# olsson-group/thermodynamic-interpolation

Hardware: AMD Instinct MI355X
Metric: integration-steps/sec (whole node) + drift rel-L2 vs CPU ref (higher is better)
Workload: dtype f32 state and accumulation; matrix products on fp16 MFMA with 2-way split fp32 operands (hi + lo halves, 3 products)

## Files before the change

### include/ti_hip.h

```cpp
#ifndef TI_HIP_H
#define TI_HIP_H

#include <stddef.h>
#include <stdint.h>

#ifdef __cplusplus
extern "C" {
#endif

#define TI_ABI_VERSION 5

enum { TI_OK = 0, TI_E_ARG = -1, TI_E_HIP = -2, TI_E_NAN = -3, TI_E_ALLOC = -4, TI_E_UNSUPPORTED = -5 };
enum { TI_MEM_HOST = 0, TI_MEM_DEVICE = 1 };
enum { TI_VARIANT_AMBIENT = 0, TI_VARIANT_LATENT_MULTI = 1, TI_VARIANT_LATENT_SINGLE = 2 };
enum { TI_PREC_F32 = 0, TI_PREC_F16X2 = 1, TI_PREC_F16 = 2 };
enum { TI_SCHEME_EULER = 0, TI_SCHEME_HEUN = 1, TI_SCHEME_EM = 2,
       TI_SCHEME_DOPRI5 = 3, TI_SCHEME_MIDPOINT = 4, TI_SCHEME_RK4 = 5,
       TI_SCHEME_DOPRI5_TRAJ = 6 };

typedef struct ti_handle ti_handle;

typedef struct ti_painn_desc {
    int32_t variant;
    int32_t n_features;
// ... 33 lines not shown

int ti_version(void);
int ti_device_count(void);
const char* ti_last_error(void);

ti_handle* ti_adw_create(const ti_adw_desc* desc, const double* weights, size_t n_weights, int device);
ti_handle* ti_adw_create_nd(const ti_adw_desc* desc, int32_t dim, const double* weights, size_t n_weights, int device);
int ti_adw_drift(ti_handle* h, const float* x, float t, const float* beta0, const float* beta1, int64_t B, float* out, int mem);
int ti_adw_drift_div(ti_handle* h, const float* x, float t, const float* beta0, const float* beta1, int64_t B, float* out,
                     float* out_div, int mem);
int ti_adw_drift_tv(ti_handle* h, const float* x, const float* t, const float* beta0, const float* beta1, int64_t B, float* out,
                    float* out_div, int mem);
int ti_adw_rollout(ti_handle* h, const ti_rollout_desc* desc, const float* x0, const float* beta0, const float* beta1,
                   int64_t B, float* out_path, int64_t* n_fevals);
int ti_adw_rollout_dlogp(ti_handle* h, const ti_rollout_desc* desc, const float* x0, const float* beta0, const float* beta1,
                         int64_t B, float* out_path, float* out_dlogp, int64_t* n_fevals);
int ti_adw_rollout_fused(ti_handle* h, const ti_rollout_desc* desc, const float* x0, const float* beta0, const float* beta1,
                         int64_t B, float* out_path, float* out_dlogp , int64_t* n_fevals);

ti_handle* ti_painn_create(const ti_painn_desc* desc, const float* weights, size_t n_weights,
                           const int32_t* edge_src, const int32_t* edge_dst, const int32_t* edge_type,
                           const int32_t* atom_ids, int device);
int ti_painn_drift(ti_handle* h, const float* x, float t, const float* cond, int64_t B, float* out, int mem);
int ti_painn_drift_tv(ti_handle* h, const float* x, const float* t, const float* cond, int64_t B, float* out, int mem);
int ti_painn_rollout(ti_handle* h, const ti_rollout_desc* desc, const float* x0, const float* cond, int64_t B,
                     float* out_path, int64_t* n_fevals);

int ti_painn_drift_jvp(ti_handle* h, const float* x, const float* xdot, float t, const float* cond, int64_t B, float* out,
                       float* out_tan, int mem);
int ti_painn_drift_div(ti_handle* h, const float* x, float t, const float* cond, int64_t B, float* out, float* out_div, int mem);
int ti_painn_drift_div_tv(ti_handle* h, const float* x, const float* t, const float* cond, int64_t B, float* out, float* out_div, int mem);
int ti_painn_rollout_dlogp(ti_handle* h, const ti_rollout_desc* desc, const float* x0, const float* cond, int64_t B,
                           float div_scale, float out_scale, int reverse_ode, float* out_path, float* out_dlogp, int64_t* n_fevals);

int ti_painn_drift_div_est(ti_handle* h, const float* x, float t, const float* cond, int64_t B, int32_t n_probes, uint64_t probe_seed,
                           int64_t traj_offset, float* out, float* out_div, int mem);
int ti_painn_drift_div_est_tv(ti_handle* h, const float* x, const float* t, const float* cond, int64_t B, int32_t n_probes,
                              uint64_t probe_seed, int64_t traj_offset, float* out, float* out_div, int mem);
int ti_painn_rollout_dlogp_est(ti_handle* h, const ti_rollout_desc* desc, int32_t n_probes, uint64_t probe_seed, const float* x0,
                               const float* cond, int64_t B, float div_scale, float out_scale, int reverse_ode, float* out_path,
                               float* out_dlogp, int64_t* n_fevals);

int ti_rollout_step_counts(ti_handle* h, int64_t* accepted, int64_t* rejected, int64_t B);
void ti_destroy(ti_handle* h);
enum { TI_STREAM_OWN = 0, TI_STREAM_EXTERNAL = 1 };
int ti_set_stream(ti_handle* h, void* hip_stream, int mode);
int ti_wait_stream(ti_handle* h, void* producer_stream);
enum { TI_TEMPLATE_AUTO = -1, TI_TEMPLATE_THROUGHPUT = 0, TI_TEMPLATE_LATENCY = 1, TI_TEMPLATE_PAIR = 2 };
int ti_painn_set_template(ti_handle* h, int which);
int ti_painn_template_for(ti_handle* h, int64_t B);
int ti_painn_set_edge_mask(ti_handle* h, const uint32_t* mask, int64_t B, int mem);
int ti_painn_set_molecules(ti_handle* h, const int32_t* n_atoms, const uint32_t* mask, const uint8_t* pair_type, int64_t B, int mem);
enum { TI_OBS_RMSD = 0, TI_OBS_DIST = 1, TI_OBS_ANGLE = 2, TI_OBS_TORSION = 3, TI_OBS_COORD = 4 };
int ti_obs_cv(ti_handle* h, const int32_t* desc, int32_t K, const float* ref, const int32_t* select, const float* x, int64_t B,
              float* out_cv, int mem);
int ti_obs_weights(ti_handle* h, const float* logw, int64_t B, float* out_w, double* out_ess, int mem);
int ti_obs_hist(ti_handle* h, const float* values, int64_t stride, const float* logw, int64_t B, int32_t n_bins, double lo, double hi,
                double* out_hist, double* out_tails, int mem);
enum { TI_BOOT_ESS = 0, TI_BOOT_TFEP = 1, TI_BOOT_MEAN = 2 };
enum { TI_BOOT_FILTER_NONE = 0, TI_BOOT_FILTER_ONCE = 1, TI_BOOT_FILTER_RESAMPLE = 2 };
#define TI_BOOT_DOMAIN 0x424f4f54u
#define TI_BOOT_MAX_RESAMPLES (1 << 20)
typedef struct {
    int32_t  estimator, filter;
    double   k;
    double   level;
    int64_t  n_boot;
    int64_t  first;
    uint64_t seed;
} ti_boot_desc;
int ti_obs_bootstrap(ti_handle* h, const float* logw, int64_t n, const ti_boot_desc* d,
                     const int32_t* idx, int64_t n_draw, double* out, double* out_boot, int mem);
int ti_obs_set_observer(ti_handle* h, const int32_t* desc, int32_t K, const float* ref, const int32_t* select, int32_t every,
                        float* out_cv, int mem);
int ti_reserve(ti_handle* h, int64_t B);
enum { TI_KERNEL_PAINN_EDGE = 0, TI_KERNEL_PAINN_UPDATE = 1, TI_KERNEL_PAINN_EMBED = 2, TI_KERNEL_PAINN_READOUT = 3,
       TI_KERNEL_ADW = 4, TI_KERNEL_INTEGRATE = 5, TI_KERNEL_PAINN_JVP_EDGE = 6, TI_KERNEL_PAINN_JVP_UPDATE = 7,
       TI_KERNEL_PAINN_JVP_READOUT = 8, TI_KERNEL_PAINN_JVP_FILTER = 9, TI_KERNEL_COUNT = 10 };
int ti_profile_enable(ti_handle* h, int on);
int ti_profile_read(ti_handle* h, int kernel, int64_t* n_launches, double* total_ms);
int ti_painn_debug_tap(ti_handle* h, int stop_after_stage);
int ti_painn_debug_read(ti_handle* h, int what, float* out, size_t n_floats);
int ti_painn_debug_poison(ti_handle* h, int64_t B, float value);
int ti_selftest(int device);

#ifdef __cplusplus
}
#endif
#endif
```

### thermodynamic-interpolation_amd/_lib.py

```python
from __future__ import annotations

import ctypes as C
import os

import numpy as np

HERE = os.path.dirname(os.path.abspath(__file__))
SO_PATH = os.environ.get("TI_LIB_PATH") or os.path.join(HERE, "libti_hip.so")

TI_OK, TI_E_ARG, TI_E_HIP, TI_E_NAN, TI_E_ALLOC, TI_E_UNSUPPORTED = 0, -1, -2, -3, -4, -5
MEM_HOST, MEM_DEVICE = 0, 1
SCHEMES = {"euler": 0, "heun": 1, "em": 2, "dopri5": 3, "midpoint": 4, "rk4": 5}
SCHEME_DOPRI5_TRAJ = 6
PRECISIONS = {"f32": 0, "f16x2": 1, "f16": 2}
KERNELS = {"painn_edge": 0, "painn_update": 1, "painn_embed": 2, "painn_readout": 3, "adw": 4, "integrate": 5,
           "painn_jvp_edge": 6, "painn_jvp_update": 7, "painn_jvp_readout": 8, "painn_jvp_filter": 9}

ABI_SYMBOLS = [
    "ti_rollout_rows", "ti_version", "ti_device_count", "ti_last_error",
    "ti_adw_create", "ti_adw_drift", "ti_adw_drift_div", "ti_adw_rollout", "ti_adw_rollout_dlogp",
    "ti_painn_create", "ti_painn_drift", "ti_painn_rollout", "ti_painn_drift_jvp", "ti_painn_drift_div", "ti_painn_rollout_dlogp",
    "ti_destroy", "ti_set_stream", "ti_wait_stream", "ti_painn_set_template", "ti_painn_template_for", "ti_reserve", "ti_profile_enable", "ti_profile_read",
    "ti_painn_debug_tap", "ti_painn_debug_read", "ti_painn_debug_poison", "ti_selftest",
    "ti_painn_drift_tv", "ti_painn_drift_div_tv", "ti_adw_drift_tv", "ti_rollout_step_counts",
    "ti_painn_drift_div_est", "ti_painn_drift_div_est_tv", "ti_painn_rollout_dlogp_est",
    "ti_adw_create_nd", "ti_painn_set_edge_mask", "ti_painn_set_molecules",
    "ti_obs_cv", "ti_obs_weights", "ti_obs_hist", "ti_obs_set_observer",
    "ti_adw_rollout_fused",
    "ti_obs_bootstrap",
]
OBS_KINDS = {"rmsd": 0, "dist": 1, "angle": 2, "torsion": 3, "coord": 4}
BOOT_ESTIMATORS = {"ess": 0, "tfep": 1, "mean": 2}
BOOT_FILTERS = {"none": 0, "once": 1, "resample": 2}
BOOT_DOMAIN = 0x424F4F54
BOOT_MAX_RESAMPLES = 1 << 20


class PainnDesc(C.Structure):
    _fields_ = [("variant", C.c_int32), ("n_features", C.c_int32), ("n_layers", C.c_int32), ("n_types", C.c_int32),
                ("n_atoms", C.c_int32), ("n_edges", C.c_int32), ("temp_length", C.c_float), ("time_length", C.c_float),
                ("length_scale", C.c_float), ("temp_mean", C.c_float), ("temp_range", C.c_float), ("precision", C.c_int32)]


class AdwDesc(C.Structure):
    _fields_ = [("hidden_size", C.c_int32), ("num_layers", C.c_int32), ("precision", C.c_int32)]


class RolloutDesc(C.Structure):
    _fields_ = [("scheme", C.c_int32), ("n_step", C.c_int32), ("save_every", C.c_int32), ("mem", C.c_int32),
                ("eps", C.c_float), ("com_free_noise", C.c_int32), ("seed", C.c_uint64), ("traj_offset", C.c_int64),
                ("t_grid", C.POINTER(C.c_float)), ("rtol", C.c_float), ("atol", C.c_float), ("step_offset", C.c_int64)]


class BootDesc(C.Structure):
    _fields_ = [("estimator", C.c_int32), ("filter", C.c_int32), ("k", C.c_double), ("level", C.c_double), ("n_boot", C.c_int64),
                ("first", C.c_int64), ("seed", C.c_uint64)]


class TiError(RuntimeError):
    def __init__(self, code, msg):
        super().__init__(f"libti_hip error {code}: {msg}")
        self.code = code


_lib = None


def _preload_torch_hip_runtime():
    import importlib.util
    try:
        spec = importlib.util.find_spec("torch")
    except (ImportError, ValueError):
        spec = None
    if spec is None or not spec.origin:
        return
    cand = os.path.join(os.path.dirname(spec.origin), "lib", "libamdhip64.so")
    if os.path.exists(cand):
        C.CDLL(cand, mode=C.RTLD_GLOBAL)


def lib():
    global _lib
    if _lib is not None:
        return _lib
    if not os.path.exists(SO_PATH):
        raise RuntimeError(f"{SO_PATH} is missing: build it with `python -c 'import __graft_entry__ as g; g.build()'` "
                           "(hipcc, gfx950).  There is no CPU fallback for the sampling path.")
    _preload_torch_hip_runtime()
    L = C.CDLL(SO_PATH)
    fp, ip, vp = C.POINTER(C.c_float), C.POINTER(C.c_int32), C.c_void_p
    L.ti_rollout_rows.restype = C.c_int64
    L.ti_rollout_rows.argtypes = [C.c_int32, C.c_int32]
    L.ti_last_error.restype = C.c_char_p
    L.ti_painn_create.restype = vp
    L.ti_painn_create.argtypes = [C.POINTER(PainnDesc), fp, C.c_size_t, ip, ip, ip, ip, C.c_int]
    L.ti_painn_drift.argtypes = [vp, vp, C.c_float, vp, C.c_int64, vp, C.c_int]
    L.ti_painn_rollout.argtypes = [vp, C.POINTER(RolloutDesc), vp, vp, C.c_int64, vp, C.POINTER(C.c_int64)]
    L.ti_painn_drift_jvp.argtypes = [vp, vp, vp, C.c_float, vp, C.c_int64, vp, vp, C.c_int]
    L.ti_painn_drift_div.argtypes = [vp, vp, C.c_float, vp, C.c_int64, vp, vp, C.c_int]
    L.ti_painn_rollout_dlogp.argtypes = [vp, C.POINTER(RolloutDesc), vp, vp, C.c_int64, C.c_float, C.c_float, C.c_int, vp, vp, C.POINTER(C.c_int64)]
    L.ti_adw_create.restype = vp
    L.ti_adw_create.argtypes = [C.POINTER(AdwDesc), C.POINTER(C.c_double), C.c_size_t, C.c_int]
    L.ti_adw_create_nd.restype = vp
    L.ti_adw_create_nd.argtypes = [C.POINTER(AdwDesc), C.c_int32, C.POINTER(C.c_double), C.c_size_t, C.c_int]
    L.ti_adw_drift.argtypes = [vp, vp, C.c_float, vp, vp, C.c_int64, vp, C.c_int]
    L.ti_adw_rollout.argtypes = [vp, C.POINTER(RolloutDesc), vp, vp, vp, C.c_int64, vp, C.POINTER(C.c_int64)]
    L.ti_adw_drift_div.argtypes = [vp, vp, C.c_float, vp, vp, C.c_int64, vp, vp, C.c_int]
    L.ti_adw_rollout_dlogp.argtypes = [vp, C.POINTER(RolloutDesc), vp, vp, vp, C.c_int64, vp, vp, C.POINTER(C.c_int64)]
    L.ti_adw_rollout_fused.argtypes = [vp, C.POINTER(RolloutDesc), vp, vp, vp, C.c_int64, vp, vp, C.POINTER(C.c_int64)]
    L.ti_destroy.argtypes = [vp]
    L.ti_destroy.restype = None
    L.ti_set_stream.argtypes = [vp, vp, C.c_int]
    L.ti_wait_stream.argtypes = [vp, vp]
    L.ti_painn_set_template.argtypes = [vp, C.c_int]
    L.ti_painn_template_for.argtypes = [vp, C.c_int64]
    L.ti_reserve.argtypes = [vp, C.c_int64]
    L.ti_profile_enable.argtypes = [vp, C.c_int]
    L.ti_profile_read.argtypes = [vp, C.c_int, C.POINTER(C.c_int64), C.POINTER(C.c_double)]
    L.ti_painn_debug_tap.argtypes = [vp, C.c_int]
    L.ti_painn_debug_read.argtypes = [vp, C.c_int, fp, C.c_size_t]
    L.ti_painn_debug_poison.argtypes = [vp, C.c_int64, C.c_float]
    L.ti_selftest.argtypes = [C.c_int]
    L.ti_painn_drift_tv.argtypes = [vp, vp, vp, vp, C.c_int64, vp, C.c_int]
    L.ti_painn_drift_div_tv.argtypes = [vp, vp, vp, vp, C.c_int64, vp, vp, C.c_int]
    L.ti_adw_drift_tv.argtypes = [vp, vp, vp, vp, vp, C.c_int64, vp, vp, C.c_int]
    L.ti_rollout_step_counts.argtypes = [vp, C.POINTER(C.c_int64), C.POINTER(C.c_int64), C.c_int64]
    L.ti_painn_drift_div_est.argtypes = [vp, vp, C.c_float, vp, C.c_int64, C.c_int32, C.c_uint64, C.c_int64, vp, vp, C.c_int]
    L.ti_painn_drift_div_est_tv.argtypes = [vp, vp, vp, vp, C.c_int64, C.c_int32, C.c_uint64, C.c_int64, vp, vp, C.c_int]
    L.ti_painn_rollout_dlogp_est.argtypes = [vp, C.POINTER(RolloutDesc), C.c_int32, C.c_uint64, vp, vp, C.c_int64, C.c_float, C.c_float,
                                             C.c_int, vp, vp, C.POINTER(C.c_int64)]
    L.ti_painn_set_edge_mask.argtypes = [vp, vp, C.c_int64, C.c_int]
    L.ti_painn_set_molecules.argtypes = [vp, vp, vp, vp, C.c_int64, C.c_int]
    L.ti_obs_cv.argtypes = [vp, ip, C.c_int32, fp, ip, vp, C.c_int64, vp, C.c_int]
    L.ti_obs_weights.argtypes = [vp, vp, C.c_int64, vp, C.POINTER(C.c_double), C.c_int]
    L.ti_obs_hist.argtypes = [vp, vp, C.c_int64, vp, C.c_int64, C.c_int32, C.c_double, C.c_double, C.POINTER(C.c_double), C.POINTER(C.c_double),
                              C.c_int]
    L.ti_obs_set_observer.argtypes = [vp, ip, C.c_int32, fp, ip, C.c_int32, vp, C.c_int]
    L.ti_obs_bootstrap.argtypes = [vp, vp, C.c_int64, C.POINTER(BootDesc), vp, C.c_int64, C.POINTER(C.c_double), vp, C.c_int]
    _lib = L
    return L


def check(rc):
    if rc != TI_OK:
        raise TiError(rc, lib().ti_last_error().decode())


def last_error() -> str:
    return lib().ti_last_error().decode()


def fptr(a: np.ndarray):
    return a.ctypes.data_as(C.POINTER(C.c_float))


def iptr(a: np.ndarray):
    return a.ctypes.data_as(C.POINTER(C.c_int32))


def as_ptr(buf, *, shape=None, out=False, what="buffer"):
    if buf is None:
        return None, None, False, None
    if isinstance(buf, int):
        return C.c_void_p(buf), None, True, None
    if hasattr(buf, "data_ptr"):
        if str(buf.dtype) != "torch.float32":
            raise TypeError(f"{what} must be float32, got {buf.dtype}")
        if not buf.is_contiguous():
            raise ValueError(f"{what} must be contiguous")
        if shape is not None and tuple(buf.shape) != tuple(shape):
            raise ValueError(f"{what} must have shape {tuple(shape)}, got {tuple(buf.shape)}")
        dev = bool(buf.is_cuda)
        return C.c_void_p(buf.data_ptr()), buf, dev, (buf.device.index if dev else None)
    if out:
        if not isinstance(buf, np.ndarray) or buf.dtype != np.float32 or not buf.flags["C_CONTIGUOUS"] or not buf.flags["WRITEABLE"]:
            raise TypeError(f"{what} must be a writable C-contiguous float32 numpy array (or a torch tensor); it is filled in place")
        a = buf
    else:
        a = np.ascontiguousarray(buf, dtype=np.float32)
    if shape is not None and tuple(a.shape) != tuple(shape):
        raise ValueError(f"{what} must have shape {tuple(shape)}, got {tuple(a.shape)}")
    return C.c_void_p(a.ctypes.data), a, False, None
```

### thermodynamic-interpolation_amd/build.py

```python
from __future__ import annotations

import os
import shutil
import subprocess
from concurrent.futures import ThreadPoolExecutor

HERE = os.path.dirname(os.path.abspath(__file__))
CSRC = os.path.join(HERE, "csrc")
SO = os.path.join(HERE, "libti_hip.so")
SOURCES = ["api_common.hip", "api_painn.hip", "api_adw.hip", "api_obs.hip", "painn_pack.hip", "painn_host.hip",
           "painn_kernels.hip", "painn_edge_nb1.hip", "painn_edge_nb2.hip", "painn_edge_nb4.hip", "painn_edge_nb8.hip",
           "painn_pair_nb1.hip", "painn_pair_nb2.hip", "painn_pair_nb4.hip", "painn_jvp_kernels.hip", "adw_kernels.hip", "ode_kernels.hip",
           "painn_edge_mask_nb1.hip", "painn_edge_mask_nb2.hip", "painn_edge_mask_nb4.hip", "painn_edge_mask_nb8.hip",
           "painn_pair_mask_nb1.hip", "painn_pair_mask_nb2.hip", "painn_pair_mask_nb4.hip",
           "ode_ragged_kernels.hip",
           "obs_kernels.hip",
           "adw_fused_kernels.hip",
           "obs_boot_kernels.hip"]
HEADERS = ["ti_handle.hpp", "rollout.hpp", "mfma_chain.hpp", "dispatch.hpp", "ti_internal.hpp", "ode_device.hpp", "adw_device.hpp", "painn_edge_kernel.hpp", "painn_pair_kernel.hpp", "pair_template.hpp",
           "painn_edge_kernel_body.inc", "painn_pair_kernel_body.inc", "painn_jvp_edge_body.inc", "painn_jvp_filter_body.inc", os.path.join("..", "..", "include", "ti_hip.h")]
FLAGS = ["--offload-arch=gfx950", "-O3", "-std=c++17", "-fPIC", "-Xclang", "-target-feature", "-Xclang", "-packed-fp32-ops"]
EXTRA_FLAGS = {"painn_edge_nb8.hip": ["-mllvm", "-amdgpu-spill-sgpr-to-vgpr=0"], "painn_edge_mask_nb8.hip": ["-mllvm", "-amdgpu-spill-sgpr-to-vgpr=0"]}


def hipcc() -> str:
    exe = shutil.which("hipcc") or "/opt/rocm/bin/hipcc"
    if not os.path.exists(exe):
        raise RuntimeError("hipcc not found (need ROCm to build libti_hip.so)")
    return exe


def _stale(target: str, deps) -> bool:
    if not os.path.exists(target):
        return True
    t = os.path.getmtime(target)
    return any(os.path.getmtime(d) > t for d in deps)


def build(force: bool = False, jobs: int = 8, verbose: bool = False) -> str:
    deps = [os.path.join(CSRC, f) for f in SOURCES + HEADERS]
    if not force and not _stale(SO, deps):
        return SO
    objdir = os.path.join(HERE, "build")
    os.makedirs(objdir, exist_ok=True)
    cc = hipcc()

    def compile_one(src):
        obj = os.path.join(objdir, src.replace(".hip", ".o"))
        if force or _stale(obj, [os.path.join(CSRC, src)] + [os.path.join(CSRC, h) for h in HEADERS]):
            cmd = [cc, *FLAGS, *EXTRA_FLAGS.get(src, []), "-c", os.path.join(CSRC, src), "-o", obj]
            if verbose:
                print(" ".join(cmd), flush=True)
            subprocess.check_call(cmd)
        return obj

    with ThreadPoolExecutor(max_workers=jobs) as ex:
        objs = list(ex.map(compile_one, SOURCES))
    subprocess.check_call([cc, "--offload-arch=gfx950", "-shared", "-fPIC", "-o", SO, *objs])
    return SO


if __name__ == "__main__":
    print(build(verbose=True))
```

### thermodynamic-interpolation_amd/csrc/api_painn.hip

```cpp
#include "rollout.hpp"

extern "C" {

ti_handle* ti_painn_create(const ti_painn_desc* d, const float* weights, size_t n_weights, const int32_t* edge_src,
                           const int32_t* edge_dst, const int32_t* edge_type, const int32_t* atom_ids, int device)
{
    ti_handle* out = nullptr;
    const int rc = guarded([&]() -> int {
        if (!d || !weights || !atom_ids) return fail(TI_E_ARG, "NULL argument");
        const int F = d->n_features, L = d->n_layers, A = d->n_atoms, E = d->n_edges;
        if (F != 32 && F != 64 && F != 128 && F != 256) return fail(TI_E_UNSUPPORTED, "n_features must be 32, 64, 128 or 256");
        if (L < 1) return fail(TI_E_ARG, "n_layers must be >= 1");
        if (A < 1 || A > 32) return fail(TI_E_UNSUPPORTED, "n_atoms must be in 1..32 (the reference caps it at n_types = 25)");
        if (E < 0 || (E > 0 && (!edge_src || !edge_dst || !edge_type))) return fail(TI_E_ARG, "edge arrays missing");
        if (d->variant < 0 || d->variant > 2) return fail(TI_E_ARG, "unknown variant");
        if (d->n_types < 1) return fail(TI_E_ARG, "n_types must be >= 1");
        if (d->precision != TI_PREC_F32 && d->precision != TI_PREC_F16X2 && d->precision != TI_PREC_F16) return fail(TI_E_ARG, "unknown precision");
        for (int k = 0; k < E; ++k)
            if (edge_src[k] < 0 || edge_src[k] >= A || edge_dst[k] < 0 || edge_dst[k] >= A || edge_type[k] < 0 || edge_type[k] > 3)
                return fail(TI_E_ARG, "edge index / type out of range");
        for (int a = 0; a < A; ++a) if (atom_ids[a] < 0 || atom_ids[a] >= d->n_types) return fail(TI_E_ARG, "atom id out of range");
        std::unique_ptr<ti_handle> h(new_handle(0, device));
        h->d = *d; h->NB = F / 32;
        h->nE = d->variant == TI_VARIANT_AMBIENT ? 4 : d->variant == TI_VARIANT_LATENT_MULTI ? 3 : 2;
        h->ncond = d->variant == TI_VARIANT_AMBIENT ? 2 : d->variant == TI_VARIANT_LATENT_MULTI ? 1 : 0;
        size_t o = 0;
        h->edge_emb = o; o += 4 * (size_t)F; h->atom_emb = o; o += (size_t)d->n_types * F;
        o = take_mlp(h->embed, o, h->nE * F, F, F);
        h->phi.resize(L); h->w.resize(L); h->upd.resize(L); h->U.resize(L); h->V.resize(L);
        for (int l = 0; l < L; ++l) {
            o = take_mlp(h->phi[l], o, 2 * F, F, 5 * F); o = take_mlp(h->w[l], o, F, F, 5 * F);
            h->U[l] = o; o += (size_t)F * F; h->V[l] = o; o += (size_t)F * F;
            o = take_mlp(h->upd[l], o, 2 * F, F, 3 * F);
        }
        o = take_mlp(h->readout, o, F, F, 2);
        h->Vr = o; o += F;
        if (o != n_weights) return fail(TI_E_ARG, "weight count mismatch: expected " + std::to_string(o) + ", got " + std::to_string(n_weights));
        h->b2_gate = weights[h->readout.b2 + 1];
        std::vector<float> flat(weights, weights + n_weights);
        if (d->precision != TI_PREC_F32)
            for (size_t i = 0; i < n_weights; ++i)
                if (!(std::fabs(weights[i]) < 65504.0f))
                    return fail(TI_E_UNSUPPORTED, "precisions f16x2 / f16 need every weight to be finite and below 65504 in magnitude (weight " + std::to_string(i) + ")");
        while (flat.size() % 4) flat.push_back(0.f);
        const size_t vr_aligned = flat.size();
        flat.insert(flat.end(), weights + h->Vr, weights + h->Vr + F);
        h->Vr = vr_aligned;
        h->flat.upload(flat);
        h->atom_ids.upload(std::vector<int32_t>(atom_ids, atom_ids + A));
        build_templates(h.get(), edge_src, edge_dst, edge_type);
        h->has_pair = pair_build_exists(h->NB, 4, d->precision) && build_pair_template(h.get(), edge_src, edge_dst, edge_type);
        select_template(h.get(), 1 << 20);
        pack_painn(h.get(), weights);
        HIP_CHECK(configure_painn_kernels(h->NB));
        HIP_CHECK(configure_painn_jvp_kernels(h->NB));
        out = h.release();
        return TI_OK;
    });
    return rc == TI_OK ? out : nullptr;
}

enum DriftMode { DRIFT, DRIFT_JVP, DRIFT_DIV, DRIFT_DIV_EST };

static int painn_drift_impl(ti_handle* h, DriftMode mode, const float* x, const float* xdot, float t, const float* tv, bool per_mol_t,
                            const float* cond, int64_t B, int32_t n_probes, uint64_t probe_seed, int64_t traj_offset, float* out,
                            float* out_tan, float* out_div, int mem)
{
    const bool jvp = mode == DRIFT_JVP, div = mode == DRIFT_DIV || mode == DRIFT_DIV_EST;
    if (!h || h->kind != 0) return fail(TI_E_ARG, "not a painn handle");
    if (mode != DRIFT && h->d.precision == TI_PREC_F16) return fail(TI_E_UNSUPPORTED, MSG_NO_FP16_TANGENT);
    if (mode == DRIFT_DIV_EST && n_probes < 1) return fail(TI_E_ARG, "n_probes must be >= 1");
    if (B < 0 || (B > 0 && (!x || (per_mol_t && !tv) || (jvp && (!xdot || !out_tan)) || !out || (div && !out_div) || (h->ncond > 0 && !cond))))
        return fail(TI_E_ARG, "NULL buffer");
    if (B == 0) return TI_OK;
    if (div && h->tap >= 0) return fail(TI_E_ARG, MSG_TAP_ENTRIES);
    return guarded([&]() -> int {
        set_device(h);
        select_template(h, B, mode == DRIFT);
        ensure_painn_ws(h, B);
        if (jvp) ensure_jvp_ws(h, B, 1);
        const size_t n = (size_t)B * h->d.n_atoms * 3, nc = (size_t)B * h->d.n_atoms * h->ncond;
        Staged sg(h, mem);
        const float* xd = sg.in(x, h->x, n);
        const float* xdd = jvp ? sg.in(xdot, h->xt, n) : nullptr;
        const float* cd = sg.in(cond, h->cond, nc);
        const float* td = per_mol_t ? sg.in(tv, h->rk_tv, (size_t)B) : nullptr;
        float* od = sg.out(out, h->b1, n);
        float* otd = jvp ? sg.out(out_tan, h->tout, n) : nullptr;
        float* dd = div ? sg.out(out_div, h->divb, (size_t)B) : nullptr;
        if (mode == DRIFT_DIV_EST) {
            painn_make_probes(h, B, n_probes, probe_seed, traj_offset);
            painn_drift_div_est_dev(h, xd, t, cd, B, n_probes, od, dd, td);
        } else if (mode == DRIFT_DIV) painn_drift_div_dev(h, xd, t, cd, B, od, dd, td);
        else {
            const JvpRun jr{1, xdd, otd};
            painn_drift_dev(h, xd, t, cd, B, od, jvp ? &jr : nullptr, td);
        }
        sg.finish(h->tap < 0);
        return TI_OK;
    });
}

int ti_painn_drift(ti_handle* h, const float* x, float t, const float* cond, int64_t B, float* out, int mem)
{
    return painn_drift_impl(h, DRIFT, x, nullptr, t, nullptr, false, cond, B, 0, 0, 0, out, nullptr, nullptr, mem);
}

int ti_painn_drift_tv(ti_handle* h, const float* x, const float* t, const float* cond, int64_t B, float* out, int mem)
{
    return painn_drift_impl(h, DRIFT, x, nullptr, 0.f, t, true, cond, B, 0, 0, 0, out, nullptr, nullptr, mem);
}

int ti_painn_drift_jvp(ti_handle* h, const float* x, const float* xdot, float t, const float* cond, int64_t B, float* out,
                       float* out_tan, int mem)
{
    return painn_drift_impl(h, DRIFT_JVP, x, xdot, t, nullptr, false, cond, B, 0, 0, 0, out, out_tan, nullptr, mem);
}

int ti_painn_drift_div(ti_handle* h, const float* x, float t, const float* cond, int64_t B, float* out, float* out_div, int mem)
{
    return painn_drift_impl(h, DRIFT_DIV, x, nullptr, t, nullptr, false, cond, B, 0, 0, 0, out, nullptr, out_div, mem);
}

int ti_painn_drift_div_tv(ti_handle* h, const float* x, const float* t, const float* cond, int64_t B, float* out, float* out_div, int mem)
{
    return painn_drift_impl(h, DRIFT_DIV, x, nullptr, 0.f, t, true, cond, B, 0, 0, 0, out, nullptr, out_div, mem);
}

int ti_painn_drift_div_est(ti_handle* h, const float* x, float t, const float* cond, int64_t B, int32_t n_probes, uint64_t probe_seed,
                           int64_t traj_offset, float* out, float* out_div, int mem)
{
    return painn_drift_impl(h, DRIFT_DIV_EST, x, nullptr, t, nullptr, false, cond, B, n_probes, probe_seed, traj_offset, out, nullptr, out_div, mem);
}

int ti_painn_drift_div_est_tv(ti_handle* h, const float* x, const float* t, const float* cond, int64_t B, int32_t n_probes,
                              uint64_t probe_seed, int64_t traj_offset, float* out, float* out_div, int mem)
{
    return painn_drift_impl(h, DRIFT_DIV_EST, x, nullptr, 0.f, t, true, cond, B, n_probes, probe_seed, traj_offset, out, nullptr, out_div, mem);
}

static int painn_rollout_impl(ti_handle* h, const ti_rollout_desc* rd, DriftMode mode, int n_probes, uint64_t probe_seed, const float* x0,
                              const float* cond, int64_t B, float div_scale, float out_scale, int reverse_ode, float* out_path,
                              float* out_dlogp, int64_t* n_fevals)
{
    const bool dlogp = mode != DRIFT;
    if (!dlogp) { if (int rc = check_rollout_desc(rd)) return rc; }
    if (!h || h->kind != 0) return fail(TI_E_ARG, "not a painn handle");
    if (dlogp) {
        if (h->d.precision == TI_PREC_F16) return fail(TI_E_UNSUPPORTED, MSG_NO_FP16_TANGENT);
        if (mode == DRIFT_DIV_EST && n_probes < 1) return fail(TI_E_ARG, "n_probes must be >= 1");
        if (int rc = check_rollout_desc(rd)) return rc;
        if (rd->scheme == TI_SCHEME_EM) return fail(TI_E_UNSUPPORTED, "dlogp is defined for the deterministic schemes only (EULER, HEUN)");
    }
    if (rd->scheme == TI_SCHEME_DOPRI5_TRAJ && h->obs[1].K > 0) return fail(TI_E_UNSUPPORTED, MSG_TRAJ_OBSERVER);
    if (B < 0 || (B > 0 && (!x0 || !out_path || (dlogp && !out_dlogp) || (h->ncond > 0 && !cond)))) return fail(TI_E_ARG, "NULL buffer");
    if (B == 0) { if (n_fevals) *n_fevals = 0; return TI_OK; }
    return guarded([&]() -> int {
        set_device(h);
        select_template(h, B, !dlogp);
        ensure_painn_ws(h, B);
        const int A = h->d.n_atoms;
        const size_t n = (size_t)B * A * 3, nc = (size_t)B * A * h->ncond;
        const hipMemcpyKind in_kind = rd->mem == TI_MEM_DEVICE ? hipMemcpyDeviceToDevice : hipMemcpyHostToDevice;
        HIP_CHECK(hipMemcpyAsync(h->x.p, x0, n * sizeof(float), in_kind, h->stream));
        const float* cd = cond;
        if (rd->mem == TI_MEM_HOST && nc) { HIP_CHECK(hipMemcpyAsync(h->cond.p, cond, nc * sizeof(float), hipMemcpyHostToDevice, h->stream)); cd = h->cond.p; }
        const int saved_tap = h->tap; h->tap = -1;
        const Ragged rg = ragged_of(h);
        if (mode == DRIFT_DIV_EST) painn_make_probes(h, B, n_probes, probe_seed, rd->traj_offset);
        DlogpAux aux;
        if (dlogp) {
            aux.dl = h->dl.p; aux.d1 = h->divb.p; aux.d2 = h->div2.p; aux.scaled = h->dlscaled.p; aux.out = out_dlogp;
            aux.n_dl = (size_t)B; aux.div_scale = div_scale; aux.out_scale = out_scale;
        }
        auto eval = [&](const float* xs, float t, const float* tv, float* o, float* dv) {
            if (!dlogp) { painn_drift_dev(h, xs, t, cd, B, o, nullptr, tv); return; }
            if (mode == DRIFT_DIV_EST) painn_drift_div_est_dev(h, xs, t, cd, B, n_probes, o, dv, tv);
            else painn_drift_div_dev(h, xs, t, cd, B, o, dv, tv);
            if (reverse_ode) {
                HIP_CHECK(launch_scale(o, o, -1.0f, (long long)n, h->stream));
                HIP_CHECK(launch_scale(dv, dv, -1.0f, (long long)B, h->stream));
            }
        };
        auto drift = [&](const float* xs, float t, float* o, float* dv) { eval(xs, t, nullptr, o, dv); };
        auto drift_tv = [&](const float* xs, const float* tv, float* o, float* dv) { eval(xs, 0.f, tv, o, dv); };
        const int rc = rd->scheme == TI_SCHEME_DOPRI5_TRAJ ? rollout_rk_traj(h, rd, h->x.p, B, A * 3, out_path, n_fevals, drift_tv, aux, rg)
                     : rd->scheme >= TI_SCHEME_DOPRI5 ? rollout_rk(h, rd, h->x.p, n, out_path, n_fevals, drift, aux, rg)
                                                      : rollout_common(h, rd, h->x.p, h->b1.p, h->b2.p, h->xt.p, n, B, A * 3, A, out_path, n_fevals, drift, aux, rg);
        h->tap = saved_tap;
        return rc;
    });
}

int ti_painn_rollout(ti_handle* h, const ti_rollout_desc* rd, const float* x0, const float* cond, int64_t B, float* out_path,
                     int64_t* n_fevals)
{
    return painn_rollout_impl(h, rd, DRIFT, 0, 0, x0, cond, B, 0.f, 0.f, 0, out_path, nullptr, n_fevals);
}

int ti_painn_rollout_dlogp(ti_handle* h, const ti_rollout_desc* rd, const float* x0, const float* cond, int64_t B, float div_scale,
                           float out_scale, int reverse_ode, float* out_path, float* out_dlogp, int64_t* n_fevals)
{
    return painn_rollout_impl(h, rd, DRIFT_DIV, 0, 0, x0, cond, B, div_scale, out_scale, reverse_ode, out_path, out_dlogp, n_fevals);
}

int ti_painn_rollout_dlogp_est(ti_handle* h, const ti_rollout_desc* rd, int32_t n_probes, uint64_t probe_seed, const float* x0,
                               const float* cond, int64_t B, float div_scale, float out_scale, int reverse_ode, float* out_path,
                               float* out_dlogp, int64_t* n_fevals)
{
    return painn_rollout_impl(h, rd, DRIFT_DIV_EST, n_probes, probe_seed, x0, cond, B, div_scale, out_scale, reverse_ode, out_path, out_dlogp, n_fevals);
}

int ti_painn_debug_tap(ti_handle* h, int stage)
{
    if (!h || h->kind != 0) return fail(TI_E_ARG, "not a painn handle");
    if (h->d.precision == TI_PREC_F16 && stage >= 0) return fail(TI_E_UNSUPPORTED, "debug taps read fp32 state; not available in the fp16 storage mode");
    h->tap = stage;
    return TI_OK;
}

int ti_painn_debug_poison(ti_handle* h, int64_t B, float value)
{
    if (!h || h->kind != 0 || B <= 0) return fail(TI_E_ARG, "not a painn handle / B");
    return guarded([&]() -> int {
        set_device(h);
        ensure_painn_ws(h, B);
        const size_t N = (size_t)B * h->d.n_atoms, F = h->d.n_features;
        const unsigned bits = __builtin_bit_cast(unsigned, value);
        HIP_CHECK(hipMemsetD32Async((hipDeviceptr_t)h->dsacc.p, (int)bits, N * F, h->stream));
        HIP_CHECK(hipMemsetD32Async((hipDeviceptr_t)h->dvacc.p, (int)bits, N * 3 * F, h->stream));
        HIP_CHECK(hipMemsetD32Async((hipDeviceptr_t)h->cacc.p, (int)bits, N * 3 * F, h->stream));
        static_assert(sizeof(*h->e.p) == 4 && sizeof(*h->enc.p) == 4 && sizeof(*h->geo.p) == 4, "32-bit fills");
        HIP_CHECK(hipMemsetD32Async((hipDeviceptr_t)h->e.p, (int)bits, h->e.n, h->stream));
        HIP_CHECK(hipMemsetD32Async((hipDeviceptr_t)h->enc.p, (int)bits, h->enc.n, h->stream));
        HIP_CHECK(hipMemsetD32Async((hipDeviceptr_t)h->geo.p, (int)bits, h->geo.n, h->stream));
        return TI_OK;
    });
}

int ti_painn_debug_read(ti_handle* h, int what, float* out, size_t n_floats)
{
    if (!h || h->kind != 0 || !out) return fail(TI_E_ARG, "bad argument");
    return guarded([&]() -> int {
        set_device(h);
        const size_t A = h->d.n_atoms, F = h->d.n_features, E = h->d.n_edges, B = (size_t)h->last_B, N = B * A;
        HIP_CHECK(hipStreamSynchronize(h->stream));
        if (what == 0) {
            if (n_floats != N * F) return fail(TI_E_ARG, "size mismatch (s)");
            std::vector<float> ds(n_floats);
            HIP_CHECK(hipMemcpy(out, h->s.p, n_floats * sizeof(float), hipMemcpyDeviceToHost));
            HIP_CHECK(hipMemcpy(ds.data(), h->dsacc.p, n_floats * sizeof(float), hipMemcpyDeviceToHost));
            for (size_t i = 0; i < n_floats; ++i) out[i] += ds[i];
        } else if (what == 1) {
            if (n_floats != N * 3 * F) return fail(TI_E_ARG, "size mismatch (v)");
            std::vector<float> v(n_floats), dv(n_floats), cc(n_floats);
            HIP_CHECK(hipMemcpy(v.data(), h->v.p, n_floats * sizeof(float), hipMemcpyDeviceToHost));
            HIP_CHECK(hipMemcpy(dv.data(), h->dvacc.p, n_floats * sizeof(float), hipMemcpyDeviceToHost));
            HIP_CHECK(hipMemcpy(cc.data(), h->cacc.p, n_floats * sizeof(float), hipMemcpyDeviceToHost));
            for (size_t nd = 0; nd < N; ++nd)
                for (size_t f = 0; f < F; ++f)
                    for (int c = 0; c < 3; ++c) {
                        const int c1 = (c + 1) % 3, c2 = (c + 2) % 3;
                        auto at = [&](const std::vector<float>& a, int cc2) { return a[(nd * 3 + cc2) * F + f]; };
                        out[(nd * 3 + c) * F + f] = (at(v, c) + at(dv, c)) + (at(cc, c1) * at(v, c2) - at(cc, c2) * at(v, c1));
                    }
        } else if (what == 2) {
            if (n_floats != B * E * F) return fail(TI_E_ARG, "size mismatch (e)");
            const size_t RB = ti::EDGE_ROWS_PER_BLOCK, rows = (B + h->G - 1) / h->G * h->parts * h->nblk * RB * (h->active == 2 ? 2 : 1);
            std::vector<float> e(rows * F);
            HIP_CHECK(hipMemcpy(e.data(), h->e.p, e.size() * sizeof(float), hipMemcpyDeviceToHost));
            for (size_t m = 0; m < B; ++m)
                for (size_t k = 0; k < E; ++k)
                    std::memcpy(out + (m * E + h->perm[k]) * F, e.data() + edge_row_of(h, m, k) * F, F * sizeof(float));
        } else if (what >= 3 && what <= 5) {
            if (h->last_D != 1 || (size_t)h->last_VB != B) return fail(TI_E_ARG, "tangent taps need a preceding ti_painn_drift_jvp call");
            auto fetch = [&](const DevBuf<float>& b, size_t n) { std::vector<float> v(n); HIP_CHECK(hipMemcpy(v.data(), b.p, n * sizeof(float), hipMemcpyDeviceToHost)); return v; };
            if (what == 3) {
                if (n_floats != N * F) return fail(TI_E_ARG, "size mismatch (ts)");
                const auto ts = fetch(h->ts, n_floats), td = fetch(h->tdsacc, n_floats);
                for (size_t i = 0; i < n_floats; ++i) out[i] = ts[i] + td[i];
            } else if (what == 4) {
                if (n_floats != N * 3 * F) return fail(TI_E_ARG, "size mismatch (tv)");
                const auto v = fetch(h->v, n_floats), cc = fetch(h->cacc, n_floats);
                const auto tv = fetch(h->tv, n_floats), tdv = fetch(h->tdvacc, n_floats), tcc = fetch(h->tcacc, n_floats);
                for (size_t nd = 0; nd < N; ++nd)
                    for (size_t f = 0; f < F; ++f)
                        for (int c = 0; c < 3; ++c) {
                            const int c1 = (c + 1) % 3, c2 = (c + 2) % 3;
                            auto at = [&](const std::vector<float>& a, int cc2) { return a[(nd * 3 + cc2) * F + f]; };
                            out[(nd * 3 + c) * F + f] = (at(tv, c) + at(tdv, c)) + ((at(tcc, c1) * at(v, c2) + at(cc, c1) * at(tv, c2)) -
                                                                                     (at(tcc, c2) * at(v, c1) + at(cc, c2) * at(tv, c1)));
                        }
            } else {
                if (n_floats != B * E * F) return fail(TI_E_ARG, "size mismatch (te)");
                const size_t RB = ti::EDGE_ROWS_PER_BLOCK, rows = (B + h->G - 1) / h->G * h->parts * h->nblk * RB;
                const auto e = fetch(h->te, rows * F);
                for (size_t m = 0; m < B; ++m)
                    for (size_t k = 0; k < E; ++k)
                        std::memcpy(out + (m * E + h->perm[k]) * F, e.data() + edge_row_of(h, m, k) * F, F * sizeof(float));
            }
        } else return fail(TI_E_ARG, "unknown tap");
        return TI_OK;
    });
}

int ti_painn_set_template(ti_handle* h, int which)
{
    if (!h || h->kind != 0) return fail(TI_E_ARG, "not a painn handle");
    if (which != TI_TEMPLATE_AUTO && which != TI_TEMPLATE_THROUGHPUT && which != TI_TEMPLATE_LATENCY && which != TI_TEMPLATE_PAIR) return fail(TI_E_ARG, "unknown template");
    if (which == TI_TEMPLATE_LATENCY && h->n_tpl < 2) which = TI_TEMPLATE_THROUGHPUT;
    if (which == TI_TEMPLATE_PAIR && !h->has_pair) which = TI_TEMPLATE_THROUGHPUT;
    h->pinned_tpl = which;
    return TI_OK;
}

int ti_painn_template_for(ti_handle* h, int64_t B)
{
    if (!h || h->kind != 0) return fail(TI_E_ARG, "not a painn handle");
// ... 53 lines not shown
```

### thermodynamic-interpolation_amd/csrc/painn_edge_kernel.hpp

```cpp
#pragma once
#include <hip/amd_detail/amd_hip_unsafe_atomics.h>

#include "dispatch.hpp"
#include "mfma_chain.hpp"
#include "ti_internal.hpp"

namespace ti {

struct EV {
    static constexpr int W_B0 = 0, W_G0 = 1, W_BE0 = 2, W_B1 = 3, W_G1 = 4, W_BE1 = 5, P_G0 = 6, P_BE0 = 7, P_B1 = 8, P_G1 = 9,
                         P_BE1 = 10, P_B2 = 11, W_B2 = 16, COUNT = 21;
};

__device__ __forceinline__ void add_noret(float* p, float v) { unsafeAtomicAdd(p, v); }
__device__ __forceinline__ void acc_out(float* p, float v, bool first)
{
    if (first) (void)__hip_atomic_exchange(p, v, __ATOMIC_RELAXED, __HIP_MEMORY_SCOPE_AGENT);
    else unsafeAtomicAdd(p, v);
}

__host__ __device__ constexpr int edge_superchunk(int NB, int WAVES, bool H16 = false) { return ((WAVES == 8 && NB == 4) ? 4 : 2) * (H16 && NB == 4 ? 2 : 1); }
__host__ __device__ constexpr int edge_chunk4(int NB, bool H16) { return (H16 ? 128 : 256) * NB; }
__host__ __device__ constexpr bool edge_build_exists(int NB, int WAVES, int PREC, int NS)
{
    return PREC >= 0 && PREC <= 2 && (WAVES == 4 ? NS == 2 || NS == 4 : WAVES == 8 && NS == 2 && NB <= 4 && !(PREC == 2 && NB == 1));
}
template <int NBK, bool FIRST, bool LAST, int PREC, int WAVES, int NS>
__global__ __launch_bounds__(64 * WAVES, (NBK <= 8 ? 2 * 4 / WAVES : 1)) void painn_edge_kernel(const EdgeParams p)
#define TI_ROWS_GROUP (gi - mg * p.parts)
#include "painn_edge_kernel_body.inc"
#undef TI_ROWS_GROUP

template <int NBK, bool FIRST, bool LAST, int PREC, int WAVES, int NS>
__global__ __launch_bounds__(64 * WAVES, (NBK <= 8 ? 2 * 4 / WAVES : 1)) void painn_edge_mask_kernel(const EdgeParams p)
#define TI_ROWS_GROUP (int)gi
#include "painn_edge_kernel_body.inc"
#undef TI_ROWS_GROUP

static size_t edge_lds_bytes(int NB, int WAVES, bool h16) { return 2 * edge_superchunk(NB, WAVES, h16) * (size_t)edge_chunk4(NB, h16) * 16 + WAVES * 256 + 21 * (size_t)32 * NB * 4; }


enum LayerPos { POS_MIDDLE = 0, POS_FIRST = 1, POS_LAST = 2, POS_ONLY = 3 };
inline int layer_pos(bool first, bool last) { return (first ? 1 : 0) | (last ? 2 : 0); }

template <int NB, bool MASK, class F>
static hipError_t with_edge_builds(int waves, int ns, int prec, int pos, F&& f)
{
    hipError_t e = hipSuccess;
    bool any = false;
    dispatch_int<4, 8>(waves, [&](auto wc) { dispatch_int<2, 4>(ns, [&](auto nc) { dispatch_int<0, 1, 2>(prec, [&](auto pc) {
        constexpr int WAVES = decltype(wc)::value, NS = decltype(nc)::value, PREC = decltype(pc)::value;
        if constexpr (edge_build_exists(NB, WAVES, PREC, NS))
            dispatch_int<POS_MIDDLE, POS_FIRST, POS_LAST, POS_ONLY>(pos, [&](auto oc) {
                constexpr bool FIRST = (decltype(oc)::value & 1) != 0, LAST = (decltype(oc)::value & 2) != 0;
                any = true;
                if (e != hipSuccess) return;
                if constexpr (MASK) e = f(painn_edge_mask_kernel<2 * NB, FIRST, LAST, PREC, WAVES, NS>, WAVES, edge_lds_bytes(NB, WAVES, PREC == 2));
                else e = f(painn_edge_kernel<2 * NB, FIRST, LAST, PREC, WAVES, NS>, WAVES, edge_lds_bytes(NB, WAVES, PREC == 2));
            });
    }); }); });
    return any ? e : hipErrorInvalidValue;
}

template <int NB, bool MASK>
hipError_t configure_edge_unit()
{
    return with_edge_builds<NB, MASK>(EVERY, EVERY, EVERY, EVERY, [](auto kernel, int, size_t lds) { return set_lds(kernel, lds); });
}
template <int NB, bool MASK>
hipError_t launch_edge_unit(bool first, bool last, int prec, const EdgeParams& p, hipStream_t st)
{
    if (p.max_slots > EDGE_MAX_SLOTS) return hipErrorInvalidValue;
    const bool wide = prec != 0 && p.n_groups >= 2048 && p.max_slots <= 2 && edge_build_exists(NB, 8, prec, 2);
    return with_edge_builds<NB, MASK>(wide ? 8 : 4, p.max_slots <= 2 ? 2 : 4, prec, layer_pos(first, last), [&](auto kernel, int waves, size_t lds) {
        hipLaunchKernelGGL(kernel, dim3((unsigned)((p.n_groups + waves - 1) / waves)), dim3(64 * waves), lds, st, p);
        return hipGetLastError();
    });
}

}
```

### thermodynamic-interpolation_amd/csrc/painn_host.hip

```cpp
#include "ti_handle.hpp"

namespace ti {

void ensure_painn_ws(ti_handle* h, long long B)
{
    if (B <= h->cap) return;
    const size_t A = h->d.n_atoms, F = h->d.n_features, N = (size_t)B * A;
    h->x.alloc(N * 3); h->b1.alloc(N * 3); h->b2.alloc(N * 3); h->xt.alloc(N * 3);
    h->cond.alloc(std::max<size_t>(N * h->ncond, 1));
    const size_t se = h->d.precision == TI_PREC_F16 ? 2 : 1;
    h->s.alloc((N * F + se - 1) / se); h->P.alloc((N * F + se - 1) / se);
    h->v.alloc((N * 3 * F + se - 1) / se); h->dvacc.alloc(N * 3 * F); h->cacc.alloc(N * 3 * F); h->dsacc.alloc(N * F);
    h->e.alloc((edge_rows_for(h, B) * F + se - 1) / se);
    h->enc.alloc((edge_rows_for(h, B) * F + se - 1) / se); h->geo.alloc(edge_rows_for(h, B) * 4);
    h->divb.alloc(B); h->div2.alloc(B); h->dl.alloc(B); h->dlscaled.alloc(B);
    h->cap = B;
}

long long jvp_virtual_molecules(const ti_handle* h, long long B, int D) { return (B + h->G - 1) / h->G * D * h->G; }

size_t jvp_bytes_per_vm(const ti_handle* h)
{
    const size_t A = h->d.n_atoms, F = h->d.n_features;
    const size_t erows = ((size_t)h->parts * h->nblk * ti::EDGE_ROWS_PER_BLOCK + h->G - 1) / h->G;
    return (A * F * 12 + erows * F + A * 3) * sizeof(float);
}

void ensure_jvp_ws(ti_handle* h, long long B, int D)
{
    const long long VB = jvp_virtual_molecules(h, B, D);
    const size_t A = h->d.n_atoms, F = h->d.n_features, N = (size_t)VB * A;
    const size_t pgroups = ((size_t)B + h->G - 1) / h->G * h->parts;
    const size_t wq_floats = std::max<size_t>(pgroups * h->nblk * 5 * h->NB * 6 * 64 * 4, 4);
    const size_t st_floats = std::max<size_t>(pgroups * h->nblk * 4 * (2 * h->NB) * 64 * 4, 4);
    grow(h->wq, wq_floats);
    grow(h->phist, st_floats);
    const size_t ns_floats = (((size_t)B * A + 15) / 16) * 13 * (2 * h->NB) * 64 * 4;
    grow(h->nodest, ns_floats);
    const size_t te_floats = (size_t)VB / h->G * h->parts * h->nblk * ti::EDGE_ROWS_PER_BLOCK * F;
    grow(h->te, te_floats);
    if (VB <= h->jvp_cap) return;
    if (N >= ((size_t)1 << 31)) throw std::invalid_argument("too many tangent nodes in one pass (lower TI_JVP_WS_GB)");
    h->ts.alloc(N * F); h->tP.alloc(N * F); h->tdsacc.alloc(N * F);
    h->tv.alloc(N * 3 * F); h->tdvacc.alloc(N * 3 * F); h->tcacc.alloc(N * 3 * F);
    h->tout.alloc(N * 3);
    h->jvp_cap = VB;
}

long long jvp_chunk_molecules(const ti_handle* h, int D)
{
    double gb = 48.0;
    if (const char* e = std::getenv("TI_JVP_WS_GB")) gb = std::max(0.001, std::atof(e));
    const double per_mol = (double)jvp_bytes_per_vm(h) * D;
    const long long by_mem = (long long)(gb * 1e9 / per_mol);
    const long long by_index = (long long)(((size_t)1 << 31) - 1) / ((long long)D * h->d.n_atoms) - h->G;
    const long long c = std::max<long long>(1, std::min(by_mem, by_index));
    return c >= h->G ? c / h->G * h->G : c;
}

#ifdef TI_STAMPS
static DevBuf<unsigned long long> stamp_buf;
static size_t stamps_len(long long groups) { return 2048 + 2 * (size_t)groups + 16; }

static unsigned long long* stamps_arm(long long groups, hipStream_t st)
{
    if (!std::getenv("TI_STAMPS_DUMP")) return nullptr;
    const size_t n_st = stamps_len(groups);
    grow(stamp_buf, n_st);
    HIP_CHECK(hipMemsetAsync(stamp_buf.p, 0, n_st * 8, st));
    return stamp_buf.p;
}

static void stamps_dump(const ti_handle* h, const unsigned long long* stamps, long long groups, hipStream_t st)
{
    if (!stamps) return;
    const size_t n_st = stamps_len(groups);
    std::vector<unsigned long long> hs(n_st);
    HIP_CHECK(hipStreamSynchronize(st));
    HIP_CHECK(hipMemcpy(hs.data(), stamps, n_st * 8, hipMemcpyDeviceToHost));
    for (int w = 0; w < 32; ++w) {
        if (!hs[(size_t)w * 64 + 1]) continue;
        std::fprintf(stderr, "STAMP %d:", w);
        for (int k = 1; k < 64 && hs[(size_t)w * 64 + k]; ++k) std::fprintf(stderr, " %llu", hs[(size_t)w * 64 + k] - hs[(size_t)w * 64 + k - 1]);
        std::fprintf(stderr, "\n");
    }
    std::vector<double> clk;
    for (long long g2 = 0; g2 < groups; ++g2) { const auto c = hs[2048 + 2 * g2], r = hs[2048 + 2 * g2 + 1]; if (r) clk.push_back(100e6 * (double)c / (double)r); }
    std::sort(clk.begin(), clk.end());
    if (!clk.empty()) std::fprintf(stderr, "INKERNEL_CLOCK_GHZ median %.4f  p10 %.4f  p90 %.4f  waves %zu  layout %d  precision %d\n", clk[clk.size() / 2] / 1e9,
                                   clk[clk.size() / 10] / 1e9, clk[clk.size() * 9 / 10] / 1e9, clk.size(), h->active, h->d.precision);
}
#endif

void painn_drift_dev(ti_handle* h, const float* x_dev, float t, const float* cond_dev, long long B, float* out_dev,
                     const JvpRun* jr, const float* tv, long long b0)
{
    const int A = h->d.n_atoms, F = h->d.n_features, L = h->d.n_layers, NB = h->NB;
    const long long N = B * A, groups = (B + h->G - 1) / h->G * h->parts;
    hipStream_t st = h->stream;
    const bool split = h->d.precision == TI_PREC_F16X2;
    const int prec = h->d.precision;
    const uint32_t* mrows = nullptr;
    if (h->emask_B > 0) {
        if (b0 % h->G) throw std::invalid_argument("an edge mask needs whole molecule groups per tangent pass (raise TI_JVP_WS_GB)");
        mrows = masked_rows(h, h->active) + (size_t)(b0 / h->G) * h->parts * h->nblk * ti::EDGE_ROWS_PER_BLOCK;
    }
    if (jr && prec == TI_PREC_F16) throw std::invalid_argument(MSG_NO_FP16_TANGENT);
    if (jr && h->active == 2) throw std::logic_error("tangent passes walk directed edge rows (select_template(.., allow_pair = false))");
    const int32_t* nat = h->ragged ? h->natoms_dev.p + b0 : nullptr;
    const float* xdot = jr ? jr->xdot : nullptr;
    if (nat) {
        const size_t n3 = (size_t)B * A * 3, nc = (size_t)B * A * h->ncond;
        grow(h->xpark, n3);
        HIP_CHECK(launch_park_pads(h->xpark.p, x_dev, nat, B, 1, A, 3, 1, st));
        x_dev = h->xpark.p;
        if (nc) {
            grow(h->cpark, nc);
            HIP_CHECK(launch_park_pads(h->cpark.p, cond_dev, nat, B, 1, A, h->ncond, 0, st));
            cond_dev = h->cpark.p;
        }
        if (xdot) {
            grow(h->dpark, n3 * jr->D);
            HIP_CHECK(launch_park_pads(h->dpark.p, xdot, nat, B * jr->D, jr->D, A, 3, 0, st));
            xdot = h->dpark.p;
        }
    }
    const long long VB = jr ? jvp_virtual_molecules(h, B, jr->D) : 0, VN = VB * A, vgroups = VB / h->G * h->parts;
    if (jr) {
        ensure_jvp_ws(h, B, jr->D);
        h->last_VB = B * jr->D; h->last_D = jr->D;
        const size_t nb = (size_t)VN * F * sizeof(float);
        HIP_CHECK(hipMemsetAsync(h->ts.p, 0, nb, st)); HIP_CHECK(hipMemsetAsync(h->tP.p, 0, nb, st));
        HIP_CHECK(hipMemsetAsync(h->tdsacc.p, 0, nb, st));
        HIP_CHECK(hipMemsetAsync(h->tv.p, 0, 3 * nb, st)); HIP_CHECK(hipMemsetAsync(h->tdvacc.p, 0, 3 * nb, st));
        HIP_CHECK(hipMemsetAsync(h->tcacc.p, 0, 3 * nb, st));
    }
    const size_t vbytes = (size_t)N * 3 * F * sizeof(float);
    const bool ft = h->first_touch && h->tap < 0;
    if (!ft || jr || L == 0) {
        HIP_CHECK(hipMemsetAsync(h->v.p, 0, prec == TI_PREC_F16 ? vbytes / 2 : vbytes, st));
        HIP_CHECK(hipMemsetAsync(h->cacc.p, 0, vbytes, st));
    }
    if (!ft) {
        HIP_CHECK(hipMemsetAsync(h->dvacc.p, 0, vbytes, st));
        HIP_CHECK(hipMemsetAsync(h->dsacc.p, 0, (size_t)N * F * sizeof(float), st));
    }
    {
        EmbedParams p{};
        p.stream = h->S(h->st_embed16); p.nch = h->st_embed16.nch; p.mlp = h->vec(h->embed);
        p.pb0 = L > 0 ? h->F(h->phi[0].b0) : h->F(h->embed.b2);
        p.atom_emb = h->F(h->atom_emb); p.atom_ids = h->atom_ids.p; p.cond = cond_dev; p.ncond = h->ncond; p.A = A; p.N = N;
        p.t = t; p.tv = tv; p.temp_length = h->d.temp_length; p.time_length = h->d.time_length; p.temp_mean = h->d.temp_mean; p.temp_range = h->d.temp_range;
        p.s = h->s.p; p.P = h->P.p;
        Timed tm(h, TI_KERNEL_PAINN_EMBED);
        HIP_CHECK(launch_embed(NB, h->nE, prec, p, st));
    }
    h->last_B = B;
    if (h->tap == 0) return;
    for (int l = 0; l < L; ++l) {
        if (jr && h->nblk > 0) {
            {
                JvpFilterParams p{};
                p.stream = h->S(h->st_edge[l]); p.nch = h->st_edge[l].nch; p.vecs = h->edge_vecs.p + (size_t)l * 21 * F;
                p.edge_emb = h->F(h->edge_emb); p.rows = h->rows.p; p.nblk = h->nblk; p.G = h->G; p.parts = h->parts; p.A = A; p.first = l == 0; p.last = l == L - 1;
                p.B = B; p.n_groups = groups; p.length_scale = h->d.length_scale; p.x = x_dev; p.P = h->P.p; p.e = h->e.p;
                p.wq = reinterpret_cast<float4*>(h->wq.p); p.st = reinterpret_cast<float4*>(h->phist.p);
                const bool typed = mrows && !h->ptype.empty();
                if (typed) p.rows = mrows;
                Timed tm(h, TI_KERNEL_PAINN_JVP_FILTER);
                HIP_CHECK(launch_jvp_filter(NB, split, p, st, typed));
            }
            JvpEdgeParams p{};
            p.stream = h->S(h->st_jvp_phi[l]); p.nch = h->st_jvp_phi[l].nch; p.pad = h->jvp_phi_pad[l]; p.vecs = h->edge_vecs.p + (size_t)l * 21 * F;
            p.edge_emb = h->F(h->edge_emb); p.rows = h->rows.p; p.slotnode = h->slotnode.p;
            p.nblk = h->nblk; p.G = h->G; p.parts = h->parts; p.A = A; p.D = jr->D; p.first = l == 0; p.last = l == L - 1;
            p.B = B; p.n_groups = vgroups;
            p.x = x_dev; p.xdot = xdot; p.P = h->P.p; p.v = h->v.p; p.e = h->e.p; p.wq = reinterpret_cast<const float4*>(h->wq.p);
            p.st = reinterpret_cast<const float4*>(h->phist.p); p.tP = h->tP.p; p.tv = h->tv.p;
            p.te = h->te.p; p.tdsacc = h->tdsacc.p; p.tdvacc = h->tdvacc.p; p.tcacc = h->tcacc.p;
            if (mrows) p.rows = mrows;
            Timed tm(h, TI_KERNEL_PAINN_JVP_EDGE);
            HIP_CHECK(launch_jvp_edge(NB, split, p, st, mrows != nullptr));
        }
        if (h->nblk > 0) {
            EdgeParams p{};
            p.stream = h->S(h->st_edge[l]); p.nch = h->st_edge[l].nch; p.vecs = h->edge_vecs.p + (size_t)l * 21 * F;
            p.edge_emb = h->F(h->edge_emb); p.rows = h->rows.p; p.slotnode = h->slotnode.p; p.nslots = nullptr;
            p.nblk = h->nblk; p.G = h->G; p.parts = h->parts; p.A = A; p.max_slots = h->max_slots; p.B = B; p.n_groups = groups; p.length_scale = h->d.length_scale;
            p.x = x_dev; p.P = h->P.p; p.v = h->v.p; p.dsacc = h->dsacc.p; p.dvacc = h->dvacc.p; p.cacc = h->cacc.p; p.e = h->e.p; p.enc = h->enc.p; p.geo = h->geo.p;
            for (int i = 0; i < 6; ++i) p.wscale[i] = 1.0f;
            if (edge_one_chain(prec)) {
                p.stream = h->S(h->st_edge1[l]); p.nch = h->st_edge1[l].nch; p.vecs = h->edge_vecs1.p + (size_t)l * 21 * F;
                for (int i = 0; i < 6; ++i) p.wscale[i] = h->edge_scale[(size_t)l * 6 + i];
            }
            if (mrows) p.rows = mrows;
            Timed tm(h, TI_KERNEL_PAINN_EDGE);
#ifdef TI_STAMPS
            if (l == 2) p.stamps = stamps_arm(groups, st);
#endif
            if (h->active == 2) {
                HIP_CHECK(launch_pair(NB, l == 0, l == L - 1, prec, p, st, mrows != nullptr));
#ifdef TI_STAMPS
                stamps_dump(h, p.stamps, groups, st);
#endif
            } else {
                HIP_CHECK(launch_edge(NB, l == 0, l == L - 1, prec, p, st, mrows != nullptr));
#ifdef TI_STAMPS
                stamps_dump(h, p.stamps, groups, st);
#endif
            }
        }
        if (h->tap == 1 + 2 * l) return;
        if (jr) {
            {
                JvpNodeParams p{};
                p.stream = h->S(h->st_jvp_update[l]); p.nch = h->st_jvp_update[l].nch; p.vecs = h->upd_vecs.p + (size_t)l * 10 * F;
                p.N = N; p.s = h->s.p; p.v = h->v.p; p.dsacc = h->dsacc.p; p.dvacc = h->dvacc.p; p.cacc = h->cacc.p;
                p.ns = reinterpret_cast<float4*>(h->nodest.p);
                Timed tm(h, TI_KERNEL_PAINN_JVP_FILTER);
                HIP_CHECK(launch_jvp_node(NB, split, p, st));
            }
            JvpUpdateParams p{};
            p.stream = h->S(h->st_jvp_update[l]); p.nch = h->st_jvp_update[l].nch; p.vecs = h->upd_vecs.p + (size_t)l * 10 * F;
            p.N = VN; p.B = B; p.A = A; p.D = jr->D; p.G = h->G; p.has_next = l + 1 < L;
            p.v = h->v.p; p.cacc = h->cacc.p; p.ns = reinterpret_cast<const float4*>(h->nodest.p);
            p.ts = h->ts.p; p.tv = h->tv.p; p.tdsacc = h->tdsacc.p; p.tdvacc = h->tdvacc.p; p.tcacc = h->tcacc.p; p.tP = h->tP.p;
            p.zero_acc = !ft;
            Timed tm(h, TI_KERNEL_PAINN_JVP_UPDATE);
            HIP_CHECK(launch_jvp_update(NB, split, p, st));
        }
        {
            UpdateParams p{};
            p.stream = h->S(h->st_update[l]); p.nch = h->st_update[l].nch; p.vecs = h->upd_vecs.p + (size_t)l * 10 * F;
            p.N = N; p.s = h->s.p; p.v = h->v.p; p.dsacc = h->dsacc.p; p.dvacc = h->dvacc.p; p.cacc = h->cacc.p; p.P = h->P.p;
            p.first_layer = l == 0; p.zero_acc = !ft;
            const bool folded = h->nblk > 0 && h->active == 2 && l > 0 && pair_folds_cross(prec);
            Timed tm(h, TI_KERNEL_PAINN_UPDATE);
            HIP_CHECK(launch_update(NB, l + 1 < L, prec, p, st, folded));
        }
        if (h->tap == 2 + 2 * l) return;
    }
    if (jr) {
        JvpReadoutParams p{};
        p.stream = h->S(h->st_jvp_readout); p.nch = h->st_jvp_readout.nch; p.vecs = h->jvp_ro_vecs.p; p.b2_gate = h->b2_gate;
        p.N = VN; p.B = B; p.A = A; p.D = jr->D; p.G = h->G; p.s = h->s.p; p.v = h->v.p; p.ts = h->ts.p; p.tv = h->tv.p; p.tout = jr->tout;
        Timed tm(h, TI_KERNEL_PAINN_JVP_READOUT);
        HIP_CHECK(launch_jvp_readout(NB, split, p, st));
    }
    {
        ReadoutParams p{};
        p.stream = h->S(h->st_jvp_readout); p.nch = h->st_jvp_readout.nch; p.mlp = h->vec(h->readout);
        p.w2_gate = h->F(h->readout.W2 + F); p.b2_gate = h->b2_gate; p.Vr = h->F(h->Vr);
        p.N = N; p.s = h->s.p; p.v = h->v.p; p.out = out_dev;
        Timed tm(h, TI_KERNEL_PAINN_READOUT);
        HIP_CHECK(launch_readout(NB, prec, p, st));
    }
    if (nat) {
        HIP_CHECK(launch_zero_pads(out_dev, nat, B, 1, A, 3, st));
        if (jr && jr->D == 1) HIP_CHECK(launch_zero_pads(jr->tout, nat, B, 1, A, 3, st));
    }
}

void painn_drift_div_dev(ti_handle* h, const float* x_dev, float t, const float* cond_dev, long long B, float* out_dev, float* div_dev,
                         const float* tv)
{
    const int A = h->d.n_atoms, D = 3 * A;
    const long long chunk = jvp_chunk_molecules(h, D);
    for (long long b0 = 0; b0 < B; b0 += chunk) {
        const long long bc = std::min(chunk, B - b0);
        ensure_jvp_ws(h, bc, D);
        JvpRun jr{D, nullptr, h->tout.p};
        painn_drift_dev(h, x_dev + (size_t)b0 * A * 3, t, cond_dev ? cond_dev + (size_t)b0 * A * h->ncond : nullptr, bc,
                        out_dev + (size_t)b0 * A * 3, &jr, tv ? tv + b0 : nullptr, b0);
        if (h->ragged) HIP_CHECK(launch_div_reduce_ragged(h->tout.p, bc, D, h->G, h->natoms_dev.p + b0, div_dev + b0, h->stream));
        else HIP_CHECK(launch_div_reduce(h->tout.p, bc, D, h->G, div_dev + b0, h->stream));
    }
    h->last_B = std::min(chunk, B);
}

void painn_make_probes(ti_handle* h, long long B, int k, uint64_t seed, long long traj0)
{
    const int n3 = 3 * h->d.n_atoms;
    grow(h->probes, (size_t)B * k * n3);
    HIP_CHECK(launch_probes(h->probes.p, seed, traj0, B, k, n3, h->stream));
// ... 61 lines not shown
```

### thermodynamic-interpolation_amd/csrc/painn_kernels.hip

```cpp
#include <hip/amd_detail/amd_hip_unsafe_atomics.h>

#include "dispatch.hpp"
#include "mfma_chain.hpp"
#include "ti_internal.hpp"

namespace ti {


struct UV {
    static constexpr int B0 = 0, G0 = 1, BE0 = 2, B1 = 3, G1 = 4, BE1 = 5, B2 = 6 , PB0 = 9, COUNT = 10;
};

__host__ __device__ constexpr int update_superchunk(int NB, bool H16) { return H16 && NB == 4 ? 4 : 2; }
__host__ __device__ constexpr int update_chunk4(int NB, bool H16) { return (H16 ? 128 : 256) * NB; }
template <int NBK, bool HAS_NEXT, int PREC, bool FOLDED = false>
__global__ __launch_bounds__(256, (NBK <= 8 ? 2 : 1)) void painn_update_kernel(const UpdateParams p)
{
    constexpr bool H16 = PREC == 2;
    constexpr int F = 16 * NBK, NB = (F + 31) / 32, WAVES = 4, T = 64 * WAVES, CH4 = update_chunk4(NB, H16);
    using A16 = r16::Act<NBK>;
    using OP = typename r16::OpSel<NBK, PREC>::type;
    extern __shared__ f32x4 lds[];
    const int lane = threadIdx.x & 63, wave = __builtin_amdgcn_readfirstlane(threadIdx.x >> 6), j = lane & 15, q = lane >> 4;
    constexpr int SC = update_superchunk(NB, H16);
// ... 338 lines not shown
    }
    pipe.drain();
    r16::ln_silu(h2, p.mlp.g1, p.mlp.be1, q);
    float gate = 0.f;
#pragma unroll
    for (int nb = 0; nb < NBK; ++nb) {
        const f32x4 w = r16::load_block(p.w2_gate, nb, q);
#pragma unroll
        for (int r = 0; r < 4; ++r) gate += h2.b[nb][r] * w[r];
    }
    gate = r16::xquarters(gate) + p.b2_gate;
#pragma unroll
    for (int c = 0; c < 3; ++c) {
        float vv = 0.f;
#pragma unroll
        for (int nb = 0; nb < NBK; ++nb) {
            const f32x4 x = r16::load_state<H16>(p.v, (nd * 3 + c) * F, nb, q), w = r16::load_block(p.Vr, nb, q);
#pragma unroll
            for (int r = 0; r < 4; ++r) vv += x[r] * w[r];
        }
        vv = r16::xquarters(vv);
        if (ok && q == 0) p.out[node * 3 + c] = vv * gate;
    }
}

static size_t update_lds_bytes(int NB, bool h16) { return 2 * update_superchunk(NB, h16) * (size_t)update_chunk4(NB, h16) * 16 + 10 * (size_t)32 * NB * 4; }
static size_t node16_lds_bytes(int NB, bool h16) { return 2 * 2 * (size_t)update_chunk4(NB, h16) * 16; }

enum NodeKernel { NODE_EMBED, NODE_UPDATE, NODE_READOUT };
constexpr bool node_build_exists(NodeKernel k, int PREC, int n, bool flag)
{
    return k == NODE_EMBED ? n >= 2 : k == NODE_UPDATE ? n <= 1 && (!flag || pair_folds_cross(PREC)) : n == 0 && !flag;
}
template <NodeKernel K, int NBK, int PREC, int N, bool FLAG>
constexpr auto node_kernel()
{
    if constexpr (K == NODE_EMBED) return painn_embed16_kernel<NBK, N, PREC, FLAG>;
    else if constexpr (K == NODE_UPDATE) return painn_update_kernel<NBK, N != 0, PREC, FLAG>;
    else return painn_readout16_kernel<NBK, PREC>;
}
template <NodeKernel K, class F>
static hipError_t with_node_builds(int NB, int prec, int n, int flag, F&& f)
{
    hipError_t e = hipSuccess;
    bool any = false;
    dispatch_int<1, 2, 4, 8>(NB, [&](auto bc) { dispatch_int<0, 1, 2>(prec, [&](auto pc) { dispatch_int<0, 1, 2, 3, 4>(n, [&](auto nc) { dispatch_bool(flag, [&](auto fc) {
        constexpr int nb = decltype(bc)::value, PREC = decltype(pc)::value, N = decltype(nc)::value;
        constexpr bool FLAG = decltype(fc)::value;
        if constexpr (node_build_exists(K, PREC, N, FLAG)) {
            any = true;
            if (e == hipSuccess) e = f(node_kernel<K, 2 * nb, PREC, N, FLAG>(), K == NODE_UPDATE ? update_lds_bytes(nb, PREC == 2) : node16_lds_bytes(nb, PREC == 2));
        }
    }); }); }); });
    return any ? e : hipErrorInvalidValue;
}
template <NodeKernel K>
static hipError_t configure_node(int NB)
{
    return with_node_builds<K>(NB, EVERY, EVERY, EVERY, [](auto kernel, size_t lds) { return set_lds(kernel, lds); });
}
template <NodeKernel K, class P>
static hipError_t launch_node(int NB, int prec, int n, bool flag, const P& p, hipStream_t st)
{
    return with_node_builds<K>(NB, prec, n, flag, [&](auto kernel, size_t lds) {
        hipLaunchKernelGGL(kernel, dim3((unsigned)((p.N + 63) / 64)), dim3(256), lds, st, p);
        return hipGetLastError();
    });
}

template <class F>
static hipError_t with_message_units(int NB, int masked, F&& f)
{
    hipError_t e = hipSuccess;
    const bool any = dispatch_int<1, 2, 4, 8>(NB, [&](auto bc) { dispatch_bool(masked, [&](auto mc) { if (e == hipSuccess) e = f(bc, mc); }); });
    return any ? e : hipErrorInvalidValue;
}

hipError_t configure_painn_kernels(int NB)
{
    hipError_t e;
    if ((e = configure_node<NODE_EMBED>(NB)) != hipSuccess) return e;
    if ((e = configure_node<NODE_UPDATE>(NB)) != hipSuccess) return e;
    if ((e = configure_node<NODE_READOUT>(NB)) != hipSuccess) return e;
    return with_message_units(NB, EVERY, [](auto bc, auto mc) {
        constexpr int nb = decltype(bc)::value;
        constexpr bool MASK = decltype(mc)::value;
        hipError_t e = configure_edge_unit<nb, MASK>();
        if constexpr (pair_build_exists(nb, 4, TI_PREC_F32)) { if (e == hipSuccess) e = configure_pair_unit<nb, MASK>(); }
        return e;
    });
}

hipError_t launch_embed(int NB, int nseg, int prec, const EmbedParams& p, hipStream_t st)
{
    return launch_node<NODE_EMBED>(NB, prec, nseg, p.tv != nullptr, p, st);
}
hipError_t launch_update(int NB, bool has_next, int prec, const UpdateParams& p, hipStream_t st, bool folded)
{
    return launch_node<NODE_UPDATE>(NB, prec, has_next, folded, p, st);
}
hipError_t launch_readout(int NB, int prec, const ReadoutParams& p, hipStream_t st) { return launch_node<NODE_READOUT>(NB, prec, 0, false, p, st); }

hipError_t launch_edge(int NB, bool first, bool last, int prec, const EdgeParams& p, hipStream_t st, bool masked)
{
    return with_message_units(NB, masked, [&](auto bc, auto mc) { return launch_edge_unit<decltype(bc)::value, decltype(mc)::value>(first, last, prec, p, st); });
}
hipError_t launch_pair(int NB, bool first, bool last, int prec, const EdgeParams& p, hipStream_t st, bool masked)
{
    return with_message_units(NB, masked, [&](auto bc, auto mc) {
        constexpr int nb = decltype(bc)::value;
        if constexpr (pair_build_exists(nb, 4, TI_PREC_F32)) return launch_pair_unit<nb, decltype(mc)::value>(first, last, prec, p, st);
        else return hipErrorInvalidValue;
    });
}

}
```

### thermodynamic-interpolation_amd/csrc/painn_pack.hip

```cpp
#include "pair_template.hpp"
#include "ti_handle.hpp"

namespace ti {

void pack_chunk16(std::vector<float>& dst, const float* W, int ld, int n_rows, int row0, int col0, int NBK)
{
    const size_t base = dst.size();
    dst.resize(base + (size_t)2 * NBK * 64 * 4);
    for (int blk = 0; blk < 2; ++blk)
        for (int nbi = 0; nbi < NBK; ++nbi)
            for (int l = 0; l < 64; ++l)
                for (int r = 0; r < 4; ++r) {
                    const int row = row0 + 16 * blk + (l & 15), col = col0 + 16 * nbi + 4 * (l >> 4) + r;
                    dst[base + ((size_t)(blk * NBK + nbi) * 64 + l) * 4 + r] = row < n_rows ? W[(size_t)row * ld + col] : 0.f;
                }
}

void pack_chunk16_split(std::vector<float>& dst, const float* W, int ld, int n_rows, int row0, int col0, int NBK)
{
    const size_t base = dst.size();
    dst.resize(base + (size_t)2 * NBK * 64 * 4);
    _Float16* out = reinterpret_cast<_Float16*>(dst.data() + base);
    const int KS = NBK / 2;
    for (int blk = 0; blk < 2; ++blk)
        for (int m = 0; m < KS; ++m)
            for (int l = 0; l < 64; ++l)
                for (int i = 0; i < 8; ++i) {
                    const int row = row0 + 16 * blk + (l & 15), col = col0 + 16 * (2 * m + (i >> 2)) + 4 * (l >> 4) + (i & 3);
                    const float w = row < n_rows ? W[(size_t)row * ld + col] : 0.f;
                    const _Float16 h = (_Float16)w;
                    const _Float16 lo = (_Float16)((w - (float)h) * 2048.0f);
                    out[((size_t)((blk * KS + m) * 2 + 0) * 64 + l) * 8 + i] = h;
                    out[((size_t)((blk * KS + m) * 2 + 1) * 64 + l) * 8 + i] = lo;
                }
}

void pack_chunk16_split1(std::vector<float>& dst, const float* W, int ld, int n_rows, int row0, int col0, int NBK, float S)
{
    const size_t base = dst.size();
    dst.resize(base + (size_t)2 * NBK * 64 * 4);
    _Float16* out = reinterpret_cast<_Float16*>(dst.data() + base);
    const int KS = NBK / 2;
    for (int blk = 0; blk < 2; ++blk)
        for (int m = 0; m < KS; ++m)
            for (int l = 0; l < 64; ++l)
                for (int i = 0; i < 8; ++i) {
                    const int row = row0 + 16 * blk + (l & 15), col = col0 + 16 * (2 * m + (i >> 2)) + 4 * (l >> 4) + (i & 3);
                    const float w = (row < n_rows ? W[(size_t)row * ld + col] : 0.f) * S;
                    const _Float16 h = (_Float16)w;
                    out[((size_t)((blk * KS + m) * 2 + 0) * 64 + l) * 8 + i] = h;
                    out[((size_t)((blk * KS + m) * 2 + 1) * 64 + l) * 8 + i] = (_Float16)(w - (float)h);
                }
}
float matrix_pow2_scale(const float* W, int ld, int rows, int col0, int cols, const float* bias = nullptr, int n_bias = 0)
{
    float mx = 0.f, mb = 0.f;
    for (int r = 0; r < rows; ++r)
        for (int c = 0; c < cols; ++c) mx = std::max(mx, std::fabs(W[(size_t)r * ld + col0 + c]));
    for (int i = 0; i < n_bias; ++i) mb = std::max(mb, std::fabs(bias[i]));
    if (!(mx > 0.f) || !std::isfinite(mx)) return 1.0f;
    int e; std::frexp(mx, &e);
    int k = std::min(60, std::max(-60, 14 - e));
    if (mb > 0.f && std::isfinite(mb)) { int eb; std::frexp(mb, &eb); k = std::min(k, std::max(-60, 14 - eb)); }
    return std::ldexp(1.0f, k);
}

void pack_chunk16_half(std::vector<float>& dst, const float* W, int ld, int n_rows, int row0, int col0, int NBK)
{
    const size_t base = dst.size();
    dst.resize(base + (size_t)NBK * 64 * 4);
    _Float16* out = reinterpret_cast<_Float16*>(dst.data() + base);
    const int KS = NBK / 2;
    for (int blk = 0; blk < 2; ++blk)
        for (int m = 0; m < KS; ++m)
            for (int l = 0; l < 64; ++l)
                for (int i = 0; i < 8; ++i) {
                    const int row = row0 + 16 * blk + (l & 15), col = col0 + 16 * (2 * m + (i >> 2)) + 4 * (l >> 4) + (i & 3);
                    out[((size_t)(blk * KS + m) * 64 + l) * 8 + i] = (_Float16)(row < n_rows ? W[(size_t)row * ld + col] : 0.f);
                }
}

size_t take_mlp(MlpOff& m, size_t o, int f_in, int f_h, int f_out)
// ... 194 lines not shown
                    if (t == 2) {
                        const long long mol = g * T.G + ti::prow_molI(w);
                        if (mol < B && !((m[mol * A + ti::prow_atomJ(w)] >> ti::prow_atomI(w)) & 1u)) w &= ~1u;
                        else if (mol < B && pt) w = (w & ~(3u << 17)) | ((uint32_t)pt[((size_t)mol * A + ti::prow_atomI(w)) * A + ti::prow_atomJ(w)] << 17);
                    } else {
                        const long long mol = g * T.G + ti::row_mol(w);
                        if (mol < B && !((m[mol * A + ti::row_dst(w)] >> ti::row_src(w)) & 1u)) w |= 63u << 18;
                        else if (mol < B && pt) w = (w & ~(3u << 16)) | ((uint32_t)pt[((size_t)mol * A + ti::row_src(w)) * A + ti::row_dst(w)] << 16);
                    }
                }
                dst[i] = w;
            }
        }
    h->mrows[t].upload(out);
    h->mrows_ok[t] = true;
    return h->mrows[t].p;
}

size_t edge_row_of(const ti_handle* h, size_t m, size_t k)
{
    const ti_handle::Tpl& T = h->tpl[h->active];
    if (h->active == 2) {
        const size_t A = h->d.n_atoms;
        return (m / T.G) * (size_t)T.nblk * 2 * ti::EDGE_ROWS_PER_BLOCK + (size_t)h->pair_pos[((m % T.G) * A + h->esrc[h->perm[k]]) * A + h->edst[h->perm[k]]];
    }
    const size_t part = T.part_of[k], r = T.pos[(m % T.G) * (size_t)h->d.n_edges + k];
    return ((m / T.G) * T.P + part) * T.nblk * ti::EDGE_ROWS_PER_BLOCK + r;
}

size_t edge_rows_for(const ti_handle* h, long long B, long long copies)
{
    size_t best = 1;
    for (int t = 0; t < h->n_tpl; ++t) {
        const ti_handle::Tpl& T = h->tpl[t];
        best = std::max<size_t>(best, (size_t)((B + T.G - 1) / T.G) * (size_t)copies * T.P * T.nblk * ti::EDGE_ROWS_PER_BLOCK);
    }
    if (h->has_pair && copies == 1)
        best = std::max<size_t>(best, (size_t)((B + h->tpl[2].G - 1) / h->tpl[2].G) * h->tpl[2].nblk * 2 * ti::EDGE_ROWS_PER_BLOCK);
    return best;
}

void pack_painn(ti_handle* h, const float* wts)
{
    const int F = h->d.n_features, L = h->d.n_layers, NB = h->NB, nE = h->nE;
    std::vector<float> pk;
    auto begin_stream = [&]() { return pk.size() / 4; };
    size_t o = 0;
    const int NBK = F / 16;
    const int prec = h->d.precision;
    const size_t ch4 = (prec == TI_PREC_F16 ? 128 : 256) * (size_t)NB;
    auto chunk16 = [&](size_t W, int ld, int n_rows, int row0, int col0) {
        if (prec == TI_PREC_F16) pack_chunk16_half(pk, wts + W, ld, n_rows, row0, col0, NBK);
        else if (prec == TI_PREC_F16X2) pack_chunk16_split(pk, wts + W, ld, n_rows, row0, col0, NBK);
        else pack_chunk16(pk, wts + W, ld, n_rows, row0, col0, NBK);
    };
    auto layer16 = [&](size_t W, int ld, int n_rows, int col0) { for (int nbo = 0; nbo < NB; ++nbo) chunk16(W, ld, n_rows, 32 * nbo, col0); };
    auto end_stream16 = [&](size_t off4) { return Stream{off4, (int)((pk.size() / 4 - off4) / ch4)}; };
    auto pad_even = [&](size_t off4) { if (((pk.size() / 4 - off4) / ch4) % 2) pk.resize(pk.size() + 4 * ch4, 0.f); };
    o = begin_stream();
    for (int seg = 0; seg < nE; ++seg) layer16(h->embed.W0, nE * F, F, seg * F);
    layer16(h->embed.W1, F, F, 0); layer16(h->embed.W2, F, F, 0);
    if (L > 0) layer16(h->phi[0].W0, 2 * F, F, 0);
    else pk.resize(pk.size() + 4 * ch4 * NB, 0.f);
    pad_even(o);
    h->st_embed16 = end_stream16(o);
    for (int l = 0; l < L; ++l) {
        const bool first = l == 0, last = l == L - 1;
        o = begin_stream();
        layer16(h->w[l].W0, F, F, 0); layer16(h->w[l].W1, F, F, 0);
        layer16(h->phi[l].W0, 2 * F, F, F);
        layer16(h->phi[l].W1, F, F, 0);
        for (int nbo = 0; nbo < NB; ++nbo)
            for (int c : {2, 3, 1, 0, 4}) {
                if (c == 3 && last) continue;
                if ((c == 0 || c == 4) && first) continue;
                chunk16(h->phi[l].W2, F, 5 * F, c * F + 32 * nbo, 0);
                chunk16(h->w[l].W2, F, 5 * F, c * F + 32 * nbo, 0);
            }
        h->st_edge.push_back(end_stream16(o));
        if (edge_one_chain(prec)) {
            const float S[6] = {matrix_pow2_scale(wts + h->w[l].W0, F, F, 0, F, wts + h->w[l].b0, F), matrix_pow2_scale(wts + h->w[l].W1, F, F, 0, F, wts + h->w[l].b1, F),
                                matrix_pow2_scale(wts + h->phi[l].W0, 2 * F, F, 0, 2 * F, wts + h->phi[l].b0, F), matrix_pow2_scale(wts + h->phi[l].W1, F, F, 0, F, wts + h->phi[l].b1, F),
                                matrix_pow2_scale(wts + h->phi[l].W2, F, 5 * F, 0, F, wts + h->phi[l].b2, 5 * F), matrix_pow2_scale(wts + h->w[l].W2, F, 5 * F, 0, F, wts + h->w[l].b2, 5 * F)};
            auto layer1 = [&](size_t W, int ld, int n_rows, int col0, float sc) { for (int nbo = 0; nbo < NB; ++nbo) pack_chunk16_split1(pk, wts + W, ld, n_rows, 32 * nbo, col0, NBK, sc); };
            o = begin_stream();
            layer1(h->w[l].W0, F, F, 0, S[0]); layer1(h->w[l].W1, F, F, 0, S[1]);
            layer1(h->phi[l].W0, 2 * F, F, F, S[2]);
            layer1(h->phi[l].W1, F, F, 0, S[3]);
            for (int nbo = 0; nbo < NB; ++nbo)
                for (int c : {2, 3, 1, 0, 4}) {
                    if (c == 3 && last) continue;
                    if ((c == 0 || c == 4) && first) continue;
                    pack_chunk16_split1(pk, wts + h->phi[l].W2, F, 5 * F, c * F + 32 * nbo, 0, NBK, S[4]);
                    pack_chunk16_split1(pk, wts + h->w[l].W2, F, 5 * F, c * F + 32 * nbo, 0, NBK, S[5]);
                }
            h->st_edge1.push_back(end_stream16(o));
            h->edge_scale.insert(h->edge_scale.end(), S, S + 6);
        }
        o = begin_stream();
        layer16(h->V[l], F, F, 0);
        layer16(h->upd[l].W0, 2 * F, F, 0); layer16(h->upd[l].W0, 2 * F, F, F);
        layer16(h->upd[l].W1, F, F, 0);
        for (int nbo = 0; nbo < NB; ++nbo) {
            chunk16(h->upd[l].W2, F, 3 * F, F + 32 * nbo, 0);
            chunk16(h->upd[l].W2, F, 3 * F, 2 * F + 32 * nbo, 0);
        }
        layer16(h->upd[l].W2, F, 3 * F, 0);
        for (int c = 0; c < 3; ++c) layer16(h->U[l], F, F, 0);
        if (!last) layer16(h->phi[l + 1].W0, 2 * F, F, 0);
        pad_even(o);
        h->st_update.push_back(end_stream16(o));
        for (int which = 1; which < 2; ++which) {
            const MlpOff& m = h->phi[l];
            o = begin_stream();
            layer16(m.W0, 2 * F, F, F);
            layer16(m.W1, F, F, 0);
            for (int nbo = 0; nbo < NB; ++nbo)
                for (int c : {2, 3, 1, 0, 4}) {
                    if (c == 3 && last) continue;
                    if ((c == 0 || c == 4) && first) continue;
                    chunk16(m.W2, F, 5 * F, c * F + 32 * nbo, 0);
                }
            const int real = end_stream16(o).nch;
            pad_even(o);
            h->st_jvp_phi.push_back(end_stream16(o));
            h->jvp_phi_pad.push_back(real & 1);
        }
        o = begin_stream();
        for (int c = 0; c < 3; ++c) layer16(h->V[l], F, F, 0);
        layer16(h->upd[l].W0, 2 * F, F, 0); layer16(h->upd[l].W0, 2 * F, F, F);
        layer16(h->upd[l].W1, F, F, 0);
        for (int nbo = 0; nbo < NB; ++nbo) {
            chunk16(h->upd[l].W2, F, 3 * F, F + 32 * nbo, 0);
            chunk16(h->upd[l].W2, F, 3 * F, 2 * F + 32 * nbo, 0);
        }
        layer16(h->upd[l].W2, F, 3 * F, 0);
        for (int c = 0; c < 3; ++c) layer16(h->U[l], F, F, 0);
        if (!last) layer16(h->phi[l + 1].W0, 2 * F, F, 0);
        pad_even(o);
        h->st_jvp_update.push_back(end_stream16(o));
    }
    o = begin_stream();
    for (size_t Wm : {h->readout.W0, h->readout.W1})
        for (int nbo = 0; nbo < NB; ++nbo) {
            chunk16(Wm, F, F, 32 * nbo, 0);
        }
    pad_even(o);
    h->st_jvp_readout = end_stream16(o);
    h->packed.upload(pk);
    {
        std::vector<float> rv;
        const MlpOff& r = h->readout;
        for (size_t off : {r.b0, r.g0, r.be0, r.b1, r.g1, r.be1, r.W2 + (size_t)F, r.b2 + 2}) rv.insert(rv.end(), wts + off, wts + off + F);
        h->jvp_ro_vecs.upload(rv);
    }
    std::vector<float> ev;
    for (int l = 0; l < L; ++l) {
        const MlpOff &w = h->w[l], &ph = h->phi[l];
        for (size_t off : {w.b0, w.g0, w.be0, w.b1, w.g1, w.be1, ph.g0, ph.be0, ph.b1, ph.g1, ph.be1}) ev.insert(ev.end(), wts + off, wts + off + F);
        ev.insert(ev.end(), wts + ph.b2, wts + ph.b2 + 5 * F);
        ev.insert(ev.end(), wts + w.b2, wts + w.b2 + 5 * F);
    }
    h->edge_vecs.upload(ev);
    if (edge_one_chain(prec)) {
        std::vector<float> ev1 = ev;
        for (int l = 0; l < L; ++l) {
            const float* S = h->edge_scale.data() + (size_t)l * 6;
            float* b = ev1.data() + (size_t)l * 21 * F;
            auto mul = [&](int row, int n, float sc) { for (int i = 0; i < n * F; ++i) b[(size_t)row * F + i] *= sc; };
            mul(0, 1, S[0]); mul(3, 1, S[1]); mul(8, 1, S[3]); mul(11, 5, S[4]); mul(16, 5, S[5]);
        }
        h->edge_vecs1.upload(ev1);
    }
    std::vector<float> uv;
    for (int l = 0; l < L; ++l) {
        const MlpOff& u = h->upd[l];
        for (size_t off : {u.b0, u.g0, u.be0, u.b1, u.g1, u.be1}) uv.insert(uv.end(), wts + off, wts + off + F);
        uv.insert(uv.end(), wts + u.b2, wts + u.b2 + 3 * F);
        if (l + 1 < L) uv.insert(uv.end(), wts + h->phi[l + 1].b0, wts + h->phi[l + 1].b0 + F);
        else uv.insert(uv.end(), F, 0.f);
// ... 6 lines not shown
```

### thermodynamic-interpolation_amd/csrc/painn_pair_kernel.hpp

```cpp
#pragma once
#include "painn_edge_kernel.hpp"

namespace ti {

__host__ __device__ constexpr int pair_superchunk() { return 2; }
static size_t pair_lds_bytes(int NB, int WAVES, int PREC)
{
    return (size_t)2 * pair_superchunk() * edge_chunk4(NB, false) * 16 + WAVES * 256 + 21 * (size_t)32 * NB * 4 +
           (pair_folds_cross(PREC) ? (size_t)WAVES * 12 * 64 * 4 : 0);
}

template <int NBK, bool FIRST, bool LAST, int PREC, int WAVES>
__global__ __launch_bounds__(64 * WAVES, 2 * 4 / WAVES) void painn_pair_kernel(const EdgeParams p)
#define TI_PAIR_ROWS p.rows
#include "painn_pair_kernel_body.inc"
#undef TI_PAIR_ROWS

template <int NBK, bool FIRST, bool LAST, int PREC, int WAVES>
__global__ __launch_bounds__(64 * WAVES, 2 * 4 / WAVES) void painn_pair_mask_kernel(const EdgeParams p)
#define TI_PAIR_ROWS (p.rows + (size_t)gi * p.nblk * 16)
#include "painn_pair_kernel_body.inc"
#undef TI_PAIR_ROWS

template <int NB, bool MASK, class F>
static hipError_t with_pair_builds(int waves, int prec, int pos, F&& f)
{
    hipError_t e = hipSuccess;
    bool any = false;
    dispatch_int<4, 8>(waves, [&](auto wc) { dispatch_int<0, 1>(prec, [&](auto pc) {
        constexpr int WAVES = decltype(wc)::value, PREC = decltype(pc)::value;
        if constexpr (pair_build_exists(NB, WAVES, PREC))
            dispatch_int<POS_MIDDLE, POS_FIRST, POS_LAST, POS_ONLY>(pos, [&](auto oc) {
                constexpr bool FIRST = (decltype(oc)::value & 1) != 0, LAST = (decltype(oc)::value & 2) != 0;
                any = true;
                if (e != hipSuccess) return;
                if constexpr (MASK) e = f(painn_pair_mask_kernel<2 * NB, FIRST, LAST, PREC, WAVES>, WAVES, pair_lds_bytes(NB, WAVES, PREC));
                else e = f(painn_pair_kernel<2 * NB, FIRST, LAST, PREC, WAVES>, WAVES, pair_lds_bytes(NB, WAVES, PREC));
            });
    }); });
    return any ? e : hipErrorInvalidValue;
}

template <int NB, bool MASK>
hipError_t configure_pair_unit()
{
    return with_pair_builds<NB, MASK>(EVERY, EVERY, EVERY, [](auto kernel, int, size_t lds) { return set_lds(kernel, lds); });
}
template <int NB, bool MASK>
hipError_t launch_pair_unit(bool first, bool last, int prec, const EdgeParams& p, hipStream_t st)
{
    const bool wide = prec == 1 && p.n_groups >= 2048;
    return with_pair_builds<NB, MASK>(wide ? 8 : 4, prec, layer_pos(first, last), [&](auto kernel, int waves, size_t lds) {
        hipLaunchKernelGGL(kernel, dim3((unsigned)((p.n_groups + waves - 1) / waves)), dim3(64 * waves), lds, st, p);
        return hipGetLastError();
    });
}

}
```

### thermodynamic-interpolation_amd/csrc/painn_pair_kernel_body.inc

```
{
    static_assert(PREC == 0 || PREC == 1, "the fp16 storage mode keeps the directed message kernel");
    constexpr int F = 16 * NBK, NB = (F + 31) / 32, T = 64 * WAVES, CH4 = edge_chunk4(NB, false);
    using A16 = r16::Act<NBK>;
    constexpr bool ONE = edge_one_chain(PREC);
    using OP = std::conditional_t<ONE, r16::Opnd1<NBK>, typename r16::OpSel<NBK, PREC>::type>;
    extern __shared__ f32x4 lds[];
    const int lane = threadIdx.x & 63, wave = __builtin_amdgcn_readfirstlane(threadIdx.x >> 6), j = lane & 15, q = lane >> 4;
    constexpr int SC = pair_superchunk(), NBUF = 2;
    float* scratch = reinterpret_cast<float*>(lds + NBUF * SC * CH4) + wave * 64;
    float* vec = reinterpret_cast<float*>(lds + NBUF * SC * CH4) + WAVES * 64;
    for (int i = threadIdx.x; i < EV::COUNT * F / 4; i += T)
        reinterpret_cast<f32x4*>(vec)[i] = reinterpret_cast<const f32x4*>(p.vecs)[i];
    PipeDMA<NB, T, SC, CH4> pipe;
    pipe.init(reinterpret_cast<const f32x4*>(p.stream), p.nch, lds, wave, lane);

    const float eps_w0 = ONE ? 1e-5f * p.wscale[0] * p.wscale[0] : 1e-5f, eps_w1 = ONE ? 1e-5f * p.wscale[1] * p.wscale[1] : 1e-5f;
    const float eps_p0 = ONE ? 1e-5f * p.wscale[2] * p.wscale[2] : 1e-5f, eps_p1 = ONE ? 1e-5f * p.wscale[3] * p.wscale[3] : 1e-5f;
    const float s_p0 = ONE ? p.wscale[2] : 1.0f, inv_out = ONE ? 1.0f / (p.wscale[4] * p.wscale[5]) : 1.0f;
    const long long gi_raw = (long long)blockIdx.x * WAVES + wave;
    const bool group_ok = gi_raw < p.n_groups;
    const long long gi = group_ok ? gi_raw : p.n_groups - 1;
    const long long gnode0 = gi * p.G * (long long)p.A;
    const unsigned mol_cap = (unsigned)(p.B - 1 - gi * p.G);
    auto lnode_of = [&](int mol_local, int atom) {
        const unsigned m = (unsigned)mol_local < mol_cap ? (unsigned)mol_local : mol_cap;
        return m * (unsigned)p.A + (unsigned)atom;
    };
    const float* const x_g = p.x + gnode0 * 3;
    const float* const P_g = p.P + gnode0 * F;
    const float* const v_g = p.v + gnode0 * 3 * F;
    float* const ds_g = p.dsacc + gnode0 * F;
    float* const dv_g = p.dvacc + gnode0 * 3 * F;
    float* const c_g = p.cacc + gnode0 * 3 * F;

#ifdef TI_STAMPS
    constexpr int STAMP_SLOTS = 64;
    const bool st_wg = blockIdx.x >= 300 && blockIdx.x < 304;
    unsigned long long* const st_buf = p.stamps ? p.stamps + ((size_t)(blockIdx.x - 300) * WAVES + wave) * STAMP_SLOTS : nullptr;
    int st_i = 0;
    unsigned long long clk0 = 0, rt0 = 0;
    if (p.stamps) { clk0 = __builtin_amdgcn_s_memtime(); rt0 = __builtin_amdgcn_s_memrealtime(); }
#define TI_STAMP() do { if (st_wg && st_buf && blk == 3 && st_i < STAMP_SLOTS) { const unsigned long long t_ = __builtin_amdgcn_s_memtime(); if (lane == 0) st_buf[st_i] = t_; ++st_i; } } while (0)
#else
#define TI_STAMP() do { } while (0)
#endif

    for (int blk = 0; blk < p.nblk; ++blk) {
        TI_STAMP();
        const uint32_t meta = TI_PAIR_ROWS[blk * 16 + j];
        const unsigned lI = lnode_of(prow_molI(meta), prow_atomI(meta)), lJ = lnode_of(prow_molJ(meta), prow_atomJ(meta));
        const bool row_ok = (meta & 1u) != 0;
        const size_t brow0 = ((size_t)gi * p.nblk + blk) * 16;
        const size_t erowA = brow0 * 2, erowB = erowA + 16;
        OP enc;
        f32x4* const enc_park = reinterpret_cast<f32x4*>(p.enc) + (brow0 / 16) * (sizeof(OP) / 16) * 64 + lane;
        f32x4* const geo_park = reinterpret_cast<f32x4*>(p.geo) + brow0 + j;
        if constexpr (FIRST) {
            const float* const xI = x_g + lI * 3u;
            const float* const xJ = x_g + lJ * 3u;
            const float rx = xI[0] - xJ[0];
            const float ry = xI[1] - xJ[1];
            const float rz = xI[2] - xJ[2];
            const float dist = sqrtf(rx * rx + ry * ry + rz * rz);
            const float den = 1.0f + dist;
            if (q == 0) {
                f32x4 dd = {rx / den, ry / den, rz / den, 0.f};
                *reinterpret_cast<f32x4*>(scratch + j * 4) = dd;
                if (group_ok && row_ok) *geo_park = dd;
            }
            A16 t;
            r16::posenc_set(t, dist / p.length_scale, q);
            enc.set(t);
            if (group_ok && row_ok) r16::opnd_store(enc, enc_park);
        } else {
            if (q == 0) {
                f32x4 dd = {0.f, 0.f, 0.f, 0.f};
                if (row_ok) dd = *geo_park;
                *reinterpret_cast<f32x4*>(scratch + j * 4) = dd;
            }
            __builtin_memset(&enc, 0, sizeof(OP));
            if (row_ok) r16::opnd_load(enc, enc_park);
        }
        TI_STAMP();
        OP g2;
        {
            OP g1;
            A16 t1;
#pragma unroll
            for (int c = 0; c < NB; ++c) {
                f32x4 a0 = r16::load_block(vec + EV::W_B0 * F, 2 * c, q), a1 = r16::load_block(vec + EV::W_B0 * F, 2 * c + 1, q);
                r16::gemm_on_pipe<false>(a0, a1, enc, pipe, lane);
                t1.b[2 * c] = a0; t1.b[2 * c + 1] = a1;
                pipe.release();
            }
            TI_STAMP();
            r16::ln_silu(t1, vec + EV::W_G0 * F, vec + EV::W_BE0 * F, q, eps_w0);
            g1.set(t1);
            TI_STAMP();
#pragma unroll
            for (int c = 0; c < NB; ++c) {
                f32x4 a0 = r16::load_block(vec + EV::W_B1 * F, 2 * c, q), a1 = r16::load_block(vec + EV::W_B1 * F, 2 * c + 1, q);
                r16::gemm_on_pipe<false>(a0, a1, g1, pipe, lane);
                t1.b[2 * c] = a0; t1.b[2 * c + 1] = a1;
                pipe.release();
            }
            TI_STAMP();
            r16::ln_silu(t1, vec + EV::W_G1 * F, vec + EV::W_BE1 * F, q, eps_w1);
            g2.set(t1);
            TI_STAMP();
        }
        OP h2A, h2B;
        {
            OP inA, inB;
            A16 tA, tB;
            float scA, scB;
            if (FIRST) {
                r16::load_set(tA, p.edge_emb + prow_type(meta) * F, q);
                scA = inA.set_scaled(tA);
                inB = inA; scB = scA;
            } else {
#pragma unroll
                for (int nb = 0; nb < NBK; ++nb) { tA.b[nb] = f32x4{0.f, 0.f, 0.f, 0.f}; tB.b[nb] = f32x4{0.f, 0.f, 0.f, 0.f}; }
                if (row_ok) {
                    r16::load_set(tA, p.e + erowA * F + (unsigned)(j * F), q);
                    r16::load_set(tB, p.e + erowB * F + (unsigned)(j * F), q);
                }
                scA = inA.set_scaled(tA);
                scB = inB.set_scaled(tB);
            }
            const float ivA = r16::pow2_inverse(scA) * s_p0, ivB = r16::pow2_inverse(scB) * s_p0;
            TI_STAMP();
#pragma unroll
            for (int c = 0; c < NB; ++c) {
                const float* const PI = P_g + lI * (unsigned)F;
                const float* const PJ = P_g + lJ * (unsigned)F;
                f32x4 a0 = r16::load_block(PI, 2 * c, q) * ivA, a1 = r16::load_block(PI, 2 * c + 1, q) * ivA;
                f32x4 b0 = r16::load_block(PJ, 2 * c, q) * ivB, b1 = r16::load_block(PJ, 2 * c + 1, q) * ivB;
                r16::gemm_x2_on_pipe<false>(a0, a1, b0, b1, inA, inB, pipe, lane);
                tA.b[2 * c] = a0 * scA; tA.b[2 * c + 1] = a1 * scA;
                tB.b[2 * c] = b0 * scB; tB.b[2 * c + 1] = b1 * scB;
                pipe.release();
            }
            TI_STAMP();
            r16::ln_silu(tA, vec + EV::P_G0 * F, vec + EV::P_BE0 * F, q, eps_p0);
            r16::ln_silu(tB, vec + EV::P_G0 * F, vec + EV::P_BE0 * F, q, eps_p0);
            inA.set(tA); inB.set(tB);
            TI_STAMP();
#pragma unroll
            for (int c = 0; c < NB; ++c) {
                f32x4 a0 = r16::load_block(vec + EV::P_B1 * F, 2 * c, q), a1 = r16::load_block(vec + EV::P_B1 * F, 2 * c + 1, q);
                f32x4 b0 = a0, b1 = a1;
                r16::gemm_x2_on_pipe<false>(a0, a1, b0, b1, inA, inB, pipe, lane);
                tA.b[2 * c] = a0; tA.b[2 * c + 1] = a1;
                tB.b[2 * c] = b0; tB.b[2 * c + 1] = b1;
                pipe.release();
            }
            TI_STAMP();
            r16::ln_silu(tA, vec + EV::P_G1 * F, vec + EV::P_BE1 * F, q, eps_p1);
            r16::ln_silu(tB, vec + EV::P_G1 * F, vec + EV::P_BE1 * F, q, eps_p1);
            h2A.set(tA); h2B.set(tB);
            TI_STAMP();
        }
        uint32_t mi[4];
#pragma unroll
        for (int r = 0; r < 4; ++r) mi[r] = TI_PAIR_ROWS[blk * 16 + 4 * q + r];
        f32x4 wfac;
#pragma unroll
        for (int r = 0; r < 4; ++r) wfac[r] = (mi[r] & 1u) ? inv_out : 0.0f;
        const int snJ = p.slotnode[blk * 16 + 4 + q], snI = p.slotnode[blk * 16 + q];
        const bool haveA = group_ok && snJ >= 0 && gi * p.G + slot_mol(snJ) < p.B;
        const bool haveB = group_ok && snI >= 0 && gi * p.G + slot_mol(snI) < p.B;
        const bool qfA = (snJ & SLOT_FIRST_TOUCH) != 0, qfB = (snI & SLOT_FIRST_TOUCH) != 0;
        const unsigned lnA = (unsigned)slot_mol(snJ) * (unsigned)p.A + (unsigned)(snJ & 255), lnB = (unsigned)slot_mol(snI) * (unsigned)p.A + (unsigned)(snI & 255);
        auto acc_ptr = [&](unsigned lnode, int off) {
            return off < F ? ds_g + (lnode * (unsigned)F + (unsigned)off) : off < 4 * F ? dv_g + (lnode * (unsigned)(3 * F) + (unsigned)(off - F)) : c_g + (lnode * (unsigned)(3 * F) + (unsigned)(off - 4 * F));
        };
        const unsigned lIq = lnode_of(prow_molI(mi[0]), prow_atomI(mi[0]));

        auto out3 = [&](int c, int nbo, f32x4& rA0, f32x4& rA1, f32x4& rB0, f32x4& rB1) {
            const float* bp = vec + (EV::P_B2 + c) * F + 32 * nbo + j;
            const float* bw = vec + (EV::W_B2 + c) * F + 32 * nbo + j;
            const float p0 = bp[0], p1 = bp[16], q0 = bw[0], q1 = bw[16];
            f32x4 a0 = {p0, p0, p0, p0}, a1 = {p1, p1, p1, p1}, b0 = a0, b1 = a1, w0 = {q0, q0, q0, q0}, w1 = {q1, q1, q1, q1};
            r16::gemm_x2_on_pipe<true>(a0, a1, b0, b1, h2A, h2B, pipe, lane);
            pipe.release();
            r16::gemm_on_pipe<true>(w0, w1, g2, pipe, lane);
            pipe.release();
            w0 *= wfac; w1 *= wfac;
            rA0 = a0 * w0; rA1 = a1 * w1;
            rB0 = b0 * w0; rB1 = b1 * w1;
        };
        auto sumA = [&](const f32x4& v) {
            using QS = r16::QuarterSum<4>;
            return QS::swap32_add(QS::swap16_add(v[0], v[1]), QS::swap16_add(v[2], v[3]));
        };
        auto putA = [&](float z0, float z1, int off) {
            if (haveA) { float* d = acc_ptr(lnA, off); acc_out(d, z0, qfA); acc_out(d + 16, z1, qfA); }
        };
        auto putB = [&](float z0, float z1, int off) {
            if (haveB) { float* d = acc_ptr(lnB, off); acc_out(d, z0, qfB); acc_out(d + 16, z1, qfB); }
        };
        auto sumB = [&](const f32x4& v) { return (v[0] + v[1]) + (v[2] + v[3]); };
        auto emitA = [&](const f32x4& v0, const f32x4& v1, int off) { putA(sumA(v0), sumA(v1), off); };
        auto emitB = [&](const f32x4& v0, const f32x4& v1, int off) { putB(sumB(v0), sumB(v1), off); };
        auto rows4 = [&](float x, float (&o)[4]) {
            float a = x, b = x;
            lane_swap16(a, b);
            o[0] = a; o[2] = a; lane_swap32(o[0], o[2]);
            o[1] = b; o[3] = b; lane_swap32(o[1], o[3]);
        };
        constexpr bool GATHER_EARLY = PREC != 0;
        constexpr bool FOLD = pair_folds_cross(PREC) && !FIRST;
        f32x4* const zpark = reinterpret_cast<f32x4*>(vec + EV::COUNT * F) + wave * 3 * 64 + lane;
        static_assert(!FOLD || GATHER_EARLY, "the fold crosses with the v[dst] rows that the early gathers hold");
        const unsigned lJq = snJ >= 0 ? lnode_of(slot_mol(snJ), snJ & 255) : lIq;
        const float wrow = (meta & 1u) ? inv_out : 0.0f;

#pragma unroll 1
        for (int nbo = 0; nbo < NB; ++nbo) {
            const int fo = 32 * nbo + j;
            TI_STAMP();
            {
                f32x4 a0, a1, b0, b1;
                out3(2, nbo, a0, a1, b0, b1);
                emitA(a0, a1, fo);
                emitB(b0, b1, fo);
            }
            TI_STAMP();
            if constexpr (!LAST) {
                f32x4 a0 = r16::load_block(vec + (EV::P_B2 + 3) * F, 2 * nbo, q), a1 = r16::load_block(vec + (EV::P_B2 + 3) * F, 2 * nbo + 1, q);
                f32x4 b0 = a0, b1 = a1;
                f32x4 w0 = r16::load_block(vec + (EV::W_B2 + 3) * F, 2 * nbo, q), w1 = r16::load_block(vec + (EV::W_B2 + 3) * F, 2 * nbo + 1, q);
                float* const ea = p.e + erowA * F + (unsigned)(j * F);
                float* const eb = p.e + erowB * F + (unsigned)(j * F);
                f32x4 oA0, oA1, oB0, oB1;
                if (FIRST) {
                    const float* em = p.edge_emb + prow_type(meta) * F;
                    oA0 = r16::load_block(em, 2 * nbo, q); oA1 = r16::load_block(em, 2 * nbo + 1, q);
                    oB0 = oA0; oB1 = oA1;
                } else {
                    oA0 = oA1 = oB0 = oB1 = f32x4{0.f, 0.f, 0.f, 0.f};
                    if (row_ok) {
                        oA0 = r16::load_block(ea, 2 * nbo, q); oA1 = r16::load_block(ea, 2 * nbo + 1, q);
                        oB0 = r16::load_block(eb, 2 * nbo, q); oB1 = r16::load_block(eb, 2 * nbo + 1, q);
                    }
                }
                r16::gemm_x2_on_pipe<false>(a0, a1, b0, b1, h2A, h2B, pipe, lane);
                pipe.release();
                r16::gemm_on_pipe<false>(w0, w1, g2, pipe, lane);
                pipe.release();
                w0 *= wrow; w1 *= wrow;
                if (group_ok && row_ok) {
                    r16::store_block(ea, 2 * nbo, q, oA0 + a0 * w0); r16::store_block(ea, 2 * nbo + 1, q, oA1 + a1 * w1);
                    r16::store_block(eb, 2 * nbo, q, oB0 + b0 * w0); r16::store_block(eb, 2 * nbo + 1, q, oB1 + b1 * w1);
                }
            }
            TI_STAMP();
            {
                f32x4 sA0, sA1, sB0, sB1, gA0 = {0, 0, 0, 0}, gA1 = {0, 0, 0, 0}, gB0 = {0, 0, 0, 0}, gB1 = {0, 0, 0, 0};
                out3(1, nbo, sA0, sA1, sB0, sB1);
                float vI[3][2], vJ[3][2];
                if (!FIRST) {
                    const float* vp = v_g + (lIq * (unsigned)(3 * F) + (unsigned)fo);
                    const float* vq = v_g + (lJq * (unsigned)(3 * F) + (unsigned)fo);
#pragma unroll
                    for (int c = 0; c < 3; ++c) {
                        vI[c][0] = vp[c * F]; vI[c][1] = vp[c * F + 16];
                        if (GATHER_EARLY) { vJ[c][0] = vq[c * F]; vJ[c][1] = vq[c * F + 16]; }
                    }
                    out3(0, nbo, gA0, gA1, gB0, gB1);
                }
                f32x4 dir[4];
#pragma unroll
                for (int r = 0; r < 4; ++r) dir[r] = *reinterpret_cast<const f32x4*>(scratch + (4 * q + r) * 4);
                float zA[3][2], zB[3][2];
#pragma unroll
                for (int c = 0; c < 3; ++c) {
                    f32x4 v0, v1;
#pragma unroll
                    for (int r = 0; r < 4; ++r) {
                        v0[r] = sA0[r] * dir[r][c]; v1[r] = sA1[r] * dir[r][c];
                        if (!FIRST) { v0[r] = fmaf(gA0[r], vI[c][0], v0[r]); v1[r] = fmaf(gA1[r], vI[c][1], v1[r]); }
                    }
                    zA[c][0] = sumA(v0); zA[c][1] = sumA(v1);
                    if (!GATHER_EARLY) putA(zA[c][0], zA[c][1], (1 + c) * F + fo);
                }
#pragma unroll
                for (int c = 0; c < 3; ++c) {
                    f32x4 v0, v1;
                    float j0[4], j1[4];
                    if (!FIRST) {
                        if (GATHER_EARLY) { rows4(vJ[c][0], j0); rows4(vJ[c][1], j1); }
                        else
#pragma unroll
                            for (int r = 0; r < 4; ++r) {
                                const float* vr = v_g + (lnode_of(prow_molJ(mi[r]), prow_atomJ(mi[r])) * (unsigned)(3 * F) + (unsigned)(c * F + fo));
                                j0[r] = vr[0]; j1[r] = vr[16];
                            }
                    }
#pragma unroll
                    for (int r = 0; r < 4; ++r) {
                        v0[r] = -(sB0[r] * dir[r][c]); v1[r] = -(sB1[r] * dir[r][c]);
                        if (!FIRST) { v0[r] = fmaf(gB0[r], j0[r], v0[r]); v1[r] = fmaf(gB1[r], j1[r], v1[r]); }
                    }
                    zB[c][0] = sumB(v0); zB[c][1] = sumB(v1);
                    if (!GATHER_EARLY) putB(zB[c][0], zB[c][1], (1 + c) * F + fo);
                }
                TI_STAMP();
                if constexpr (FOLD) {
                    zpark[0] = f32x4{zA[0][0], zA[0][1], zA[1][0], zA[1][1]};
                    zpark[64] = f32x4{zA[2][0], zA[2][1], zB[0][0], zB[0][1]};
                    zpark[128] = f32x4{zB[1][0], zB[1][1], zB[2][0], zB[2][1]};
                    f32x4 cA0, cA1, cB0, cB1;
                    out3(4, nbo, cA0, cA1, cB0, cB1);
                    f32x4 dc[4];
#pragma unroll
                    for (int r = 0; r < 4; ++r) dc[r] = *reinterpret_cast<const f32x4*>(scratch + (4 * q + r) * 4);
                    {
                        const f32x4 z0 = zpark[0], z1 = zpark[64], z2 = zpark[128];
                        zA[0][0] = z0[0]; zA[0][1] = z0[1]; zA[1][0] = z0[2]; zA[1][1] = z0[3];
                        zA[2][0] = z1[0]; zA[2][1] = z1[1]; zB[0][0] = z1[2]; zB[0][1] = z1[3];
                        zB[1][0] = z2[0]; zB[1][1] = z2[1]; zB[2][0] = z2[2]; zB[2][1] = z2[3];
                    }
                    float kA[3][2], kB[3][2];
#pragma unroll
                    for (int c = 0; c < 3; ++c) {
                        f32x4 a0, a1, b0, b1;
#pragma unroll
                        for (int r = 0; r < 4; ++r) {
                            a0[r] = cA0[r] * dc[r][c]; a1[r] = cA1[r] * dc[r][c];
                            b0[r] = -(cB0[r] * dc[r][c]); b1[r] = -(cB1[r] * dc[r][c]);
                        }
                        kA[c][0] = sumA(a0); kA[c][1] = sumA(a1);
                        kB[c][0] = sumB(b0); kB[c][1] = sumB(b1);
                    }
#pragma unroll
                    for (int c = 0; c < 3; ++c) {
                        const int c1 = (c + 1) % 3, c2 = (c + 2) % 3;
#pragma unroll
                        for (int h = 0; h < 2; ++h) {
                            zA[c][h] += kA[c1][h] * vJ[c2][h] - kA[c2][h] * vJ[c1][h];
                            zB[c][h] += kB[c1][h] * vI[c2][h] - kB[c2][h] * vI[c1][h];
                        }
                    }
                }
                if (GATHER_EARLY)
#pragma unroll
                    for (int c = 0; c < 3; ++c) { putA(zA[c][0], zA[c][1], (1 + c) * F + fo); putB(zB[c][0], zB[c][1], (1 + c) * F + fo); }
                if (!FIRST && !FOLD) {
                    f32x4 cA0, cA1, cB0, cB1;
                    out3(4, nbo, cA0, cA1, cB0, cB1);
#pragma unroll
                    for (int c = 0; c < 3; ++c) {
                        f32x4 v0, v1;
#pragma unroll
                        for (int r = 0; r < 4; ++r) { v0[r] = cA0[r] * dir[r][c]; v1[r] = cA1[r] * dir[r][c]; }
                        emitA(v0, v1, (4 + c) * F + fo);
                    }
#pragma unroll
                    for (int c = 0; c < 3; ++c) {
                        f32x4 v0, v1;
#pragma unroll
                        for (int r = 0; r < 4; ++r) { v0[r] = -(cB0[r] * dir[r][c]); v1[r] = -(cB1[r] * dir[r][c]); }
                        emitB(v0, v1, (4 + c) * F + fo);
                    }
                }
            }
        }
    }
    pipe.drain();
#ifdef TI_STAMPS
    if (p.stamps && lane == 0) {
        const unsigned long long clk1 = __builtin_amdgcn_s_memtime(), rt1 = __builtin_amdgcn_s_memrealtime();
        unsigned long long* c = p.stamps + 2048 + 2 * (size_t)gi_raw;
        c[0] = clk1 - clk0; c[1] = rt1 - rt0;
    }
#endif
}
```

### thermodynamic-interpolation_amd/csrc/painn_pair_mask_nb1.hip

```cpp
#include "painn_pair_kernel.hpp"

namespace ti {
template hipError_t configure_pair_unit<1, true>();
template hipError_t launch_pair_unit<1, true>(bool, bool, int, const EdgeParams&, hipStream_t);
}
```

### thermodynamic-interpolation_amd/csrc/painn_pair_mask_nb2.hip

```cpp
#include "painn_pair_kernel.hpp"

namespace ti {
template hipError_t configure_pair_unit<2, true>();
template hipError_t launch_pair_unit<2, true>(bool, bool, int, const EdgeParams&, hipStream_t);
}
```

### thermodynamic-interpolation_amd/csrc/painn_pair_mask_nb4.hip

```cpp
#include "painn_pair_kernel.hpp"

namespace ti {
template hipError_t configure_pair_unit<4, true>();
template hipError_t launch_pair_unit<4, true>(bool, bool, int, const EdgeParams&, hipStream_t);
}
```

### thermodynamic-interpolation_amd/csrc/painn_pair_nb1.hip

```cpp
#include "painn_pair_kernel.hpp"

namespace ti {
template hipError_t configure_pair_unit<1, false>();
template hipError_t launch_pair_unit<1, false>(bool, bool, int, const EdgeParams&, hipStream_t);
}
```

### thermodynamic-interpolation_amd/csrc/painn_pair_nb2.hip

```cpp
#include "painn_pair_kernel.hpp"

namespace ti {
template hipError_t configure_pair_unit<2, false>();
template hipError_t launch_pair_unit<2, false>(bool, bool, int, const EdgeParams&, hipStream_t);
}
```

### thermodynamic-interpolation_amd/csrc/painn_pair_nb4.hip

```cpp
#include "painn_pair_kernel.hpp"

namespace ti {
template hipError_t configure_pair_unit<4, false>();
template hipError_t launch_pair_unit<4, false>(bool, bool, int, const EdgeParams&, hipStream_t);
}
```

### thermodynamic-interpolation_amd/csrc/ti_handle.hpp

```cpp
#pragma once
#include <algorithm>
#include <array>
#include <climits>
#include <cmath>
#include <cstdio>
#include <cstdlib>
#include <cstring>
#include <map>
#include <memory>
#include <stdexcept>
#include <string>
#include <utility>
#include <vector>

#include "ti_internal.hpp"

namespace ti {

int fail(int code, const std::string& msg);

struct HipError : std::runtime_error { using std::runtime_error::runtime_error; };
struct Unsupported : std::runtime_error { using std::runtime_error::runtime_error; };
#define HIP_CHECK(expr) do { hipError_t e__ = (expr); if (e__ != hipSuccess) \
    throw HipError(std::string(#expr) + ": " + hipGetErrorString(e__)); } while (0)

constexpr const char* MSG_NO_FP16_TANGENT = "the fp16 storage mode has no divergence / tangent path (use f32 or f16x2)";
constexpr const char* MSG_TRAJ_OBSERVER = "TI_SCHEME_DOPRI5_TRAJ writes its rows per trajectory inside a kernel: detach the observer (ti_obs_set_observer)";
constexpr const char* MSG_TAP_ENTRIES = "debug taps apply to ti_painn_drift / ti_painn_drift_jvp only";
constexpr const char* MSG_EM_DLOGP = "dlogp is defined for a deterministic flow: EM needs eps = 0";

struct MlpOff { size_t W0, b0, g0, be0, W1, b1, g1, be1, W2, b2; int f_in, f_h, f_out; };

template <typename T>
struct DevBuf {
    T* p = nullptr; size_t n = 0;
    void alloc(size_t count) { release(); if (count) { HIP_CHECK(hipMalloc((void**)&p, count * sizeof(T))); n = count; } }
    void upload(const std::vector<T>& h) { alloc(h.size()); if (n) HIP_CHECK(hipMemcpy(p, h.data(), n * sizeof(T), hipMemcpyHostToDevice)); }
    void release() { if (p) { (void)hipFree(p); p = nullptr; n = 0; } }
    ~DevBuf() { release(); }
};

template <typename T>
void grow(DevBuf<T>& b, size_t n) { if (b.n < n) b.alloc(n); }

struct Stream { size_t off4; int nch; };

}

using namespace ti;

struct ti_handle {
    int kind = 0;
    int device = 0;
    hipStream_t own_stream = nullptr, stream = nullptr;
    hipEvent_t wait_ev = nullptr;
    bool prof = false;
    std::vector<std::pair<hipEvent_t, hipEvent_t>> ev[TI_KERNEL_COUNT];
    DevBuf<float> flat, packed;
    DevBuf<int> nanflag;
    long long cap = 0;

    ti_painn_desc d{};
    int NB = 0, nE = 0, ncond = 0, G = 1, nblk = 0;
    MlpOff embed{}, readout{}; std::vector<MlpOff> phi, w, upd; std::vector<size_t> U, V;
    size_t edge_emb = 0, atom_emb = 0, Vr = 0; float b2_gate = 0.f;
    Stream st_embed16{}; std::vector<Stream> st_edge, st_edge1, st_update;
    struct Tpl {
        int G = 1, P = 1, nblk = 0;
        DevBuf<uint32_t> rows; DevBuf<int32_t> slotnode;
        std::vector<uint32_t> rows_h;
        std::vector<int> part_of, part_start, part_len;
        std::vector<int> pos;
        int max_slots = 0;
    } tpl[3];
    bool has_pair = false; std::vector<int> pair_pos; double pair_fill = 0.0;
    int n_tpl = 1, active = 0, parts = 1, max_slots = 0, pinned_tpl = TI_TEMPLATE_AUTO;
    bool first_touch = false;
    std::vector<uint32_t> emask; long long emask_B = 0; bool emask_sym = true;
    DevBuf<uint32_t> mrows[3]; bool mrows_ok[3] = {false, false, false};
    std::vector<int32_t> natoms; std::vector<uint8_t> ptype; bool ragged = false; long long n_real = 0;
    DevBuf<int32_t> natoms_dev; DevBuf<float> xpark, cpark, dpark;
    struct { const uint32_t* p = nullptr; } rows; struct { const int32_t* p = nullptr; } slotnode;
    DevBuf<int32_t> atom_ids;
    std::vector<int> perm;
    std::vector<int32_t> esrc, edst;
    DevBuf<float> x, cond, s, P, v, dsacc, dvacc, cacc, e, enc, geo, b1, b2, xt, edge_vecs, edge_vecs1, upd_vecs;
    std::vector<float> edge_scale;
    int tap = -1; long long last_B = 0;
    std::vector<Stream> st_jvp_update, st_jvp_phi; Stream st_jvp_readout{}; std::vector<int> jvp_phi_pad;
    DevBuf<float> jvp_ro_vecs, ts, tP, tv, tdsacc, tdvacc, tcacc, te, tout, wq, phist, nodest, divb, dl, dlscaled, div2;
    long long jvp_cap = 0, last_VB = 0; int last_D = 1;
    DevBuf<float> probes;
    DevBuf<float> rk_ws; DevBuf<double> rk_red;
    DevBuf<TrajCtl> rk_ctl; DevBuf<float> rk_tv, rk_path, rk_dpath; DevBuf<int> rk_status; DevBuf<double> rk_grid;
    std::vector<int64_t> traj_accepted, traj_rejected;

    ti_adw_desc ad{};
    size_t a_be_vecs = 0, a_net_vecs = 0;
    float a_be_b_out = 0.f, a_b_out = 0.f;
    int a_dim = 1;
    Stream st_be{}, st_net{};
    DevBuf<float> ax, ab1, ab2, axt, aemb_u, abeta0_u, abeta1_u, adl, ad1, ad2; DevBuf<int32_t> aidx;
    DevBuf<float> abeta0_r, abeta1_r, aemb_r, atv;
    DevBuf<float> af_b0, af_b1, af_tv, af_emb, af_path, af_dl; DevBuf<AdwFusedStep> af_steps;

    struct ObsSet { int K = 0; bool has_ref = false, has_sel = false; DevBuf<int32_t> desc, sel; DevBuf<float> ref; } obs[2];
    int obs_every = 0, obs_mem = TI_MEM_HOST; float* obs_out = nullptr;
    DevBuf<float> obs_x, obs_cv, obs_val, obs_logw, obs_w; DevBuf<double> obs_red, obs_part;
    DevBuf<float> boot_pop; DevBuf<int32_t> boot_idx; DevBuf<double> boot_est, boot_pt; DevBuf<int> boot_flag;

    ~ti_handle()
    {
        for (auto& v2 : ev) for (auto& pr : v2) { (void)hipEventDestroy(pr.first); (void)hipEventDestroy(pr.second); }
        if (wait_ev) (void)hipEventDestroy(wait_ev);
        if (own_stream) (void)hipStreamDestroy(own_stream);
    }
    const float* F(size_t off) const { return flat.p + off; }
    const float4* S(const Stream& s2) const { return reinterpret_cast<const float4*>(packed.p) + s2.off4; }
    MlpVec vec(const MlpOff& m) const { return MlpVec{F(m.b0), F(m.g0), F(m.be0), F(m.b1), F(m.g1), F(m.be1), F(m.b2)}; }
};

namespace ti {

struct Timed {
    ti_handle* h; int slot; hipEvent_t a = nullptr, b = nullptr;
    Timed(ti_handle* h_, int slot_) : h(h_), slot(slot_)
    {
        if (!h->prof) return;
        HIP_CHECK(hipEventCreate(&a)); HIP_CHECK(hipEventCreate(&b));
        HIP_CHECK(hipEventRecord(a, h->stream));
    }
    ~Timed()
    {
        if (!a) return;
        (void)hipEventRecord(b, h->stream);
        h->ev[slot].emplace_back(a, b);
    }
};

inline void set_device(const ti_handle* h) { HIP_CHECK(hipSetDevice(h->device)); }

template <typename Fn>
int guarded(Fn&& fn)
{
    try { return fn(); }
    catch (const HipError& e) { return fail(TI_E_HIP, e.what()); }
    catch (const Unsupported& e) { return fail(TI_E_UNSUPPORTED, e.what()); }
    catch (const std::bad_alloc&) { return fail(TI_E_ALLOC, "host allocation failed"); }
    catch (const std::exception& e) { return fail(TI_E_ARG, e.what()); }
}

inline ti_handle* new_handle(int kind, int device)
{
    int ndev = 0;
    if (hipGetDeviceCount(&ndev) != hipSuccess || ndev <= 0) throw HipError("no HIP device available (libti_hip has no CPU fallback)");
    if (device < 0 || device >= ndev) throw std::invalid_argument("device index out of range");
    HIP_CHECK(hipSetDevice(device));
    std::unique_ptr<ti_handle> h(new ti_handle());
    h->kind = kind; h->device = device;
    HIP_CHECK(hipStreamCreateWithFlags(&h->own_stream, hipStreamNonBlocking));
    h->stream = h->own_stream;
    h->nanflag.alloc(1);
    return h.release();
}

struct Staged {
    ti_handle* h; bool host;
    struct { void* dst; const void* src; size_t bytes; } back[2] = {}; int n_back = 0;
    Staged(ti_handle* h_, int mem) : h(h_), host(mem == TI_MEM_HOST) {}
    template <typename T>
    const T* in(const T* p, DevBuf<T>& b, size_t n)
    {
        if (!host) return p;
        grow(b, n);
        if (n) HIP_CHECK(hipMemcpyAsync(b.p, p, n * sizeof(T), hipMemcpyHostToDevice, h->stream));
        return b.p;
    }
    template <typename T>
    T* out(T* p, DevBuf<T>& b, size_t n)
    {
        if (!host) return p;
        grow(b, n);
        back[n_back++] = {p, b.p, n * sizeof(T)};
        return b.p;
    }
    void finish(bool copy_back = true)
    {
        for (int i = 0; copy_back && i < n_back; ++i) HIP_CHECK(hipMemcpyAsync(back[i].dst, back[i].src, back[i].bytes, hipMemcpyDeviceToHost, h->stream));
        HIP_CHECK(hipStreamSynchronize(h->stream));
    }
};

struct JvpRun {
    int D;
    const float* xdot;
    float* tout;
};

inline int obs_floats_per_traj(const ti_handle* h) { return h->kind == 0 ? 3 * h->d.n_atoms : h->a_dim; }

void pack_chunk16(std::vector<float>& dst, const float* W, int ld, int n_rows, int row0, int col0, int NBK);
void pack_chunk16_split(std::vector<float>& dst, const float* W, int ld, int n_rows, int row0, int col0, int NBK);
size_t take_mlp(MlpOff& m, size_t o, int f_in, int f_h, int f_out);
void pack_painn(ti_handle* h, const float* wts);
void build_templates(ti_handle* h, const int32_t* src, const int32_t* dst, const int32_t* etype);
bool build_pair_template(ti_handle* h, const int32_t* src, const int32_t* dst, const int32_t* etype);
int pinned_template(const ti_handle* h);
bool mask_blocks_pair(const ti_handle* h);
int template_for(const ti_handle* h, long long B, bool allow_pair = true);
void select_template(ti_handle* h, long long B, bool allow_pair = true);
const uint32_t* masked_rows(ti_handle* h, int t);
size_t edge_row_of(const ti_handle* h, size_t m, size_t k);
size_t edge_rows_for(const ti_handle* h, long long B, long long copies = 1);

void ensure_painn_ws(ti_handle* h, long long B);
void ensure_jvp_ws(ti_handle* h, long long B, int D);
void painn_drift_dev(ti_handle* h, const float* x_dev, float t, const float* cond_dev, long long B, float* out_dev,
                     const JvpRun* jr = nullptr, const float* tv = nullptr, long long b0 = 0);
void painn_drift_div_dev(ti_handle* h, const float* x_dev, float t, const float* cond_dev, long long B, float* out_dev, float* div_dev,
                         const float* tv = nullptr);
void painn_make_probes(ti_handle* h, long long B, int k, uint64_t seed, long long traj0);
void painn_drift_div_est_dev(ti_handle* h, const float* x_dev, float t, const float* cond_dev, long long B, int k, float* out_dev,
                             float* est_dev, const float* tv = nullptr);
int set_graph_state(ti_handle* h, std::vector<uint32_t>& m, std::vector<int32_t>& natoms, std::vector<uint8_t>& ptype, long long B);
void clear_graph_state(ti_handle* h);

void ensure_adw_ws(ti_handle* h, long long B);
void obs_cv_dev(ti_handle* h, int which, const float* x_dev, long long B, float* cv_dev);

}
```

### thermodynamic-interpolation_amd/csrc/ti_internal.hpp

```cpp
#pragma once
#include <hip/hip_runtime.h>
#include <stdint.h>

#include <algorithm>
#include <string>
#include <vector>

#include "../../include/ti_hip.h"

namespace ti {

constexpr int32_t SLOT_FIRST_TOUCH = 1 << 30;
__host__ __device__ inline int slot_mol(int32_t sn) { return (sn >> 8) & 0x3fffff; }
constexpr int ROW_VALID = 1;
constexpr int EDGE_ROWS_PER_BLOCK = 16;
constexpr int EDGE_MAX_SLOTS = 4;
__host__ __device__ inline int row_mol(uint32_t w) { return (w >> 1) & 31; }
__host__ __device__ inline int row_src(uint32_t w) { return (w >> 6) & 31; }
__host__ __device__ inline int row_dst(uint32_t w) { return (w >> 11) & 31; }
__host__ __device__ inline int row_type(uint32_t w) { return (w >> 16) & 3; }
__host__ __device__ inline int row_slot(uint32_t w) { return (w >> 18) & 63; }

constexpr int PAIR_MAX_G = 8;
__host__ __device__ inline int prow_molI(uint32_t w) { return (w >> 1) & 7; }
__host__ __device__ inline int prow_atomI(uint32_t w) { return (w >> 4) & 31; }
__host__ __device__ inline int prow_molJ(uint32_t w) { return (w >> 9) & 7; }
__host__ __device__ inline int prow_atomJ(uint32_t w) { return (w >> 12) & 31; }
__host__ __device__ inline int prow_type(uint32_t w) { return (w >> 17) & 3; }

struct MlpVec {
    const float *b0, *g0, *be0, *b1, *g1, *be1, *b2;
};

struct EdgeParams {
    const float4* stream; int nch;
    const float* vecs;
    const float* edge_emb;
    const uint32_t* rows; const int32_t* slotnode; const int32_t* nslots;
    int nblk, G, parts, A;
    int max_slots;
    long long B, n_groups;
    float length_scale;
    const float* x;
    const float* P;
    const float* v;
    float* dsacc;
    float* dvacc;
    float* cacc;
    float* e;
    float* enc;
    float wscale[6];
    float* geo;
    unsigned long long* stamps;
};

struct EmbedParams {
    const float4* stream; int nch;
    MlpVec mlp; const float* pb0;
    const float* atom_emb; const int32_t* atom_ids; const float* cond;
    int ncond, A; long long N;
    float t, temp_length, time_length, temp_mean, temp_range;
    const float* tv;
    float* s; float* P;
};

struct UpdateParams {
    const float4* stream; int nch;
    const float* vecs;
    long long N;
    float *s, *v, *dsacc, *dvacc, *cacc, *P;
    int first_layer;
    int zero_acc;
};

struct ReadoutParams {
    const float4* stream; int nch;
    MlpVec mlp; const float* w2_gate; float b2_gate; const float* Vr;
    long long N;
    const float *s, *v; float* out;
};

hipError_t launch_embed(int NB, int nseg, int prec, const EmbedParams& p, hipStream_t st);
hipError_t launch_edge(int NB, bool first, bool last, int prec, const EdgeParams& p, hipStream_t st, bool masked = false);
__host__ __device__ constexpr bool edge_one_chain(int prec) { return prec == TI_PREC_F16X2; }
hipError_t launch_pair(int NB, bool first, bool last, int prec, const EdgeParams& p, hipStream_t st, bool masked = false);
__host__ __device__ constexpr bool pair_build_exists(int NB, int WAVES, int PREC)
{
    return (NB == 1 || NB == 2 || NB == 4) && (PREC == TI_PREC_F32 ? WAVES == 4 : PREC == TI_PREC_F16X2 && (WAVES == 4 || WAVES == 8));
}
__host__ __device__ constexpr bool pair_folds_cross(int prec) { return prec == TI_PREC_F16X2; }
hipError_t launch_update(int NB, bool has_next, int prec, const UpdateParams& p, hipStream_t st, bool folded = false);
hipError_t launch_readout(int NB, int prec, const ReadoutParams& p, hipStream_t st);
hipError_t configure_painn_kernels(int NB);
template <int NB, bool MASK> hipError_t launch_edge_unit(bool first, bool last, int prec, const EdgeParams& p, hipStream_t st);
template <int NB, bool MASK> hipError_t configure_edge_unit();
template <int NB, bool MASK> hipError_t launch_pair_unit(bool first, bool last, int prec, const EdgeParams& p, hipStream_t st);
template <int NB, bool MASK> hipError_t configure_pair_unit();

struct JvpFilterParams {
    const float4* stream; int nch; const float* vecs; const float* edge_emb;
    const uint32_t* rows;
    int nblk, G, parts, A, first, last;
    long long B, n_groups;
    float length_scale;
    const float *x, *P, *e;
    float4* wq;
    float4* st;
};
struct JvpEdgeParams {
    const float4* stream; int nch, pad; const float* vecs; const float* edge_emb;
    const uint32_t* rows; const int32_t* slotnode;
    int nblk, G, parts, A, D, first, last;
    long long B, n_groups;
    const float *x, *xdot;
    const float *P, *v, *e;
    const float4 *wq, *st;
    const float *tP, *tv;
    float *te, *tdsacc, *tdvacc, *tcacc;
};
struct JvpNodeParams {
    const float4* stream; int nch; const float* vecs;
    long long N;
    const float *s, *v, *dsacc, *dvacc, *cacc;
    float4* ns;
};
struct JvpUpdateParams {
    const float4* stream; int nch; const float* vecs;
    long long N, B; int A, D, G, has_next;
    const float *v, *cacc;
    const float4* ns;
    float *ts, *tv, *tdsacc, *tdvacc, *tcacc, *tP;
    int zero_acc;
};
struct JvpReadoutParams {
    const float4* stream; int nch; const float* vecs; float b2_gate;
    long long N, B; int A, D, G;
    const float *s, *v, *ts, *tv;
    float* tout;
};
hipError_t launch_jvp_filter(int NB, bool split, const JvpFilterParams& p, hipStream_t st, bool masked = false);
hipError_t launch_jvp_edge(int NB, bool split, const JvpEdgeParams& p, hipStream_t st, bool masked = false);
hipError_t launch_jvp_node(int NB, bool split, const JvpNodeParams& p, hipStream_t st);
hipError_t launch_jvp_update(int NB, bool split, const JvpUpdateParams& p, hipStream_t st);
hipError_t launch_jvp_readout(int NB, bool split, const JvpReadoutParams& p, hipStream_t st);
hipError_t launch_div_reduce(const float* tout, long long B, int D, int G, float* div, hipStream_t st);
hipError_t launch_hutch_reduce(const float* tout, const float* eps, long long B, int k, int A, int G, float* est, hipStream_t st);
hipError_t configure_painn_jvp_kernels(int NB);

struct AdwParams {
    const float4* stream; int nch;
    const float* vecs;
    float b_out;
    int n_hidden; long long B;
    const float* x; const float* in1; const float* emb; const int32_t* idx;
    float t;
    float* out;
    float* out_div;
    int dim;
};
hipError_t launch_adw(int NB, bool split, const AdwParams& p, hipStream_t st);
hipError_t configure_adw_kernels(int NB, int max_hidden, int dim);

enum { ADW_FUSED_EULER = 0, ADW_FUSED_HEUN = 1, ADW_FUSED_EM = 2 };
struct AdwFusedStep {
    float t, t_next;
    float dt, hdt;
    float ndt, nhdt;
    float sigma;
    float pad;
};
struct AdwFusedParams {
    const float4* stream; int nch;
    const float* vecs;
    float b_out;
    int n_hidden; long long B;
    float* x;
    const int32_t* idx;
    const float* emb; long long U;
    const AdwFusedStep* steps;
// ... 113 lines not shown
```

### thermodynamic-interpolation_amd/engine.py

```python
from __future__ import annotations

import ctypes as C

import numpy as np

from . import _lib
from . import weights as W


def time_grid(start: float, end: float, n_step: int) -> np.ndarray:
    try:
        import torch
        return torch.linspace(float(start), float(end), int(n_step), dtype=torch.float32).numpy().copy()
    except ImportError:
        return _time_grid_numpy(start, end, n_step)


def _time_grid_numpy(start: float, end: float, n_step: int) -> np.ndarray:
    start, end = np.float32(start), np.float32(end)
    if n_step == 1:
        return np.asarray([start], np.float32)
    step = np.float32((end - start) / np.float32(n_step - 1))
    i = np.arange(n_step, dtype=np.int64)
    lo = start + step * i.astype(np.float32)
# ... 339 lines not shown
        on_gpu = hasattr(x0, "data_ptr") and x0.is_cuda
        rd = _rollout_desc(scheme, t_grid, save_every, _lib.MEM_DEVICE if on_gpu else _lib.MEM_HOST, eps, seed, traj_offset, com_free_noise,
                           rtol, atol, step_offset, step_control)
        rows = int(_lib.lib().ti_rollout_rows(rd.n_step, rd.save_every))
        if out is None:
            out = _alloc_like(x0 if on_gpu else None, (rows, B, self.A, 3))
        (xp, cp, op), dev, keep = self._ptrs((x0, (B, self.A, 3), False, "x0"), self._cond_spec(cond, B), (out, (rows, B, self.A, 3), True, "out"))
        nfe = C.c_int64(0)
        _lib.check(_lib.lib().ti_painn_rollout(self.h, C.byref(rd), xp, cp, B, op, C.byref(nfe)))
        return out, nfe.value

    def jvp(self, x, xdot, t, cond=None):
        B = self._check_x(x)
        like = x if hasattr(x, "data_ptr") and x.is_cuda else None
        out, tan = _alloc_like(like, (B, self.A, 3)), _alloc_like(like, (B, self.A, 3))
        (xp, tp, cp, op, tnp), dev, keep = self._ptrs((x, (B, self.A, 3), False, "x"), (xdot, (B, self.A, 3), False, "xdot"), self._cond_spec(cond, B),
                                                      (out, None, True, "out"), (tan, None, True, "out_tan"))
        _lib.check(_lib.lib().ti_painn_drift_jvp(self.h, xp, tp, float(t), cp, B, op, tnp, _lib.MEM_DEVICE if dev else _lib.MEM_HOST))
        return out, tan

    def drift_div(self, x, t, cond=None):
        B = self._check_x(x)
        like = x if hasattr(x, "data_ptr") and x.is_cuda else None
        out, div = _alloc_like(like, (B, self.A, 3)), _alloc_like(like, (B,))
        tv = self._times(t, B)
        if tv is not None:
            (xp, tp, cp, op, dp), dev, keep = self._ptrs((x, (B, self.A, 3), False, "x"), tv, self._cond_spec(cond, B), (out, None, True, "out"),
                                                         (div, None, True, "out_div"))
            _lib.check(_lib.lib().ti_painn_drift_div_tv(self.h, xp, tp, cp, B, op, dp, _lib.MEM_DEVICE if dev else _lib.MEM_HOST))
            return out, div
        (xp, cp, op, dp), dev, keep = self._ptrs((x, (B, self.A, 3), False, "x"), self._cond_spec(cond, B), (out, None, True, "out"), (div, None, True, "out_div"))
        _lib.check(_lib.lib().ti_painn_drift_div(self.h, xp, float(t), cp, B, op, dp, _lib.MEM_DEVICE if dev else _lib.MEM_HOST))
        return out, div

    def rollout_dlogp(self, x0, cond, t_grid, scheme="euler", save_every=1, div_scale=1.0, out_scale=1.0, reverse_ode=False,
                      rtol=1e-4, atol=1e-4, step_control="batch"):
        B = self._check_x(x0, "x0")
        on_gpu = hasattr(x0, "data_ptr") and x0.is_cuda
        rd = _rollout_desc(scheme, t_grid, save_every, _lib.MEM_DEVICE if on_gpu else _lib.MEM_HOST, 0.0, 0, 0, False, rtol, atol,
                           step_control=step_control)
        rows = int(_lib.lib().ti_rollout_rows(rd.n_step, rd.save_every))
        out, dl = _alloc_like(x0 if on_gpu else None, (rows, B, self.A, 3)), _alloc_like(x0 if on_gpu else None, (rows, B))
        (xp, cp, op, dp), dev, keep = self._ptrs((x0, (B, self.A, 3), False, "x0"), self._cond_spec(cond, B), (out, None, True, "out"), (dl, None, True, "out_dlogp"))
        nfe = C.c_int64(0)
        _lib.check(_lib.lib().ti_painn_rollout_dlogp(self.h, C.byref(rd), xp, cp, B, float(div_scale), float(out_scale), int(bool(reverse_ode)),
                                                     op, dp, C.byref(nfe)))
        return out, dl, nfe.value

    def drift_div_est(self, x, t, cond=None, n_probes=1, probe_seed=0, traj_offset=0):
        B = self._check_x(x)
        like = x if hasattr(x, "data_ptr") and x.is_cuda else None
        out, div = _alloc_like(like, (B, self.A, 3)), _alloc_like(like, (B,))
        tv = self._times(t, B)
        mem = lambda dev: _lib.MEM_DEVICE if dev else _lib.MEM_HOST
        if tv is not None:
            (xp, tp, cp, op, dp), dev, keep = self._ptrs((x, (B, self.A, 3), False, "x"), tv, self._cond_spec(cond, B), (out, None, True, "out"),
                                                         (div, None, True, "out_div"))
            _lib.check(_lib.lib().ti_painn_drift_div_est_tv(self.h, xp, tp, cp, B, int(n_probes), int(probe_seed), int(traj_offset), op, dp, mem(dev)))
            return out, div
        (xp, cp, op, dp), dev, keep = self._ptrs((x, (B, self.A, 3), False, "x"), self._cond_spec(cond, B), (out, None, True, "out"), (div, None, True, "out_div"))
        _lib.check(_lib.lib().ti_painn_drift_div_est(self.h, xp, float(t), cp, B, int(n_probes), int(probe_seed), int(traj_offset), op, dp, mem(dev)))
        return out, div

    def rollout_dlogp_est(self, x0, cond, t_grid, n_probes=1, probe_seed=0, traj_offset=0, scheme="euler", save_every=1, div_scale=1.0,
                          out_scale=1.0, reverse_ode=False, rtol=1e-4, atol=1e-4, step_control="batch"):
        B = self._check_x(x0, "x0")
        on_gpu = hasattr(x0, "data_ptr") and x0.is_cuda
        rd = _rollout_desc(scheme, t_grid, save_every, _lib.MEM_DEVICE if on_gpu else _lib.MEM_HOST, 0.0, 0, traj_offset, False, rtol, atol,
                           step_control=step_control)
        rows = int(_lib.lib().ti_rollout_rows(rd.n_step, rd.save_every))
        out, dl = _alloc_like(x0 if on_gpu else None, (rows, B, self.A, 3)), _alloc_like(x0 if on_gpu else None, (rows, B))
        (xp, cp, op, dp), dev, keep = self._ptrs((x0, (B, self.A, 3), False, "x0"), self._cond_spec(cond, B), (out, None, True, "out"), (dl, None, True, "out_dlogp"))
        nfe = C.c_int64(0)
        _lib.check(_lib.lib().ti_painn_rollout_dlogp_est(self.h, C.byref(rd), int(n_probes), int(probe_seed), xp, cp, B, float(div_scale),
                                                         float(out_scale), int(bool(reverse_ode)), op, dp, C.byref(nfe)))
        return out, dl, nfe.value

    def debug_tap(self, stage: int):
        _lib.check(_lib.lib().ti_painn_debug_tap(self.h, int(stage)))

    def debug_poison(self, B: int, value: float):
        _lib.check(_lib.lib().ti_painn_debug_poison(self.h, int(B), float(value)))

    def debug_read(self, what: str, B: int):
        shape = {"s": (B, self.A, self.F), "v": (B, self.A, 3, self.F), "e": (B, self.E, self.F)}[what[-1]]
        out = np.empty(shape, np.float32)
        _lib.check(_lib.lib().ti_painn_debug_read(self.h, {"s": 0, "v": 1, "e": 2, "ts": 3, "tv": 4, "te": 5}[what], _lib.fptr(out), out.size))
        return out


class AdwEngine(_Engine):

    def __init__(self, hidden, num_layers, flat_weights_f64, device=0, precision="f32", dim=1):
        if precision not in _lib.PRECISIONS:
            raise ValueError(f"precision must be one of {sorted(_lib.PRECISIONS)}")
        self.hidden, self.num_layers, self.precision, self.dim = int(hidden), int(num_layers), precision, int(dim)
        self.desc = _lib.AdwDesc(self.hidden, self.num_layers, _lib.PRECISIONS[precision])
        w = np.ascontiguousarray(flat_weights_f64, np.float64)
        self.device = int(device)
        if self.dim == 1:
            self.h = _lib.lib().ti_adw_create(C.byref(self.desc), w.ctypes.data_as(C.POINTER(C.c_double)), w.size, self.device)
        else:
            self.h = _lib.lib().ti_adw_create_nd(C.byref(self.desc), self.dim, w.ctypes.data_as(C.POINTER(C.c_double)), w.size, self.device)
        if not self.h:
            raise _lib.TiError(-1, _lib.last_error())

    def _obs_x_shape(self, x):
        B = int(x.shape[0])
        return B, self._xs(B)

    def _xs(self, *lead):
        return tuple(lead) + ((self.dim,) if self.dim > 1 else ())

    def drift(self, x, t, beta0, beta1, out=None, return_div=False):
        B = int(x.shape[0])
        xs = self._xs(B)
        like = x if hasattr(x, "data_ptr") and x.is_cuda else None
        if out is None:
            out = _alloc_like(like, xs)
        div = _alloc_like(like, (B,)) if return_div else None
        tv = self._times(t, B)
        if tv is not None:
            (xp, tp, b0p, b1p, op, dp), dev, keep = self._ptrs((x, xs, False, "x"), tv, (beta0, (B,), False, "beta0"), (beta1, (B,), False, "beta1"),
                                                               (out, xs, True, "out"), (div, None, True, "out_div"))
            _lib.check(_lib.lib().ti_adw_drift_tv(self.h, xp, tp, b0p, b1p, B, op, dp, _lib.MEM_DEVICE if dev else _lib.MEM_HOST))
            return (out, div) if return_div else out
        (xp, b0p, b1p, op, dp), dev, keep = self._ptrs((x, xs, False, "x"), (beta0, (B,), False, "beta0"), (beta1, (B,), False, "beta1"),
                                                       (out, xs, True, "out"), (div, None, True, "out_div"))
        mem = _lib.MEM_DEVICE if dev else _lib.MEM_HOST
        if not return_div:
            _lib.check(_lib.lib().ti_adw_drift(self.h, xp, float(t), b0p, b1p, B, op, mem))
            return out
        _lib.check(_lib.lib().ti_adw_drift_div(self.h, xp, float(t), b0p, b1p, B, op, dp, mem))
        return out, div

    def rollout(self, x0, beta0, beta1, t_grid, scheme="euler", save_every=1, eps=0.0, seed=0, traj_offset=0, out=None,
                return_dlogp=False, rtol=1e-4, atol=1e-4, step_offset=0, step_control="batch", *, fused=False):
        B = int(x0.shape[0])
        on_gpu = hasattr(x0, "data_ptr") and x0.is_cuda
        rd = _rollout_desc(scheme, t_grid, save_every, _lib.MEM_DEVICE if on_gpu else _lib.MEM_HOST, eps, seed, traj_offset, False, rtol, atol,
                           step_offset, step_control)
        rows = int(_lib.lib().ti_rollout_rows(rd.n_step, rd.save_every))
        if out is None:
            out = _alloc_like(x0 if on_gpu else None, self._xs(rows, B))
        dl = _alloc_like(x0 if on_gpu else None, (rows, B)) if return_dlogp else None
        (xp, b0p, b1p, op, dp), dev, keep = self._ptrs((x0, self._xs(B), False, "x0"), (beta0, (B,), False, "beta0"), (beta1, (B,), False, "beta1"),
                                                       (out, self._xs(rows, B), True, "out"), (dl, None, True, "out_dlogp"))
        nfe = C.c_int64(0)
        if fused:
            _lib.check(_lib.lib().ti_adw_rollout_fused(self.h, C.byref(rd), xp, b0p, b1p, B, op, dp, C.byref(nfe)))
            return (out, dl, nfe.value) if return_dlogp else (out, nfe.value)
        if not return_dlogp:
            _lib.check(_lib.lib().ti_adw_rollout(self.h, C.byref(rd), xp, b0p, b1p, B, op, C.byref(nfe)))
            return out, nfe.value
        _lib.check(_lib.lib().ti_adw_rollout_dlogp(self.h, C.byref(rd), xp, b0p, b1p, B, op, dp, C.byref(nfe)))
        return out, dl, nfe.value


def selftest(device: int = 0):
    _lib.check(_lib.lib().ti_selftest(int(device)))
```

Before: 465,500.

## Precompute first-layer phi filter table per conditioning class for pair kernel

Adds a pre-pass that groups molecules by identical conditioning vectors into at most 16 classes, then builds a per-class, per-atom, per-type table of the first layer's phi-branch MLP outputs. The first-layer pair kernel then reads this table instead of recomputing the phi matrix products per edge, and streams only the W-branch weights. It also uses a larger superchunk for the 8-wave table build. The aim is to remove redundant first-layer message MLP work. In exchange it adds a class-detection kernel plus a blocking host sync per call, and it applies only to eligible f16x2 unmasked, non-ragged paths.

```diff
diff --git a/include/ti_hip.h b/include/ti_hip.h
--- a/include/ti_hip.h
+++ b/include/ti_hip.h
@@ -139,6 +139,8 @@
 int ti_painn_debug_tap(ti_handle* h, int stop_after_stage);
 int ti_painn_debug_read(ti_handle* h, int what, float* out, size_t n_floats);
 int ti_painn_debug_poison(ti_handle* h, int64_t B, float value);
+#define TI_PHI0_MAX_CLASSES 16
+int ti_painn_debug_phi0_path(ti_handle* h, int32_t* n_classes);
 int ti_selftest(int device);
 
 #ifdef __cplusplus
diff --git a/thermodynamic-interpolation_amd/_lib.py b/thermodynamic-interpolation_amd/_lib.py
--- a/thermodynamic-interpolation_amd/_lib.py
+++ b/thermodynamic-interpolation_amd/_lib.py
@@ -28,6 +28,7 @@
     "ti_obs_cv", "ti_obs_weights", "ti_obs_hist", "ti_obs_set_observer",
     "ti_adw_rollout_fused",
     "ti_obs_bootstrap",
+    "ti_painn_debug_phi0_path",
 ]
 OBS_KINDS = {"rmsd": 0, "dist": 1, "angle": 2, "torsion": 3, "coord": 4}
 BOOT_ESTIMATORS = {"ess": 0, "tfep": 1, "mean": 2}
@@ -120,6 +121,7 @@
     L.ti_painn_debug_tap.argtypes = [vp, C.c_int]
     L.ti_painn_debug_read.argtypes = [vp, C.c_int, fp, C.c_size_t]
     L.ti_painn_debug_poison.argtypes = [vp, C.c_int64, C.c_float]
+    L.ti_painn_debug_phi0_path.argtypes = [vp, ip]
     L.ti_selftest.argtypes = [C.c_int]
     L.ti_painn_drift_tv.argtypes = [vp, vp, vp, vp, C.c_int64, vp, C.c_int]
     L.ti_painn_drift_div_tv.argtypes = [vp, vp, vp, vp, C.c_int64, vp, vp, C.c_int]
diff --git a/thermodynamic-interpolation_amd/build.py b/thermodynamic-interpolation_amd/build.py
--- a/thermodynamic-interpolation_amd/build.py
+++ b/thermodynamic-interpolation_amd/build.py
@@ -16,8 +16,9 @@
            "ode_ragged_kernels.hip",
            "obs_kernels.hip",
            "adw_fused_kernels.hip",
-           "obs_boot_kernels.hip"]
-HEADERS = ["ti_handle.hpp", "rollout.hpp", "mfma_chain.hpp", "dispatch.hpp", "ti_internal.hpp", "ode_device.hpp", "adw_device.hpp", "painn_edge_kernel.hpp", "painn_pair_kernel.hpp", "pair_template.hpp",
+           "obs_boot_kernels.hip",
+           "painn_phi0_kernels.hip"]
+HEADERS = ["ti_handle.hpp", "rollout.hpp", "mfma_chain.hpp", "dispatch.hpp", "ti_internal.hpp", "ode_device.hpp", "adw_device.hpp", "painn_edge_kernel.hpp", "painn_pair_kernel.hpp", "pair_template.hpp", "message_stream.hpp",
            "painn_edge_kernel_body.inc", "painn_pair_kernel_body.inc", "painn_jvp_edge_body.inc", "painn_jvp_filter_body.inc", os.path.join("..", "..", "include", "ti_hip.h")]
 FLAGS = ["--offload-arch=gfx950", "-O3", "-std=c++17", "-fPIC", "-Xclang", "-target-feature", "-Xclang", "-packed-fp32-ops"]
 EXTRA_FLAGS = {"painn_edge_nb8.hip": ["-mllvm", "-amdgpu-spill-sgpr-to-vgpr=0"], "painn_edge_mask_nb8.hip": ["-mllvm", "-amdgpu-spill-sgpr-to-vgpr=0"]}
diff --git a/thermodynamic-interpolation_amd/csrc/api_painn.hip b/thermodynamic-interpolation_amd/csrc/api_painn.hip
--- a/thermodynamic-interpolation_amd/csrc/api_painn.hip
+++ b/thermodynamic-interpolation_amd/csrc/api_painn.hip
@@ -88,6 +88,8 @@
         float* od = sg.out(out, h->b1, n);
         float* otd = jvp ? sg.out(out_tan, h->tout, n) : nullptr;
         float* dd = div ? sg.out(out_div, h->divb, (size_t)B) : nullptr;
+        phi0_begin_call(h, cd, B, mode == DRIFT && !per_mol_t);
+        struct Phi0End { ti_handle* h; ~Phi0End() { phi0_end_call(h); } } phi0_end{h};
         if (mode == DRIFT_DIV_EST) {
             painn_make_probes(h, B, n_probes, probe_seed, traj_offset);
             painn_drift_div_est_dev(h, xd, t, cd, B, n_probes, od, dd, td);
@@ -168,6 +170,8 @@
         const int saved_tap = h->tap; h->tap = -1;
         const Ragged rg = ragged_of(h);
         if (mode == DRIFT_DIV_EST) painn_make_probes(h, B, n_probes, probe_seed, rd->traj_offset);
+        phi0_begin_call(h, cd, B, !dlogp && rd->scheme != TI_SCHEME_DOPRI5_TRAJ);
+        struct Phi0End { ti_handle* h; ~Phi0End() { phi0_end_call(h); } } phi0_end{h};
         DlogpAux aux;
         if (dlogp) {
             aux.dl = h->dl.p; aux.d1 = h->divb.p; aux.d2 = h->div2.p; aux.scaled = h->dlscaled.p; aux.out = out_dlogp;
@@ -219,6 +223,13 @@
     return TI_OK;
 }
 
+int ti_painn_debug_phi0_path(ti_handle* h, int32_t* n_classes)
+{
+    if (!h || h->kind != 0) return fail(TI_E_ARG, "not a painn handle");
+    if (n_classes) *n_classes = h->phi0_found;
+    return h->phi0_last;
+}
+
 int ti_painn_debug_poison(ti_handle* h, int64_t B, float value)
 {
     if (!h || h->kind != 0 || B <= 0) return fail(TI_E_ARG, "not a painn handle / B");
@@ -234,6 +245,7 @@
         HIP_CHECK(hipMemsetD32Async((hipDeviceptr_t)h->e.p, (int)bits, h->e.n, h->stream));
         HIP_CHECK(hipMemsetD32Async((hipDeviceptr_t)h->enc.p, (int)bits, h->enc.n, h->stream));
         HIP_CHECK(hipMemsetD32Async((hipDeviceptr_t)h->geo.p, (int)bits, h->geo.n, h->stream));
+        if (h->phi0_tab.n) HIP_CHECK(hipMemsetD32Async((hipDeviceptr_t)h->phi0_tab.p, (int)bits, h->phi0_tab.n, h->stream));
         return TI_OK;
     });
 }
diff --git a/thermodynamic-interpolation_amd/csrc/message_stream.hpp b/thermodynamic-interpolation_amd/csrc/message_stream.hpp
--- /dev/null
+++ b/thermodynamic-interpolation_amd/csrc/message_stream.hpp
@@ -0,0 +1,31 @@
+#pragma once
+#include <vector>
+
+namespace ti {
+
+enum MsgMatrix { MSG_W_W0 = 0, MSG_W_W1 = 1, MSG_PHI_W0E = 2 , MSG_PHI_W1 = 3, MSG_PHI_W2 = 4, MSG_W_W2 = 5 };
+enum MsgPart { MSG_ALL = 0, MSG_W = 1, MSG_PHI = 2 };
+struct MsgChunk { int matrix, row0; };
+
+inline bool msg_is_phi(int matrix) { return matrix == MSG_PHI_W0E || matrix == MSG_PHI_W1 || matrix == MSG_PHI_W2; }
+
+inline std::vector<MsgChunk> message_chunks(int NB, bool first, bool last, MsgPart part)
+{
+    std::vector<MsgChunk> out;
+    auto put = [&](int matrix, int row0) {
+        if (part == MSG_ALL || (part == MSG_PHI) == msg_is_phi(matrix)) out.push_back(MsgChunk{matrix, row0});
+    };
+    for (int m : {MSG_W_W0, MSG_W_W1, MSG_PHI_W0E, MSG_PHI_W1})
+        for (int nbo = 0; nbo < NB; ++nbo) put(m, 32 * nbo);
+    const int F = 32 * NB;
+    for (int nbo = 0; nbo < NB; ++nbo)
+        for (int c : {2, 3, 1, 0, 4}) {
+            if (c == 3 && last) continue;
+            if ((c == 0 || c == 4) && first) continue;
+            put(MSG_PHI_W2, c * F + 32 * nbo);
+            put(MSG_W_W2, c * F + 32 * nbo);
+        }
+    return out;
+}
+
+}
diff --git a/thermodynamic-interpolation_amd/csrc/painn_edge_kernel.hpp b/thermodynamic-interpolation_amd/csrc/painn_edge_kernel.hpp
--- a/thermodynamic-interpolation_amd/csrc/painn_edge_kernel.hpp
+++ b/thermodynamic-interpolation_amd/csrc/painn_edge_kernel.hpp
@@ -40,7 +40,7 @@
 static size_t edge_lds_bytes(int NB, int WAVES, bool h16) { return 2 * edge_superchunk(NB, WAVES, h16) * (size_t)edge_chunk4(NB, h16) * 16 + WAVES * 256 + 21 * (size_t)32 * NB * 4; }
 
 
-enum LayerPos { POS_MIDDLE = 0, POS_FIRST = 1, POS_LAST = 2, POS_ONLY = 3 };
+enum LayerPos { POS_MIDDLE = 0, POS_FIRST = 1, POS_LAST = 2, POS_ONLY = 3, POS_TABLE = 4, POS_FIRST_TABLE = 5, POS_ONLY_TABLE = 7 };
 inline int layer_pos(bool first, bool last) { return (first ? 1 : 0) | (last ? 2 : 0); }
 
 template <int NB, bool MASK, class F>
diff --git a/thermodynamic-interpolation_amd/csrc/painn_host.hip b/thermodynamic-interpolation_amd/csrc/painn_host.hip
--- a/thermodynamic-interpolation_amd/csrc/painn_host.hip
+++ b/thermodynamic-interpolation_amd/csrc/painn_host.hip
@@ -16,6 +16,32 @@
     h->divb.alloc(B); h->div2.alloc(B); h->dl.alloc(B); h->dlscaled.alloc(B);
     h->cap = B;
 }
+
+void phi0_begin_call(ti_handle* h, const float* cond_dev, long long B, bool eligible)
+{
+    h->phi0_ncls = 0; h->phi0_found = 0; h->phi0_B = 0; h->phi0_cond = nullptr;
+    if (!eligible || !h->phi0_ok || h->active != 2 || h->ragged || h->emask_B > 0 || h->tap >= 0 || h->nblk == 0) return;
+    const int A = h->d.n_atoms, F = h->d.n_features;
+    grow(h->phi0_cls, (size_t)B); grow(h->phi0_state, (size_t)PHI0_STATE_WORDS);
+    grow(h->phi0_tab, (size_t)TI_PHI0_MAX_CLASSES * A * PHI0_TYPES * 3 * F);
+    int32_t state[PHI0_STATE_WORDS];
+    {
+        Timed tm(h, TI_KERNEL_PAINN_EMBED);
+        HIP_CHECK(hipMemsetAsync(h->phi0_state.p, 0xff, sizeof(state), h->stream));
+        Phi0ClassParams p{};
+        p.cond = reinterpret_cast<const uint32_t*>(cond_dev); p.words = A * h->ncond; p.B = B; p.state = h->phi0_state.p; p.cls = h->phi0_cls.p;
+        HIP_CHECK(launch_phi0_classes(p, h->stream));
+    }
+    HIP_CHECK(hipMemcpyAsync(state, h->phi0_state.p, sizeof(state), hipMemcpyDeviceToHost, h->stream));
+    HIP_CHECK(hipStreamSynchronize(h->stream));
+    int n = 0;
+    while (n < TI_PHI0_MAX_CLASSES && state[n] >= 0) ++n;
+    const bool over = state[TI_PHI0_MAX_CLASSES] == 1;
+    h->phi0_found = over ? TI_PHI0_MAX_CLASSES + 1 : n;
+    if (over) return;
+    h->phi0_ncls = n; h->phi0_B = B; h->phi0_cond = cond_dev;
+}
+void phi0_end_call(ti_handle* h) { h->phi0_ncls = 0; h->phi0_B = 0; h->phi0_cond = nullptr; }
 
 long long jvp_virtual_molecules(const ti_handle* h, long long B, int D) { return (B + h->G - 1) / h->G * D * h->G; }
 
@@ -155,6 +181,17 @@
         Timed tm(h, TI_KERNEL_PAINN_EMBED);
         HIP_CHECK(launch_embed(NB, h->nE, prec, p, st));
     }
+    const bool table = h->phi0_ncls > 0 && h->phi0_B == B && h->phi0_cond == cond_dev && b0 == 0 && h->active == 2 && !tv && !jr && !nat && !mrows &&
+                       h->tap < 0 && h->nblk > 0 && L > 0;
+    h->phi0_last = table ? 1 : 0;
+    if (table) {
+        Phi0TableParams p{};
+        p.stream = h->S(h->st_phi0_tab); p.nch = h->st_phi0_tab.nch; p.vecs = h->edge_vecs1.p; p.edge_emb = h->F(h->edge_emb);
+        for (int i = 0; i < 6; ++i) p.wscale[i] = h->edge_scale[i];
+        p.P = h->P.p; p.state = h->phi0_state.p; p.n_cls = h->phi0_ncls; p.A = A; p.tab = h->phi0_tab.p;
+        Timed tm(h, TI_KERNEL_PAINN_EMBED);
+        HIP_CHECK(launch_phi0_table(NB, L == 1, p, st));
+    }
     h->last_B = B;
     if (h->tap == 0) return;
     for (int l = 0; l < L; ++l) {
@@ -198,8 +235,13 @@
 #ifdef TI_STAMPS
             if (l == 2) p.stamps = stamps_arm(groups, st);
 #endif
+            const bool on_table = table && l == 0;
+            if (on_table) {
+                p.stream = h->S(h->st_phi0_w); p.nch = h->st_phi0_w.nch; p.wpad = h->phi0_wpad;
+                p.phi0_tab = h->phi0_tab.p; p.cls = h->phi0_cls.p;
+            }
             if (h->active == 2) {
-                HIP_CHECK(launch_pair(NB, l == 0, l == L - 1, prec, p, st, mrows != nullptr));
+                HIP_CHECK(launch_pair(NB, l == 0, l == L - 1, prec, p, st, mrows != nullptr, on_table));
 #ifdef TI_STAMPS
                 stamps_dump(h, p.stamps, groups, st);
 #endif
diff --git a/thermodynamic-interpolation_amd/csrc/painn_kernels.hip b/thermodynamic-interpolation_amd/csrc/painn_kernels.hip
--- a/thermodynamic-interpolation_amd/csrc/painn_kernels.hip
+++ b/thermodynamic-interpolation_amd/csrc/painn_kernels.hip
@@ -444,6 +444,7 @@
     if ((e = configure_node<NODE_EMBED>(NB)) != hipSuccess) return e;
     if ((e = configure_node<NODE_UPDATE>(NB)) != hipSuccess) return e;
     if ((e = configure_node<NODE_READOUT>(NB)) != hipSuccess) return e;
+    if ((e = configure_phi0_kernels(NB)) != hipSuccess) return e;
     return with_message_units(NB, EVERY, [](auto bc, auto mc) {
         constexpr int nb = decltype(bc)::value;
         constexpr bool MASK = decltype(mc)::value;
@@ -467,11 +468,11 @@
 {
     return with_message_units(NB, masked, [&](auto bc, auto mc) { return launch_edge_unit<decltype(bc)::value, decltype(mc)::value>(first, last, prec, p, st); });
 }
-hipError_t launch_pair(int NB, bool first, bool last, int prec, const EdgeParams& p, hipStream_t st, bool masked)
+hipError_t launch_pair(int NB, bool first, bool last, int prec, const EdgeParams& p, hipStream_t st, bool masked, bool table)
 {
     return with_message_units(NB, masked, [&](auto bc, auto mc) {
         constexpr int nb = decltype(bc)::value;
-        if constexpr (pair_build_exists(nb, 4, TI_PREC_F32)) return launch_pair_unit<nb, decltype(mc)::value>(first, last, prec, p, st);
+        if constexpr (pair_build_exists(nb, 4, TI_PREC_F32)) return launch_pair_unit<nb, decltype(mc)::value>(first, last, prec, p, st, table);
         else return hipErrorInvalidValue;
     });
 }
diff --git a/thermodynamic-interpolation_amd/csrc/painn_pack.hip b/thermodynamic-interpolation_amd/csrc/painn_pack.hip
--- a/thermodynamic-interpolation_amd/csrc/painn_pack.hip
+++ b/thermodynamic-interpolation_amd/csrc/painn_pack.hip
@@ -1,3 +1,4 @@
+#include "message_stream.hpp"
 #include "pair_template.hpp"
 #include "ti_handle.hpp"
 
@@ -358,20 +359,31 @@
             const float S[6] = {matrix_pow2_scale(wts + h->w[l].W0, F, F, 0, F, wts + h->w[l].b0, F), matrix_pow2_scale(wts + h->w[l].W1, F, F, 0, F, wts + h->w[l].b1, F),
                                 matrix_pow2_scale(wts + h->phi[l].W0, 2 * F, F, 0, 2 * F, wts + h->phi[l].b0, F), matrix_pow2_scale(wts + h->phi[l].W1, F, F, 0, F, wts + h->phi[l].b1, F),
                                 matrix_pow2_scale(wts + h->phi[l].W2, F, 5 * F, 0, F, wts + h->phi[l].b2, 5 * F), matrix_pow2_scale(wts + h->w[l].W2, F, 5 * F, 0, F, wts + h->w[l].b2, 5 * F)};
-            auto layer1 = [&](size_t W, int ld, int n_rows, int col0, float sc) { for (int nbo = 0; nbo < NB; ++nbo) pack_chunk16_split1(pk, wts + W, ld, n_rows, 32 * nbo, col0, NBK, sc); };
+            auto pack_message = [&](MsgPart part) {
+                for (const MsgChunk& ch : message_chunks(NB, first, last, part)) {
+                    const size_t W = ch.matrix == MSG_W_W0 ? h->w[l].W0 : ch.matrix == MSG_W_W1 ? h->w[l].W1 : ch.matrix == MSG_PHI_W0E ? h->phi[l].W0
+                                   : ch.matrix == MSG_PHI_W1 ? h->phi[l].W1 : ch.matrix == MSG_PHI_W2 ? h->phi[l].W2 : h->w[l].W2;
+                    const int ld = ch.matrix == MSG_PHI_W0E ? 2 * F : F, n_rows = ch.matrix >= MSG_PHI_W2 ? 5 * F : F, col0 = ch.matrix == MSG_PHI_W0E ? F : 0;
+                    pack_chunk16_split1(pk, wts + W, ld, n_rows, ch.row0, col0, NBK, S[ch.matrix]);
+                }
+            };
             o = begin_stream();
-            layer1(h->w[l].W0, F, F, 0, S[0]); layer1(h->w[l].W1, F, F, 0, S[1]);
-            layer1(h->phi[l].W0, 2 * F, F, F, S[2]);
-            layer1(h->phi[l].W1, F, F, 0, S[3]);
-            for (int nbo = 0; nbo < NB; ++nbo)
-                for (int c : {2, 3, 1, 0, 4}) {
-                    if (c == 3 && last) continue;
-                    if ((c == 0 || c == 4) && first) continue;
-                    pack_chunk16_split1(pk, wts + h->phi[l].W2, F, 5 * F, c * F + 32 * nbo, 0, NBK, S[4]);
-                    pack_chunk16_split1(pk, wts + h->w[l].W2, F, 5 * F, c * F + 32 * nbo, 0, NBK, S[5]);
-                }
+            pack_message(MSG_ALL);
             h->st_edge1.push_back(end_stream16(o));
             h->edge_scale.insert(h->edge_scale.end(), S, S + 6);
+            if (first && h->has_pair && pair_table_build_exists(NB, prec, false)) {
+                o = begin_stream();
+                pack_message(MSG_W);
+                h->phi0_wpad = end_stream16(o).nch & 1;
+                pad_even(o);
+                h->st_phi0_w = end_stream16(o);
+                o = begin_stream();
+                pack_message(MSG_PHI);
+                pad_even(o);
+                h->st_phi0_tab = end_stream16(o);
+                h->phi0_ok = true;
+                if (const char* z = std::getenv("TI_PHI0_TABLE")) if (z[0] == '0') h->phi0_ok = false;
+            }
         }
         o = begin_stream();
         layer16(h->V[l], F, F, 0);
diff --git a/thermodynamic-interpolation_amd/csrc/painn_pair_kernel.hpp b/thermodynamic-interpolation_amd/csrc/painn_pair_kernel.hpp
--- a/thermodynamic-interpolation_amd/csrc/painn_pair_kernel.hpp
+++ b/thermodynamic-interpolation_amd/csrc/painn_pair_kernel.hpp
@@ -3,20 +3,20 @@
 
 namespace ti {
 
-__host__ __device__ constexpr int pair_superchunk() { return 2; }
-static size_t pair_lds_bytes(int NB, int WAVES, int PREC)
+__host__ __device__ constexpr int pair_superchunk(int NB = 0, int WAVES = 0, bool TABLE = false) { return TABLE && WAVES == 8 && NB == 4 ? 4 : 2; }
+static size_t pair_lds_bytes(int NB, int WAVES, int PREC, bool TABLE = false)
 {
-    return (size_t)2 * pair_superchunk() * edge_chunk4(NB, false) * 16 + WAVES * 256 + 21 * (size_t)32 * NB * 4 +
-           (pair_folds_cross(PREC) ? (size_t)WAVES * 12 * 64 * 4 : 0);
+    return (size_t)2 * pair_superchunk(NB, WAVES, TABLE) * edge_chunk4(NB, false) * 16 + WAVES * 256 + 21 * (size_t)32 * NB * 4 +
+           (pair_folds_cross(PREC) && !TABLE ? (size_t)WAVES * 12 * 64 * 4 : 0);
 }
 
-template <int NBK, bool FIRST, bool LAST, int PREC, int WAVES>
+template <int NBK, bool FIRST, bool LAST, int PREC, int WAVES, bool TABLE = false>
 __global__ __launch_bounds__(64 * WAVES, 2 * 4 / WAVES) void painn_pair_kernel(const EdgeParams p)
 #define TI_PAIR_ROWS p.rows
 #include "painn_pair_kernel_body.inc"
 #undef TI_PAIR_ROWS
 
-template <int NBK, bool FIRST, bool LAST, int PREC, int WAVES>
+template <int NBK, bool FIRST, bool LAST, int PREC, int WAVES, bool TABLE = false>
 __global__ __launch_bounds__(64 * WAVES, 2 * 4 / WAVES) void painn_pair_mask_kernel(const EdgeParams p)
 #define TI_PAIR_ROWS (p.rows + (size_t)gi * p.nblk * 16)
 #include "painn_pair_kernel_body.inc"
@@ -30,12 +30,14 @@
     dispatch_int<4, 8>(waves, [&](auto wc) { dispatch_int<0, 1>(prec, [&](auto pc) {
         constexpr int WAVES = decltype(wc)::value, PREC = decltype(pc)::value;
         if constexpr (pair_build_exists(NB, WAVES, PREC))
-            dispatch_int<POS_MIDDLE, POS_FIRST, POS_LAST, POS_ONLY>(pos, [&](auto oc) {
-                constexpr bool FIRST = (decltype(oc)::value & 1) != 0, LAST = (decltype(oc)::value & 2) != 0;
-                any = true;
-                if (e != hipSuccess) return;
-                if constexpr (MASK) e = f(painn_pair_mask_kernel<2 * NB, FIRST, LAST, PREC, WAVES>, WAVES, pair_lds_bytes(NB, WAVES, PREC));
-                else e = f(painn_pair_kernel<2 * NB, FIRST, LAST, PREC, WAVES>, WAVES, pair_lds_bytes(NB, WAVES, PREC));
+            dispatch_int<POS_MIDDLE, POS_FIRST, POS_LAST, POS_ONLY, POS_FIRST_TABLE, POS_ONLY_TABLE>(pos, [&](auto oc) {
+                constexpr bool FIRST = (decltype(oc)::value & 1) != 0, LAST = (decltype(oc)::value & 2) != 0, TABLE = (decltype(oc)::value & 4) != 0;
+                if constexpr (!TABLE || pair_table_build_exists(NB, PREC, MASK)) {
+                    any = true;
+                    if (e != hipSuccess) return;
+                    if constexpr (MASK) e = f(painn_pair_mask_kernel<2 * NB, FIRST, LAST, PREC, WAVES>, WAVES, pair_lds_bytes(NB, WAVES, PREC));
+                    else e = f(painn_pair_kernel<2 * NB, FIRST, LAST, PREC, WAVES, TABLE>, WAVES, pair_lds_bytes(NB, WAVES, PREC, TABLE));
+                }
             });
     }); });
     return any ? e : hipErrorInvalidValue;
@@ -47,10 +49,11 @@
     return with_pair_builds<NB, MASK>(EVERY, EVERY, EVERY, [](auto kernel, int, size_t lds) { return set_lds(kernel, lds); });
 }
 template <int NB, bool MASK>
-hipError_t launch_pair_unit(bool first, bool last, int prec, const EdgeParams& p, hipStream_t st)
+hipError_t launch_pair_unit(bool first, bool last, int prec, const EdgeParams& p, hipStream_t st, bool table)
 {
+    if (table && !first) return hipErrorInvalidValue;
     const bool wide = prec == 1 && p.n_groups >= 2048;
-    return with_pair_builds<NB, MASK>(wide ? 8 : 4, prec, layer_pos(first, last), [&](auto kernel, int waves, size_t lds) {
+    return with_pair_builds<NB, MASK>(wide ? 8 : 4, prec, layer_pos(first, last) | (table ? POS_TABLE : 0), [&](auto kernel, int waves, size_t lds) {
         hipLaunchKernelGGL(kernel, dim3((unsigned)((p.n_groups + waves - 1) / waves)), dim3(64 * waves), lds, st, p);
         return hipGetLastError();
     });
diff --git a/thermodynamic-interpolation_amd/csrc/painn_pair_kernel_body.inc b/thermodynamic-interpolation_amd/csrc/painn_pair_kernel_body.inc
--- a/thermodynamic-interpolation_amd/csrc/painn_pair_kernel_body.inc
+++ b/thermodynamic-interpolation_amd/csrc/painn_pair_kernel_body.inc
@@ -1,12 +1,13 @@
 {
     static_assert(PREC == 0 || PREC == 1, "the fp16 storage mode keeps the directed message kernel");
+    static_assert(!TABLE || (FIRST && PREC == 1), "the phi table serves layer 0 of the split path");
     constexpr int F = 16 * NBK, NB = (F + 31) / 32, T = 64 * WAVES, CH4 = edge_chunk4(NB, false);
     using A16 = r16::Act<NBK>;
     constexpr bool ONE = edge_one_chain(PREC);
     using OP = std::conditional_t<ONE, r16::Opnd1<NBK>, typename r16::OpSel<NBK, PREC>::type>;
     extern __shared__ f32x4 lds[];
     const int lane = threadIdx.x & 63, wave = __builtin_amdgcn_readfirstlane(threadIdx.x >> 6), j = lane & 15, q = lane >> 4;
-    constexpr int SC = pair_superchunk(), NBUF = 2;
+    constexpr int SC = pair_superchunk(NB, WAVES, TABLE), NBUF = 2;
     float* scratch = reinterpret_cast<float*>(lds + NBUF * SC * CH4) + wave * 64;
     float* vec = reinterpret_cast<float*>(lds + NBUF * SC * CH4) + WAVES * 64;
     for (int i = threadIdx.x; i < EV::COUNT * F / 4; i += T)
@@ -32,6 +33,13 @@
     float* const ds_g = p.dsacc + gnode0 * F;
     float* const dv_g = p.dvacc + gnode0 * 3 * F;
     float* const c_g = p.cacc + gnode0 * 3 * F;
+    unsigned clsw = 0;
+    if constexpr (TABLE)
+        for (int m = 0; m < p.G; ++m) clsw |= (unsigned)p.cls[gi * p.G + ((unsigned)m < mol_cap ? (unsigned)m : mol_cap)] << (4 * m);
+    auto tab_off = [&](int mol_local, int atom, int type) {
+        const unsigned cls = (clsw >> (4 * mol_local)) & 15u;
+        return ((cls * (unsigned)p.A + (unsigned)atom) * (unsigned)PHI0_TYPES + (unsigned)type) * (unsigned)(3 * F);
+    };
 
 #ifdef TI_STAMPS
     constexpr int STAMP_SLOTS = 64;
@@ -110,7 +118,7 @@
             TI_STAMP();
         }
         OP h2A, h2B;
-        {
+        if constexpr (!TABLE) {
             OP inA, inB;
             A16 tA, tB;
             float scA, scB;
@@ -176,14 +184,30 @@
             return off < F ? ds_g + (lnode * (unsigned)F + (unsigned)off) : off < 4 * F ? dv_g + (lnode * (unsigned)(3 * F) + (unsigned)(off - F)) : c_g + (lnode * (unsigned)(3 * F) + (unsigned)(off - 4 * F));
         };
         const unsigned lIq = lnode_of(prow_molI(mi[0]), prow_atomI(mi[0]));
+        unsigned tfA[4], tfB[4], trA = 0, trB = 0;
+        f32x4 tv[3][4];
+        if constexpr (TABLE) {
+#pragma unroll
+            for (int r = 0; r < 4; ++r) {
+                tfA[r] = tab_off(prow_molI(mi[r]), prow_atomI(mi[r]), prow_type(mi[r])) + (unsigned)j;
+                tfB[r] = tab_off(prow_molJ(mi[r]), prow_atomJ(mi[r]), prow_type(mi[r])) + (unsigned)j;
+            }
+            trA = tab_off(prow_molI(meta), prow_atomI(meta), prow_type(meta));
+            trB = tab_off(prow_molJ(meta), prow_atomJ(meta), prow_type(meta));
+        }
 
         auto out3 = [&](int c, int nbo, f32x4& rA0, f32x4& rA1, f32x4& rB0, f32x4& rB1) {
             const float* bp = vec + (EV::P_B2 + c) * F + 32 * nbo + j;
             const float* bw = vec + (EV::W_B2 + c) * F + 32 * nbo + j;
             const float p0 = bp[0], p1 = bp[16], q0 = bw[0], q1 = bw[16];
             f32x4 a0 = {p0, p0, p0, p0}, a1 = {p1, p1, p1, p1}, b0 = a0, b1 = a1, w0 = {q0, q0, q0, q0}, w1 = {q1, q1, q1, q1};
-            r16::gemm_x2_on_pipe<true>(a0, a1, b0, b1, h2A, h2B, pipe, lane);
-            pipe.release();
+            if constexpr (TABLE) {
+                const int sl = c == 2 ? 0 : 1;
+                a0 = tv[sl][0]; a1 = tv[sl][1]; b0 = tv[sl][2]; b1 = tv[sl][3];
+            } else {
+                r16::gemm_x2_on_pipe<true>(a0, a1, b0, b1, h2A, h2B, pipe, lane);
+                pipe.release();
+            }
             r16::gemm_on_pipe<true>(w0, w1, g2, pipe, lane);
             pipe.release();
             w0 *= wfac; w1 *= wfac;
@@ -220,6 +244,20 @@
         for (int nbo = 0; nbo < NB; ++nbo) {
             const int fo = 32 * nbo + j;
             TI_STAMP();
+            if constexpr (TABLE) {
+                const float* const tb = p.phi0_tab + 32 * nbo;
+#pragma unroll
+                for (int sl = 0; sl < 2; ++sl)
+#pragma unroll
+                    for (int r = 0; r < 4; ++r) {
+                        tv[sl][0][r] = tb[tfA[r] + (unsigned)(sl * F)]; tv[sl][1][r] = tb[tfA[r] + (unsigned)(sl * F + 16)];
+                        tv[sl][2][r] = tb[tfB[r] + (unsigned)(sl * F)]; tv[sl][3][r] = tb[tfB[r] + (unsigned)(sl * F + 16)];
+                    }
+                if constexpr (!LAST) {
+                    tv[2][0] = r16::load_block(p.phi0_tab + trA + (unsigned)(2 * F), 2 * nbo, q); tv[2][1] = r16::load_block(p.phi0_tab + trA + (unsigned)(2 * F), 2 * nbo + 1, q);
+                    tv[2][2] = r16::load_block(p.phi0_tab + trB + (unsigned)(2 * F), 2 * nbo, q); tv[2][3] = r16::load_block(p.phi0_tab + trB + (unsigned)(2 * F), 2 * nbo + 1, q);
+                }
+            }
             {
                 f32x4 a0, a1, b0, b1;
                 out3(2, nbo, a0, a1, b0, b1);
@@ -245,8 +283,12 @@
                         oB0 = r16::load_block(eb, 2 * nbo, q); oB1 = r16::load_block(eb, 2 * nbo + 1, q);
                     }
                 }
-                r16::gemm_x2_on_pipe<false>(a0, a1, b0, b1, h2A, h2B, pipe, lane);
-                pipe.release();
+                if constexpr (TABLE) {
+                    a0 = tv[2][0]; a1 = tv[2][1]; b0 = tv[2][2]; b1 = tv[2][3];
+                } else {
+                    r16::gemm_x2_on_pipe<false>(a0, a1, b0, b1, h2A, h2B, pipe, lane);
+                    pipe.release();
+                }
                 r16::gemm_on_pipe<false>(w0, w1, g2, pipe, lane);
                 pipe.release();
                 w0 *= wrow; w1 *= wrow;
@@ -367,6 +409,7 @@
                 }
             }
         }
+        if constexpr (TABLE) { if (p.wpad) pipe.release(); }
     }
     pipe.drain();
 #ifdef TI_STAMPS
diff --git a/thermodynamic-interpolation_amd/csrc/painn_pair_mask_nb1.hip b/thermodynamic-interpolation_amd/csrc/painn_pair_mask_nb1.hip
--- a/thermodynamic-interpolation_amd/csrc/painn_pair_mask_nb1.hip
+++ b/thermodynamic-interpolation_amd/csrc/painn_pair_mask_nb1.hip
@@ -2,5 +2,5 @@
 
 namespace ti {
 template hipError_t configure_pair_unit<1, true>();
-template hipError_t launch_pair_unit<1, true>(bool, bool, int, const EdgeParams&, hipStream_t);
+template hipError_t launch_pair_unit<1, true>(bool, bool, int, const EdgeParams&, hipStream_t, bool);
 }
diff --git a/thermodynamic-interpolation_amd/csrc/painn_pair_mask_nb2.hip b/thermodynamic-interpolation_amd/csrc/painn_pair_mask_nb2.hip
--- a/thermodynamic-interpolation_amd/csrc/painn_pair_mask_nb2.hip
+++ b/thermodynamic-interpolation_amd/csrc/painn_pair_mask_nb2.hip
@@ -2,5 +2,5 @@
 
 namespace ti {
 template hipError_t configure_pair_unit<2, true>();
-template hipError_t launch_pair_unit<2, true>(bool, bool, int, const EdgeParams&, hipStream_t);
+template hipError_t launch_pair_unit<2, true>(bool, bool, int, const EdgeParams&, hipStream_t, bool);
 }
diff --git a/thermodynamic-interpolation_amd/csrc/painn_pair_mask_nb4.hip b/thermodynamic-interpolation_amd/csrc/painn_pair_mask_nb4.hip
--- a/thermodynamic-interpolation_amd/csrc/painn_pair_mask_nb4.hip
+++ b/thermodynamic-interpolation_amd/csrc/painn_pair_mask_nb4.hip
@@ -2,5 +2,5 @@
 
 namespace ti {
 template hipError_t configure_pair_unit<4, true>();
-template hipError_t launch_pair_unit<4, true>(bool, bool, int, const EdgeParams&, hipStream_t);
+template hipError_t launch_pair_unit<4, true>(bool, bool, int, const EdgeParams&, hipStream_t, bool);
 }
diff --git a/thermodynamic-interpolation_amd/csrc/painn_pair_nb1.hip b/thermodynamic-interpolation_amd/csrc/painn_pair_nb1.hip
--- a/thermodynamic-interpolation_amd/csrc/painn_pair_nb1.hip
+++ b/thermodynamic-interpolation_amd/csrc/painn_pair_nb1.hip
@@ -2,5 +2,5 @@
 
 namespace ti {
 template hipError_t configure_pair_unit<1, false>();
-template hipError_t launch_pair_unit<1, false>(bool, bool, int, const EdgeParams&, hipStream_t);
+template hipError_t launch_pair_unit<1, false>(bool, bool, int, const EdgeParams&, hipStream_t, bool);
 }
diff --git a/thermodynamic-interpolation_amd/csrc/painn_pair_nb2.hip b/thermodynamic-interpolation_amd/csrc/painn_pair_nb2.hip
--- a/thermodynamic-interpolation_amd/csrc/painn_pair_nb2.hip
+++ b/thermodynamic-interpolation_amd/csrc/painn_pair_nb2.hip
@@ -2,5 +2,5 @@
 
 namespace ti {
 template hipError_t configure_pair_unit<2, false>();
-template hipError_t launch_pair_unit<2, false>(bool, bool, int, const EdgeParams&, hipStream_t);
+template hipError_t launch_pair_unit<2, false>(bool, bool, int, const EdgeParams&, hipStream_t, bool);
 }
diff --git a/thermodynamic-interpolation_amd/csrc/painn_pair_nb4.hip b/thermodynamic-interpolation_amd/csrc/painn_pair_nb4.hip
--- a/thermodynamic-interpolation_amd/csrc/painn_pair_nb4.hip
+++ b/thermodynamic-interpolation_amd/csrc/painn_pair_nb4.hip
@@ -2,5 +2,5 @@
 
 namespace ti {
 template hipError_t configure_pair_unit<4, false>();
-template hipError_t launch_pair_unit<4, false>(bool, bool, int, const EdgeParams&, hipStream_t);
+template hipError_t launch_pair_unit<4, false>(bool, bool, int, const EdgeParams&, hipStream_t, bool);
 }
diff --git a/thermodynamic-interpolation_amd/csrc/painn_phi0_kernels.hip b/thermodynamic-interpolation_amd/csrc/painn_phi0_kernels.hip
--- /dev/null
+++ b/thermodynamic-interpolation_amd/csrc/painn_phi0_kernels.hip
@@ -0,0 +1,141 @@
+#include "painn_edge_kernel.hpp"
+
+namespace ti {
+
+__global__ __launch_bounds__(256) void painn_phi0_class_kernel(const Phi0ClassParams p)
+{
+    const long long m = (long long)blockIdx.x * 256 + threadIdx.x;
+    if (m >= p.B) return;
+    const uint32_t* const mine = p.cond + (size_t)m * p.words;
+    int k = 0;
+    for (; k < TI_PHI0_MAX_CLASSES; ++k) {
+        int r = __hip_atomic_load(p.state + k, __ATOMIC_RELAXED, __HIP_MEMORY_SCOPE_AGENT);
+        if (r < 0) {
+            const int lead = __builtin_amdgcn_readfirstlane((int)m);
+            int old = 0;
+            if ((int)m == lead) old = atomicCAS(p.state + k, -1, lead);
+            old = __builtin_amdgcn_readfirstlane(old);
+            if (old < 0 && (int)m == lead) break;
+            r = old < 0 ? lead : old;
+        }
+        const uint32_t* const other = p.cond + (size_t)r * p.words;
+        bool same = true;
+        for (int i = 0; i < p.words && same; ++i) same = mine[i] == other[i];
+        if (same) break;
+    }
+    if (k == TI_PHI0_MAX_CLASSES) { p.state[TI_PHI0_MAX_CLASSES] = 1; k = 0; }
+    p.cls[m] = (uint8_t)k;
+}
+
+template <int NBK, bool LAST>
+__global__ __launch_bounds__(256) void painn_phi0_table_kernel(const Phi0TableParams p)
+{
+    constexpr int F = 16 * NBK, NB = (F + 31) / 32, WAVES = 4, T = 64 * WAVES, CH4 = edge_chunk4(NB, false), SC = 2;
+    using A16 = r16::Act<NBK>;
+    using OP = r16::Opnd1<NBK>;
+    extern __shared__ f32x4 lds[];
+    const int lane = threadIdx.x & 63, wave = __builtin_amdgcn_readfirstlane(threadIdx.x >> 6), j = lane & 15, q = lane >> 4;
+    float* vec = reinterpret_cast<float*>(lds + 2 * SC * CH4);
+    for (int i = threadIdx.x; i < EV::COUNT * F / 4; i += T)
+        reinterpret_cast<f32x4*>(vec)[i] = reinterpret_cast<const f32x4*>(p.vecs)[i];
+    PipeDMA<NB, T, SC, CH4> pipe;
+    pipe.init(reinterpret_cast<const f32x4*>(p.stream), p.nch, lds, wave, lane);
+    const float eps_p0 = 1e-5f * p.wscale[2] * p.wscale[2], eps_p1 = 1e-5f * p.wscale[3] * p.wscale[3], s_p0 = p.wscale[2];
+
+    const int n_rows = p.n_cls * p.A * PHI0_TYPES, row0 = (blockIdx.x * WAVES + wave) * 16;
+    const int row = row0 + j < n_rows ? row0 + j : n_rows - 1;
+    const int type = row % PHI0_TYPES, atom = (row / PHI0_TYPES) % p.A, cls = row / (PHI0_TYPES * p.A);
+    const float* const PI = p.P + ((size_t)p.state[cls] * p.A + atom) * F;
+
+    OP h2A;
+    {
+        OP inA;
+        A16 tA;
+        r16::load_set(tA, p.edge_emb + type * F, q);
+        const float scA = inA.set_scaled(tA);
+        const float ivA = r16::pow2_inverse(scA) * s_p0;
+#pragma unroll
+        for (int c = 0; c < NB; ++c) {
+            f32x4 a0 = r16::load_block(PI, 2 * c, q) * ivA, a1 = r16::load_block(PI, 2 * c + 1, q) * ivA;
+            r16::gemm_on_pipe<false>(a0, a1, inA, pipe, lane);
+            tA.b[2 * c] = a0 * scA; tA.b[2 * c + 1] = a1 * scA;
+            pipe.release();
+        }
+        r16::ln_silu(tA, vec + EV::P_G0 * F, vec + EV::P_BE0 * F, q, eps_p0);
+        inA.set(tA);
+#pragma unroll
+        for (int c = 0; c < NB; ++c) {
+            f32x4 a0 = r16::load_block(vec + EV::P_B1 * F, 2 * c, q), a1 = r16::load_block(vec + EV::P_B1 * F, 2 * c + 1, q);
+            r16::gemm_on_pipe<false>(a0, a1, inA, pipe, lane);
+            tA.b[2 * c] = a0; tA.b[2 * c + 1] = a1;
+            pipe.release();
+        }
+        r16::ln_silu(tA, vec + EV::P_G1 * F, vec + EV::P_BE1 * F, q, eps_p1);
+        h2A.set(tA);
+    }
+    auto flipped = [&](int c, int sl, int nbo) {
+        const float* bp = vec + (EV::P_B2 + c) * F + 32 * nbo + j;
+        const float p0 = bp[0], p1 = bp[16];
+        f32x4 a0 = {p0, p0, p0, p0}, a1 = {p1, p1, p1, p1};
+        r16::gemm_on_pipe<true>(a0, a1, h2A, pipe, lane);
+        pipe.release();
+#pragma unroll
+        for (int r = 0; r < 4; ++r) {
+            const int tr = row0 + 4 * q + r;
+            if (tr < n_rows) {
+                float* d = p.tab + ((size_t)tr * 3 + sl) * F + 32 * nbo + j;
+                d[0] = a0[r]; d[16] = a1[r];
+            }
+        }
+    };
+#pragma unroll 1
+    for (int nbo = 0; nbo < NB; ++nbo) {
+        flipped(2, 0, nbo);
+        if constexpr (!LAST) {
+            f32x4 a0 = r16::load_block(vec + (EV::P_B2 + 3) * F, 2 * nbo, q), a1 = r16::load_block(vec + (EV::P_B2 + 3) * F, 2 * nbo + 1, q);
+            r16::gemm_on_pipe<false>(a0, a1, h2A, pipe, lane);
+            pipe.release();
+            if (row0 + j < n_rows) {
+                float* d = p.tab + ((size_t)(row0 + j) * 3 + 2) * F;
+                r16::store_block(d, 2 * nbo, q, a0); r16::store_block(d, 2 * nbo + 1, q, a1);
+            }
+        }
+        flipped(1, 1, nbo);
+    }
+    pipe.drain();
+}
+
+static size_t phi0_lds_bytes(int NB) { return (size_t)2 * 2 * edge_chunk4(NB, false) * 16 + 21 * (size_t)32 * NB * 4; }
+
+template <class Fn>
+static hipError_t with_phi0_builds(int NB, int last, Fn&& f)
+{
+    hipError_t e = hipSuccess;
+    const bool any = dispatch_int<1, 2, 4>(NB, [&](auto bc) { dispatch_bool(last, [&](auto lc) {
+        if (e == hipSuccess) e = f(painn_phi0_table_kernel<2 * decltype(bc)::value, decltype(lc)::value>, phi0_lds_bytes(decltype(bc)::value));
+    }); });
+    return any ? e : hipErrorInvalidValue;
+}
+
+hipError_t configure_phi0_kernels(int NB)
+{
+    if (!pair_table_build_exists(NB, TI_PREC_F16X2, false)) return hipSuccess;
+    return with_phi0_builds(NB, EVERY, [](auto kernel, size_t lds) { return set_lds(kernel, lds); });
+}
+
+hipError_t launch_phi0_classes(const Phi0ClassParams& p, hipStream_t st)
+{
+    hipLaunchKernelGGL(painn_phi0_class_kernel, dim3((unsigned)((p.B + 255) / 256)), dim3(256), 0, st, p);
+    return hipGetLastError();
+}
+
+hipError_t launch_phi0_table(int NB, bool last, const Phi0TableParams& p, hipStream_t st)
+{
+    const int n_rows = p.n_cls * p.A * PHI0_TYPES;
+    return with_phi0_builds(NB, last, [&](auto kernel, size_t lds) {
+        hipLaunchKernelGGL(kernel, dim3((unsigned)((n_rows + 63) / 64)), dim3(256), lds, st, p);
+        return hipGetLastError();
+    });
+}
+
+}
diff --git a/thermodynamic-interpolation_amd/csrc/ti_handle.hpp b/thermodynamic-interpolation_amd/csrc/ti_handle.hpp
--- a/thermodynamic-interpolation_amd/csrc/ti_handle.hpp
+++ b/thermodynamic-interpolation_amd/csrc/ti_handle.hpp
@@ -87,6 +87,9 @@
     DevBuf<float> x, cond, s, P, v, dsacc, dvacc, cacc, e, enc, geo, b1, b2, xt, edge_vecs, edge_vecs1, upd_vecs;
     std::vector<float> edge_scale;
     int tap = -1; long long last_B = 0;
+    bool phi0_ok = false; Stream st_phi0_w{}, st_phi0_tab{}; int phi0_wpad = 0;
+    DevBuf<uint8_t> phi0_cls; DevBuf<int32_t> phi0_state; DevBuf<float> phi0_tab;
+    int phi0_ncls = 0, phi0_found = 0, phi0_last = -1; long long phi0_B = 0; const float* phi0_cond = nullptr;
     std::vector<Stream> st_jvp_update, st_jvp_phi; Stream st_jvp_readout{}; std::vector<int> jvp_phi_pad;
     DevBuf<float> jvp_ro_vecs, ts, tP, tv, tdsacc, tdvacc, tcacc, te, tout, wq, phist, nodest, divb, dl, dlscaled, div2;
     long long jvp_cap = 0, last_VB = 0; int last_D = 1;
@@ -222,6 +225,8 @@
 void painn_make_probes(ti_handle* h, long long B, int k, uint64_t seed, long long traj0);
 void painn_drift_div_est_dev(ti_handle* h, const float* x_dev, float t, const float* cond_dev, long long B, int k, float* out_dev,
                              float* est_dev, const float* tv = nullptr);
+void phi0_begin_call(ti_handle* h, const float* cond_dev, long long B, bool eligible);
+void phi0_end_call(ti_handle* h);
 int set_graph_state(ti_handle* h, std::vector<uint32_t>& m, std::vector<int32_t>& natoms, std::vector<uint8_t>& ptype, long long B);
 void clear_graph_state(ti_handle* h);
 
diff --git a/thermodynamic-interpolation_amd/csrc/ti_internal.hpp b/thermodynamic-interpolation_amd/csrc/ti_internal.hpp
--- a/thermodynamic-interpolation_amd/csrc/ti_internal.hpp
+++ b/thermodynamic-interpolation_amd/csrc/ti_internal.hpp
@@ -52,7 +52,32 @@
     float wscale[6];
     float* geo;
     unsigned long long* stamps;
-};
+    const float* phi0_tab;
+    const uint8_t* cls;
+    int wpad;
+};
+
+constexpr int PHI0_TYPES = 4;
+static_assert(TI_PHI0_MAX_CLASSES <= 16, "the pair kernel packs the class ids of a group's <= 8 molecules into one 32-bit word");
+constexpr int PHI0_STATE_WORDS = TI_PHI0_MAX_CLASSES + 1;
+struct Phi0ClassParams {
+    const uint32_t* cond; int words;
+    long long B;
+    int32_t* state;
+    uint8_t* cls;
+};
+struct Phi0TableParams {
+    const float4* stream; int nch;
+    const float* vecs; const float* edge_emb; float wscale[6];
+    const float* P;
+    const int32_t* state;
+    int n_cls, A;
+    float* tab;
+};
+hipError_t launch_phi0_classes(const Phi0ClassParams& p, hipStream_t st);
+hipError_t launch_phi0_table(int NB, bool last, const Phi0TableParams& p, hipStream_t st);
+hipError_t configure_phi0_kernels(int NB);
+__host__ __device__ constexpr bool pair_table_build_exists(int NB, int PREC, bool MASK) { return PREC == TI_PREC_F16X2 && !MASK && (NB == 1 || NB == 2 || NB == 4); }
 
 struct EmbedParams {
     const float4* stream; int nch;
@@ -83,7 +108,7 @@
 hipError_t launch_embed(int NB, int nseg, int prec, const EmbedParams& p, hipStream_t st);
 hipError_t launch_edge(int NB, bool first, bool last, int prec, const EdgeParams& p, hipStream_t st, bool masked = false);
 __host__ __device__ constexpr bool edge_one_chain(int prec) { return prec == TI_PREC_F16X2; }
-hipError_t launch_pair(int NB, bool first, bool last, int prec, const EdgeParams& p, hipStream_t st, bool masked = false);
+hipError_t launch_pair(int NB, bool first, bool last, int prec, const EdgeParams& p, hipStream_t st, bool masked = false, bool table = false);
 __host__ __device__ constexpr bool pair_build_exists(int NB, int WAVES, int PREC)
 {
     return (NB == 1 || NB == 2 || NB == 4) && (PREC == TI_PREC_F32 ? WAVES == 4 : PREC == TI_PREC_F16X2 && (WAVES == 4 || WAVES == 8));
@@ -94,7 +119,7 @@
 hipError_t configure_painn_kernels(int NB);
 template <int NB, bool MASK> hipError_t launch_edge_unit(bool first, bool last, int prec, const EdgeParams& p, hipStream_t st);
 template <int NB, bool MASK> hipError_t configure_edge_unit();
-template <int NB, bool MASK> hipError_t launch_pair_unit(bool first, bool last, int prec, const EdgeParams& p, hipStream_t st);
+template <int NB, bool MASK> hipError_t launch_pair_unit(bool first, bool last, int prec, const EdgeParams& p, hipStream_t st, bool table);
 template <int NB, bool MASK> hipError_t configure_pair_unit();
 
 struct JvpFilterParams {
diff --git a/thermodynamic-interpolation_amd/engine.py b/thermodynamic-interpolation_amd/engine.py
--- a/thermodynamic-interpolation_amd/engine.py
+++ b/thermodynamic-interpolation_amd/engine.py
@@ -445,6 +445,11 @@
     def debug_poison(self, B: int, value: float):
         _lib.check(_lib.lib().ti_painn_debug_poison(self.h, int(B), float(value)))
 
+    def debug_phi0_path(self):
+        n = np.zeros(1, np.int32)
+        path = _lib.lib().ti_painn_debug_phi0_path(self.h, _lib.iptr(n))
+        return int(path), int(n[0])
+
     def debug_read(self, what: str, B: int):
         shape = {"s": (B, self.A, self.F), "v": (B, self.A, 3, self.F), "e": (B, self.E, self.F)}[what[-1]]
         out = np.empty(shape, np.float32)
```

After: 491,200 (median of 6 runs). +5.5%, better.
